# jianzhnie/RLZero

Measured on AMD Instinct MI355X. Metric: mcts_sims_per_sec, higher is better.
Workload: dtype f32 net (hi + lo f16 operand pairs on the f16 MFMA pipe, f32 accumulation) / f64 tree

## Files before the change

### include/rlzero_hip.h

```cpp
#ifndef RLZERO_HIP_H
#define RLZERO_HIP_H

#include <stdint.h>

#ifdef __cplusplus
extern "C" {
#endif

#define RZ_ABI_VERSION 31
#define RZ_MAX_BOARD_SIZE 16
#define RZ_BOARD_WORDS 4
#define RZ_MAX_IN_FLIGHT 16

enum {
    RZ_OK = 0,
    RZ_ERR_ARG = -1,
    RZ_ERR_HIP = -2,
    RZ_ERR_OOM = -3,
    RZ_ERR_OVERFLOW = -4,
    RZ_ERR_ILLEGAL = -5,
    RZ_ERR_INTERNAL = -6
};

enum {
    RZ_GAME_GOMOKU = 0,
    RZ_GAME_CONNECT4 = 1
};

enum {
    RZ_SCORE_UCT_REF = 0,
    RZ_SCORE_PUCT = 1
};

enum { RZ_EVAL_V0 = 0, RZ_EVAL_VLIN = 1 };

enum {
    RZ_FLAG_ARENA_FULL = 1,
    RZ_FLAG_BLOCKS_FULL = 2,
    RZ_FLAG_ILLEGAL_MOVE = 4,
    RZ_FLAG_LOGTAB = 8,
    RZ_FLAG_INTERNAL = 16,
    RZ_FLAG_REUSE_DROPPED = 32
};

typedef struct rz_engine rz_engine;

typedef struct rz_config {
    int32_t abi_version;
    int32_t game_kind;
    int32_t board_size;
    int32_t n_in_row;
    int32_t n_games;
    int32_t n_playout;
    int32_t score_mode;
    int32_t add_noise;
    double c_puct;
    double pool_factor;
    int32_t device;
    int32_t noise_seed;
    int32_t board_height;
    int32_t board_width;
    int32_t sims_in_flight;
    int32_t in_flight_impl;
} rz_config;

typedef struct rz_stats {
    int32_t error_flags;
    int32_t first_bad_game;
    int64_t arena_slots;
    int64_t prior_floats;
    int64_t max_slots_used;
    int64_t max_blocks_used;
    int64_t device_bytes;
    int64_t n_select_calls;
    int64_t reuse_dropped;
} rz_stats;

int rz_abi_version(void);
const char *rz_source_hash(void);
const char *rz_last_error(void);

int rz_create(const rz_config *cfg, rz_engine **out);
int rz_destroy(rz_engine *e);
int rz_geometry(rz_engine *e, int32_t *height, int32_t *width, int32_t *n_actions);

int rz_upload_log_table(rz_engine *e, const double *h_table, int64_t count);
int rz_log_table_size(rz_engine *e, int64_t *count);

int rz_set_roots(rz_engine *e, const uint64_t *d_stones, const int32_t *d_to_move,
                 const int32_t *d_last_move, const uint8_t *d_mask, int reset_trees,
                 void *stream);
int rz_get_roots(rz_engine *e, uint64_t *d_stones, int32_t *d_to_move, int32_t *d_last_move,
                 void *stream);
int rz_set_active(rz_engine *e, const uint8_t *d_active, void *stream);
int rz_set_noise_keys(rz_engine *e, const uint64_t *d_keys, const uint8_t *d_mask, void *stream);

int rz_select_step(rz_engine *e, float *d_obs, void *stream);
int rz_set_in_flight(rz_engine *e, int32_t k_backup, int32_t k_select);

int rz_leaf_buffers(rz_engine *e, const uint64_t **d_stones, const int32_t **d_to_move, const int32_t **d_last_cell);

int rz_encode_leaf_obs(rz_engine *e, float *d_obs, void *stream);
int rz_encode_root_obs(rz_engine *e, float *d_obs, void *stream);

int rz_get_leaves(rz_engine *e, uint64_t *d_stones, int32_t *d_to_move, int32_t *d_last_move,
                  int32_t *d_terminal, void *stream);

int rz_eval_synthetic(rz_engine *e, int kind, float *d_logp, float *d_value, void *stream);

int rz_eval_rollout(rz_engine *e, uint64_t seed, uint32_t sim_index, int32_t n_limit, float *d_value,
                    void *stream);

int rz_expand_backup(rz_engine *e, const float *d_logp, const float *d_value, void *stream);
int rz_expand_backup_f64(rz_engine *e, const float *d_logp, const double *d_value, void *stream);
int rz_expand_backup_probs(rz_engine *e, const float *d_probs, const double *d_value, void *stream);

int rz_tree_step(rz_engine *e, const float *d_logp, const float *d_value, float *d_obs, void *stream);

typedef struct rz_raw_heads {
    const float *raw;
    const float *hid;
    const float *w2;
    const float *b2;
    const float *act_scale;
    const float *act_bias;
    const float *val_scale;
    const float *val_bias;
    int64_t raw_part_stride;
    int64_t hid_part_stride;
    int32_t ld;
    int32_t n_parts;
} rz_raw_heads;

int rz_expand_backup_raw(rz_engine *e, const rz_raw_heads *heads, void *stream);
int rz_tree_step_raw(rz_engine *e, const rz_raw_heads *heads, float *d_obs, void *stream);

typedef struct rz_value_head {
    const float *valfeat;
    const float *w1t;
    const float *b1;
    const float *w2;
    const float *b2;
    int32_t ld;
    int32_t groups;
} rz_value_head;
typedef struct rz_deferred_logits {
    const float *raw;
    int32_t ld;
    int32_t rows_per_slot;
} rz_deferred_logits;
int rz_deferred_reserve(rz_engine *e, int32_t slots);
int rz_trace_attach(rz_engine *e, void *d_trace);
int rz_device_view(rz_engine *e, void *out, int64_t out_bytes);
int rz_set_playouts(rz_engine *e, const int32_t *d_counts, const int32_t *d_order, void *stream);
int rz_playouts_view(rz_engine *e, const int32_t **d_counts, const int32_t **d_order);
int rz_playouts_read(rz_engine *e, int32_t *h_counts, int32_t *h_order, int32_t *h_source);
int rz_deferred_slots(rz_engine *e, const int32_t **d_slot_of_game);
int rz_expand_backup_deferred(rz_engine *e, const rz_value_head *head, void *stream);
int rz_tree_step_deferred(rz_engine *e, const rz_value_head *head, void *stream);
int rz_deferred_flush(rz_engine *e, const rz_deferred_logits *logits, int32_t n_slots, void *stream);
typedef struct rz_kept_rows {
    const int32_t *rows;
    const int32_t *count;
    int64_t capacity;
    int32_t n_games;
    int32_t reserved;
} rz_kept_rows;
int rz_deferred_keep(rz_engine *e, rz_kept_rows *out, void *stream);
int rz_deferred_flush_kept(rz_engine *e, const rz_deferred_logits *logits, void *stream);
int rz_deferred_keep_stats(rz_engine *e, uint64_t *h_out2, int32_t reset);

int rz_root_visits(rz_engine *e, int32_t *d_visits, void *stream);
int rz_root_wsum(rz_engine *e, double *d_w, void *stream);
int rz_root_priors(rz_engine *e, float *d_p, void *stream);
int rz_root_stats(rz_engine *e, int32_t *d_n, double *d_w, void *stream);
int rz_root_values(rz_engine *e, double *d_out, void *stream);

int rz_advance_roots(rz_engine *e, const int32_t *d_moves, void *stream);

int rz_step_games(rz_engine *e, const int32_t *d_moves, int32_t *d_winner, uint8_t *d_ended,
                  void *stream);

#define RZ_PLAY_RECORD_WORDS 8
enum {
    RZ_PLAY_RUNNING = 1,
    RZ_PLAY_STALLED = 2,
    RZ_PLAY_RESOLVED = 4,
    RZ_PLAY_ENDED = 8,
    RZ_PLAY_SEARCHED = 16,
    RZ_PLAY_RESIGNED = 32,
    RZ_PLAY_NO_RESIGN = 64,
    RZ_PLAY_WOULD_RESIGN = 128,
    RZ_PLAY_FULL = 256
};
typedef struct rz_play_config {
    uint64_t seed;
    double temperature;
    double stall_margin;
    const int64_t *d_queue_ids;
    int32_t *d_queue_ctl;
    int32_t *d_log;
    int32_t ring_steps;
    int32_t reserved;
} rz_play_config;
int rz_play_attach(rz_engine *e, const rz_play_config *cfg);
int rz_play_draw(rz_engine *e, void *stream);
int rz_play_apply(rz_engine *e, void *stream);
int rz_play_set_resign(rz_engine *e, double threshold, double disabled_frac, void *stream);
int rz_play_set_cap(rz_engine *e, int32_t n_fast, double p_full, void *stream);
int rz_play_set_cap_order(rz_engine *e, int32_t longest_first);
int rz_play_set_match(rz_engine *e, const uint64_t *d_open_stones, const int32_t *d_open_to_move, const int32_t *d_open_last, int32_t n_openings,
                      void *stream);
int rz_play_side(rz_engine *e, int32_t side, void *stream);
int rz_active_read(rz_engine *e, uint8_t *h_active);
int rz_play_resolve(rz_engine *e, int32_t slot, int32_t move, void *stream);
int rz_play_stop(rz_engine *e, void *stream);
int rz_play_state(rz_engine *e, int64_t *h_game_id, int32_t *h_ply, int32_t *h_state, int64_t *h_steps);

int rz_get_stats(rz_engine *e, rz_stats *out);
int rz_clear_errors(rz_engine *e);
int rz_poll_errors(rz_engine *e, int32_t *h_flags, int32_t *h_reuse_dropped, void *stream);

int rz_copy_arena(rz_engine *e, int32_t game, int64_t max_slots, int32_t *h_n, double *h_w,
                  int32_t *h_first_child, int32_t *h_n_visited, int32_t *h_n_children,
                  int32_t *h_prior_block, float *h_root_prior, int32_t *h_top);
int rz_copy_priors(rz_engine *e, int32_t game, int64_t max_floats, float *h_priors, int32_t *h_count);

int rz_uct_scores(rz_engine *e, const double *d_w, const int32_t *d_n, const int32_t *d_np,
                  double c_puct, double *d_out, int64_t count, void *stream);

typedef struct rz_net rz_net;
enum {
    RZ_NET_DIRECT = 0,
    RZ_NET_WINOGRAD_F4 = 1,
    RZ_NET_SPLIT_F16 = 2
    ,
    RZ_NET_SPLIT_F16_TILES = 3
    ,
    RZ_NET_SPLIT_F16_FP8 = 4
};
int rz_net_range_info(rz_net *net, float *h_info8);
enum { RZ_NET_FLAG_F16_RANGE = 1 };
int rz_net_error_flags(rz_net *net, uint32_t *h_flags);
int rz_net_set_algo(rz_net *net, int32_t algo);
int rz_net_set_max_workgroups(rz_net *net, int32_t max_workgroups);
enum { RZ_NET_HEADS_AUTO = 0, RZ_NET_HEADS_F32 = 1, RZ_NET_HEADS_SPLIT_32 = 2, RZ_NET_HEADS_SPLIT_64 = 3, RZ_NET_HEADS_SPLIT_PARTS = 4,
       RZ_NET_HEADS_IN_TRUNK = 5    };
int rz_net_set_heads_algo(rz_net *net, int32_t heads_algo);
int rz_net_create(int32_t height, int32_t width, int32_t n_actions, int32_t device, rz_net **out);
int rz_net_destroy(rz_net *net);
int rz_net_load(rz_net *net, const float *const *h_params, int32_t n_params);
int rz_net_reserve(rz_net *net, int32_t max_boards);
int rz_net_trunk(rz_net *net, const float *d_obs, int32_t n_boards, float *d_feat, void *stream);
int rz_net_trunk_leaves(rz_net *net, const uint64_t *d_stones, const int32_t *d_to_move, const int32_t *d_last_cell,
                        int32_t n_boards, void *stream);
int rz_net_deferred_reserve(rz_net *net, int32_t max_boards, int32_t slots);
int rz_net_trunk_leaves_deferred(rz_net *net, const uint64_t *d_stones, const int32_t *d_to_move, const int32_t *d_last_cell,
                                 int32_t n_boards, const int32_t *d_slot_of_board, rz_value_head *out, void *stream);
int rz_net_deferred_gemm(rz_net *net, int32_t n_boards, int32_t n_slots, rz_deferred_logits *out, void *stream);
int rz_net_deferred_gemm_rows(rz_net *net, const rz_kept_rows *kept, rz_deferred_logits *out, void *stream);
int rz_net_trace_attach(rz_net *net, void *d_trace);
int rz_net_delta_reserve(rz_net *net, int32_t n_games);
int rz_net_delta_invalidate(rz_net *net, void *stream);
int rz_net_delta_resident(rz_net *net, int32_t on);
int rz_net_delta_bases(rz_net *net, const uint64_t *d_root_stones, const int32_t *d_root_to_move, int32_t n_games, void *stream);
int rz_net_delta_leaves(rz_net *net, const uint64_t *d_stones, const int32_t *d_to_move, const int32_t *d_last_cell, int32_t n_boards,
                        const int32_t *d_slot_of_board, const uint8_t *d_active, float *d_feat32, int32_t without_base, rz_value_head *out,
                        void *stream);
int rz_net_delta_bases_engine(rz_net *net, rz_engine *engine, void *stream);
int rz_net_delta_step(rz_net *net, rz_engine *engine, rz_value_head *out, void *stream);
int rz_net_delta_trunk_engine(rz_net *net, rz_engine *engine, void *stream);
int rz_net_delta_stats(rz_net *net, uint32_t *h_out8, int32_t reset);
int rz_net_search_resident(rz_net *net, rz_engine *engine, int32_t n_sims, int32_t select_first, void *stream);
int rz_net_heads(rz_net *net, int32_t n_boards, float *d_logp, float *d_value, void *stream);
int rz_net_heads_gemm(rz_net *net, int32_t n_boards, rz_raw_heads *out, void *stream);
int rz_net_forward(rz_net *net, const float *d_obs, int32_t n_boards, float *d_logp,
                   float *d_value, void *stream);

typedef struct rz_muzero rz_muzero;
typedef struct rz_mz_config {
    int32_t abi_version;
    int32_t n_games;
    int32_t n_actions;
    int32_t n_sims;
    double discount;
    double pb_c_base;
    double pb_c_init;
    int32_t device;
    int32_t reserved;
} rz_mz_config;

int rz_mz_create(const rz_mz_config *cfg, rz_muzero **out);
int rz_mz_destroy(rz_muzero *e);
int rz_mz_upload_log_table(rz_muzero *e, const double *h_table, int64_t count);
int rz_mz_init_roots(rz_muzero *e, const float *d_probs, const double *d_noise, double noise_frac,
                     const uint8_t *d_mask, void *stream);
int rz_mz_select(rz_muzero *e, int32_t *d_parent, int32_t *d_action, int32_t *d_leaf, const uint8_t *d_mask,
                 void *stream);
int rz_mz_expand_backup(rz_muzero *e, const float *d_reward, const float *d_probs, const float *d_value,
                        const uint8_t *d_mask, void *stream);
int rz_mz_load_model(rz_muzero *e, const float *const *h_params, int32_t n_params, int32_t hidden);
int rz_mz_search(rz_muzero *e, float *d_hidden, int32_t n_sims, int32_t *d_trace_parent, int32_t *d_trace_action,
                 int32_t *d_trace_leaf, float *d_trace_reward, float *d_trace_probs, float *d_trace_value, void *stream);
int rz_mz_set_search_shape(rz_muzero *e, int32_t games_per_workgroup);
typedef struct rz_mz_cartpole_play {
    double *d_state;
    int64_t *d_steps, *d_episode, *d_episode_start;
    uint64_t env_seed, noise_seed;
    double noise_frac, dirichlet_alpha, temperature;
    double *d_ring;
    int32_t ring_steps, reserved;
    int64_t first_step;
    double *d_arena;
    int64_t arena_rows;
    int64_t *d_counters, *d_entries;
    int64_t max_entries;
} rz_mz_cartpole_play;
int rz_mz_load_representation(rz_muzero *e, const float *const *h_params, int32_t n_params, int32_t obs_dim, int32_t hidden);
int rz_mz_play_cartpole(rz_muzero *e, float *d_hidden, int32_t n_sims, int32_t n_moves, const rz_mz_cartpole_play *play, void *stream);
int rz_cartpole_step(double *d_state, int64_t *d_steps, int64_t *d_episode, const int64_t *d_actions, int32_t n_envs, uint64_t seed,
                     float *d_obs, float *d_reward, uint8_t *d_terminated, uint8_t *d_truncated, void *stream);
int rz_mz_root_children(rz_muzero *e, int32_t what, void *d_out, void *stream);
int rz_mz_root_stats(rz_muzero *e, int32_t *d_n, double *d_value_sum, double *d_vmin, double *d_vmax, void *stream);
int rz_mz_geometry(rz_muzero *e, int32_t *slots_per_game, int64_t *device_bytes);
int rz_mz_error_flags(rz_muzero *e, int32_t *flags);

typedef struct rz_replay rz_replay;
int rz_replay_create(int32_t board_size, int64_t capacity, int32_t device, rz_replay **out);
int rz_replay_destroy(rz_replay *r);
int rz_replay_set_tables(rz_replay *r, const int16_t *h_src_state, const int16_t *h_src_pi, void *stream);
int rz_replay_state(rz_replay *r, int64_t *count, int64_t *cursor, int64_t *capacity);
int rz_replay_add(rz_replay *r, int32_t n_games, const int32_t *h_offsets, const int32_t *h_moves, const uint8_t *h_keep,
                  const int32_t *h_winner, const float *h_pi, void *stream);
int rz_replay_gather(rz_replay *r, const int64_t *h_indices, const int64_t *d_indices, int64_t n, float *d_states, float *d_pis,
                     float *d_zs, void *stream);
int rz_replay_sample(rz_replay *r, uint64_t seed, uint64_t step, int64_t n, float *d_states, float *d_pis, float *d_zs,
                     void *stream);
int rz_replay_read(rz_replay *r, int64_t first, int64_t n, uint64_t *h_stones, int32_t *h_meta, float *h_pi, void *stream);
int rz_replay_poll_errors(rz_replay *r, int32_t *flags, void *stream);

#ifdef __cplusplus
}
#endif
#endif
```

### profiles/microbench/delta_resident_phases.py

```python
import ctypes, os, sys
sys.path.insert(0, os.environ.get('GRAFT_REPO_ROOT', '.'))
import rlzero_amd._hip as H
H.library_path = lambda: os.environ.get('RZ_NETPROF_LIB') or os.path.join(os.path.dirname(os.path.abspath(__file__)), 'librlzero_netprof.so')
import rlzero_amd._build as B
B.needs_build = lambda: False
import numpy as np, torch
from rlzero_amd.engine import HipNetEvaluator, MCTSEngine
from rlzero_amd.games.gomoku.policy_value_net import PolicyValueNet
lib = H.load()
NAMES = [(0, 'leaf + changed cells'), (1, 'distances, requests, ranks'), (3, 'maps, base records'), (4, 'bar'), (5, 'conv1'), (6, 'bar'), (7, 'conv2'),
         (9, 'bar + conv3 + heads'), (10, 'bar'), (11, 'features'), (12, 'bar'), (16, 'value layer'), (17, 'expand + backup'),
         (2, 'sel: root record'), (8, 'sel: root scan / answer'), (13, 'sel: level-0 cell'), (14, 'sel: deeper levels'), (15, 'sel: terminal test + leaf stores'),
         (18, 'selection (rest: hand-over)'), (19, 'wave 1: pre-scan'), (20, 'wave 1: wait behind it')]
sizes = [int(a) for a in sys.argv[1:]] or [1, 256, 512]
for games in sizes:
    torch.manual_seed(0)
    net = PolicyValueNet(15).to('cuda:0')
    ev = HipNetEvaluator(net, 15, 'cuda:0', max_boards=games)
    sims = 800
    eng = MCTSEngine(15, 5, n_games=games, n_playout=sims, device='cuda:0', add_noise=True)
    eng.reset_games()
    assert ev.resident_ok(eng) and ev.resident_delta_ok(eng)
    rng = np.random.default_rng(0)
    for ply in range(6):
        eng.sim_chunk(ev, 40)
        visits = eng.root_visits()
        moves = np.array([int(rng.choice(np.flatnonzero(v > 0))) for v in visits], dtype=np.int32)
        eng.advance(moves)
        eng.step(moves)
    a, b = torch.cuda.Event(enable_timing=True), torch.cuda.Event(enable_timing=True)
    ev.hip.delta_stats(reset=True)
    a.record(); eng.sim_chunk(ev, sims); b.record(); torch.cuda.synchronize()
    st = ev.hip.delta_stats()
    out = (ctypes.c_longlong * 24)()
    assert lib.rz_net_debug_profile(out) == 0
    us = 1e3 * a.elapsed_time(b) / sims
    total = out[23] / sims
    print('%d games, %d simulations: %.2f us per simulation of a game (events, bases included), %d cycles (%.2f GHz); %.2f conv3 / %.2f conv2 tiles, %.2f changed cells per leaf, %d leaves without a base' % (
        games, sims, us, total, total / us / 1e3, st['tiles3'] / max(1, st['delta'] + st['no_base']), st['tiles2'] / max(1, st['delta'] + st['no_base']),
        st['cells'] / max(1, st['delta'] + st['no_base']), st['no_base']))
    print('   ' + '  '.join('%s=%d' % (nm, out[k] / sims) for k, nm in NAMES) + '  prescans=%d' % st['prescans'], flush=True)
    eng.close(); ev.hip.close()
```

### rlzero_amd/_hip.py

```python
import ctypes
import os
from ctypes import (POINTER, Structure, c_char_p, c_double, c_int, c_int32, c_int64, c_uint32, c_uint64,
                    c_void_p)

ABI_VERSION = 31
BOARD_WORDS = 4
MAX_BOARD_SIZE = 16
MAX_IN_FLIGHT = 16

OK = 0
SCORE_UCT_REF, SCORE_PUCT = 0, 1
GAME_GOMOKU, GAME_CONNECT4 = 0, 1
NET_DIRECT, NET_WINOGRAD_F4, NET_SPLIT_F16, NET_SPLIT_F16_TILES, NET_SPLIT_F16_FP8 = 0, 1, 2, 3, 4
NET_FLAG_F16_RANGE = 1
NET_HEADS_AUTO, NET_HEADS_F32, NET_HEADS_SPLIT_32, NET_HEADS_SPLIT_64, NET_HEADS_SPLIT_PARTS, NET_HEADS_IN_TRUNK = 0, 1, 2, 3, 4, 5
EVAL_V0, EVAL_VLIN = 0, 1
FLAG_NAMES = {1: 'arena full', 2: 'block queue full', 4: 'illegal move', 8: 'ln table too short',
              16: 'internal'}
FLAG_REUSE_DROPPED = 32


class RzConfig(Structure):
    _fields_ = [('abi_version', c_int32), ('game_kind', c_int32), ('board_size', c_int32),
                ('n_in_row', c_int32), ('n_games', c_int32), ('n_playout', c_int32),
                ('score_mode', c_int32), ('add_noise', c_int32), ('c_puct', c_double),
                ('pool_factor', c_double), ('device', c_int32), ('noise_seed', c_int32),
                ('board_height', c_int32), ('board_width', c_int32),
                ('sims_in_flight', c_int32), ('in_flight_impl', c_int32)]


class RzStats(Structure):
    _fields_ = [('error_flags', c_int32), ('first_bad_game', c_int32), ('arena_slots', c_int64),
                ('prior_floats', c_int64), ('max_slots_used', c_int64), ('max_blocks_used', c_int64),
                ('device_bytes', c_int64), ('n_select_calls', c_int64), ('reuse_dropped', c_int64)]


class RzMzConfig(Structure):
    _fields_ = [('abi_version', c_int32), ('n_games', c_int32), ('n_actions', c_int32), ('n_sims', c_int32),
                ('discount', c_double), ('pb_c_base', c_double), ('pb_c_init', c_double),
                ('device', c_int32), ('reserved', c_int32)]


class RzMzCartPolePlay(Structure):
    _fields_ = [('d_state', c_void_p), ('d_steps', c_void_p), ('d_episode', c_void_p), ('d_episode_start', c_void_p),
                ('env_seed', c_uint64), ('noise_seed', c_uint64), ('noise_frac', c_double), ('dirichlet_alpha', c_double),
                ('temperature', c_double), ('d_ring', c_void_p), ('ring_steps', c_int32), ('reserved', c_int32),
                ('first_step', c_int64), ('d_arena', c_void_p), ('arena_rows', c_int64), ('d_counters', c_void_p),
                ('d_entries', c_void_p), ('max_entries', c_int64)]


class RzRawHeads(Structure):
    _fields_ = [('raw', c_void_p), ('hid', c_void_p), ('w2', c_void_p), ('b2', c_void_p), ('act_scale', c_void_p),
                ('act_bias', c_void_p), ('val_scale', c_void_p), ('val_bias', c_void_p), ('raw_part_stride', c_int64),
                ('hid_part_stride', c_int64), ('ld', c_int32), ('n_parts', c_int32)]


class RzValueHead(Structure):
    _fields_ = [('valfeat', c_void_p), ('w1t', c_void_p), ('b1', c_void_p), ('w2', c_void_p), ('b2', c_void_p),
                ('ld', c_int32), ('groups', c_int32)]


class RzDeferredLogits(Structure):
    _fields_ = [('raw', c_void_p), ('ld', c_int32), ('rows_per_slot', c_int32)]


class RzKeptRows(Structure):
    _fields_ = [('rows', c_void_p), ('count', c_void_p), ('capacity', c_int64), ('n_games', c_int32), ('reserved', c_int32)]


class RzPlayConfig(Structure):
    _fields_ = [('seed', c_uint64), ('temperature', c_double), ('stall_margin', c_double), ('d_queue_ids', c_void_p),
                ('d_queue_ctl', c_void_p), ('d_log', c_void_p), ('ring_steps', c_int32), ('reserved', c_int32)]


PLAY_RECORD_WORDS = 8
PLAY_RUNNING, PLAY_STALLED, PLAY_RESOLVED, PLAY_ENDED, PLAY_SEARCHED = 1, 2, 4, 8, 16
PLAY_RESIGNED, PLAY_NO_RESIGN, PLAY_WOULD_RESIGN = 32, 64, 128
PLAY_FULL = 256
REPLAY_BAD_INDEX = 1


class HipError(RuntimeError):
    pass


P = c_void_p

_SIGNATURES = {
    'rz_abi_version': (c_int, []),
    'rz_last_error': (c_char_p, []),
    'rz_source_hash': (c_char_p, []),
    'rz_create': (c_int, [POINTER(RzConfig), POINTER(c_void_p)]),
    'rz_destroy': (c_int, [P]),
    'rz_geometry': (c_int, [P, POINTER(c_int32), POINTER(c_int32), POINTER(c_int32)]),
    'rz_upload_log_table': (c_int, [P, P, c_int64]),
    'rz_log_table_size': (c_int, [P, POINTER(c_int64)]),
    'rz_set_roots': (c_int, [P, P, P, P, P, c_int, P]),
    'rz_get_roots': (c_int, [P, P, P, P, P]),
    'rz_set_active': (c_int, [P, P, P]),
    'rz_set_noise_keys': (c_int, [P, P, P, P]),
    'rz_select_step': (c_int, [P, P, P]),
    'rz_set_in_flight': (c_int, [P, c_int32, c_int32]),
    'rz_leaf_buffers': (c_int, [P, POINTER(c_void_p), POINTER(c_void_p), POINTER(c_void_p)]),
    'rz_encode_leaf_obs': (c_int, [P, P, P]),
    'rz_encode_root_obs': (c_int, [P, P, P]),
    'rz_get_leaves': (c_int, [P, P, P, P, P, P]),
    'rz_eval_synthetic': (c_int, [P, c_int, P, P, P]),
    'rz_eval_rollout': (c_int, [P, c_uint64, c_uint32, c_int32, P, P]),
    'rz_expand_backup': (c_int, [P, P, P, P]),
    'rz_expand_backup_f64': (c_int, [P, P, P, P]),
    'rz_expand_backup_probs': (c_int, [P, P, P, P]),
    'rz_tree_step': (c_int, [P, P, P, P, P]),
    'rz_expand_backup_raw': (c_int, [P, POINTER(RzRawHeads), P]),
    'rz_tree_step_raw': (c_int, [P, POINTER(RzRawHeads), P, P]),
    'rz_trace_attach': (c_int, [P, P]),
    'rz_net_trace_attach': (c_int, [P, P]),
    'rz_device_view': (c_int, [P, P, c_int64]),
    'rz_deferred_reserve': (c_int, [P, c_int32]),
    'rz_deferred_slots': (c_int, [P, POINTER(c_void_p)]),
    'rz_expand_backup_deferred': (c_int, [P, POINTER(RzValueHead), P]),
    'rz_tree_step_deferred': (c_int, [P, POINTER(RzValueHead), P]),
    'rz_deferred_flush': (c_int, [P, POINTER(RzDeferredLogits), c_int32, P]),
    'rz_deferred_keep': (c_int, [P, POINTER(RzKeptRows), P]),
    'rz_deferred_flush_kept': (c_int, [P, POINTER(RzDeferredLogits), P]),
    'rz_deferred_keep_stats': (c_int, [P, POINTER(c_uint64), c_int32]),
    'rz_root_visits': (c_int, [P, P, P]),
    'rz_root_wsum': (c_int, [P, P, P]),
    'rz_root_priors': (c_int, [P, P, P]),
    'rz_root_stats': (c_int, [P, P, P, P]),
    'rz_root_values': (c_int, [P, P, P]),
    'rz_advance_roots': (c_int, [P, P, P]),
    'rz_step_games': (c_int, [P, P, P, P, P]),
    'rz_play_attach': (c_int, [P, POINTER(RzPlayConfig)]),
    'rz_play_draw': (c_int, [P, P]),
    'rz_play_apply': (c_int, [P, P]),
    'rz_play_set_resign': (c_int, [P, c_double, c_double, P]),
    'rz_play_set_cap': (c_int, [P, c_int32, c_double, P]),
    'rz_set_playouts': (c_int, [P, P, P, P]),
    'rz_playouts_view': (c_int, [P, POINTER(c_void_p), POINTER(c_void_p)]),
    'rz_play_set_cap_order': (c_int, [P, c_int32]),
    'rz_playouts_read': (c_int, [P, P, P, POINTER(c_int32)]),
    'rz_play_set_match': (c_int, [P, P, P, P, c_int32, P]),
    'rz_play_side': (c_int, [P, c_int32, P]),
    'rz_active_read': (c_int, [P, P]),
    'rz_play_resolve': (c_int, [P, c_int32, c_int32, P]),
    'rz_play_stop': (c_int, [P, P]),
    'rz_play_state': (c_int, [P, P, P, P, POINTER(c_int64)]),
    'rz_get_stats': (c_int, [P, POINTER(RzStats)]),
    'rz_clear_errors': (c_int, [P]),
    'rz_poll_errors': (c_int, [P, POINTER(c_int32), POINTER(c_int32), P]),
    'rz_copy_arena': (c_int, [P, c_int32, c_int64, P, P, P, P, P, P, P, P]),
    'rz_copy_priors': (c_int, [P, c_int32, c_int64, P, P]),
    'rz_uct_scores': (c_int, [P, P, P, P, c_double, P, c_int64, P]),
    'rz_net_create': (c_int, [c_int32, c_int32, c_int32, c_int32, POINTER(c_void_p)]),
    'rz_net_destroy': (c_int, [P]),
    'rz_net_set_algo': (c_int, [P, c_int32]),
    'rz_net_set_max_workgroups': (c_int, [P, c_int32]),
    'rz_net_set_heads_algo': (c_int, [P, c_int32]),
    'rz_net_error_flags': (c_int, [P, POINTER(ctypes.c_uint32)]),
    'rz_net_range_info': (c_int, [P, POINTER(ctypes.c_float)]),
    'rz_net_load': (c_int, [P, POINTER(c_void_p), c_int32]),
    'rz_net_reserve': (c_int, [P, c_int32]),
    'rz_net_trunk': (c_int, [P, P, c_int32, P, P]),
    'rz_net_trunk_leaves': (c_int, [P, P, P, P, c_int32, P]),
    'rz_net_deferred_reserve': (c_int, [P, c_int32, c_int32]),
    'rz_net_trunk_leaves_deferred': (c_int, [P, P, P, P, c_int32, P, POINTER(RzValueHead), P]),
    'rz_net_deferred_gemm': (c_int, [P, c_int32, c_int32, POINTER(RzDeferredLogits), P]),
    'rz_net_deferred_gemm_rows': (c_int, [P, POINTER(RzKeptRows), POINTER(RzDeferredLogits), P]),
    'rz_net_search_resident': (c_int, [P, P, c_int32, c_int32, P]),
    'rz_net_delta_reserve': (c_int, [P, c_int32]),
    'rz_net_delta_invalidate': (c_int, [P, P]),
    'rz_net_delta_resident': (c_int, [P, c_int32]),
    'rz_net_delta_bases': (c_int, [P, P, P, c_int32, P]),
    'rz_net_delta_leaves': (c_int, [P, P, P, P, c_int32, P, P, P, c_int32, POINTER(RzValueHead), P]),
    'rz_net_delta_stats': (c_int, [P, POINTER(ctypes.c_uint32), c_int32]),
    'rz_net_delta_bases_engine': (c_int, [P, P, P]),
    'rz_net_delta_step': (c_int, [P, P, POINTER(RzValueHead), P]),
    'rz_net_delta_trunk_engine': (c_int, [P, P, P]),
    'rz_net_heads': (c_int, [P, c_int32, P, P, P]),
    'rz_net_heads_gemm': (c_int, [P, c_int32, POINTER(RzRawHeads), P]),
    'rz_net_forward': (c_int, [P, P, c_int32, P, P, P]),
    'rz_mz_create': (c_int, [POINTER(RzMzConfig), POINTER(c_void_p)]),
    'rz_mz_destroy': (c_int, [P]),
    'rz_mz_upload_log_table': (c_int, [P, P, c_int64]),
    'rz_mz_init_roots': (c_int, [P, P, P, c_double, P, P]),
    'rz_mz_select': (c_int, [P, P, P, P, P, P]),
    'rz_mz_expand_backup': (c_int, [P, P, P, P, P, P]),
    'rz_mz_load_model': (c_int, [P, POINTER(c_void_p), c_int32, c_int32]),
    'rz_mz_search': (c_int, [P, P, c_int32, P, P, P, P, P, P, P]),
    'rz_mz_set_search_shape': (c_int, [P, c_int32]),
    'rz_mz_load_representation': (c_int, [P, POINTER(c_void_p), c_int32, c_int32, c_int32]),
    'rz_mz_play_cartpole': (c_int, [P, P, c_int32, c_int32, POINTER(RzMzCartPolePlay), P]),
    'rz_cartpole_step': (c_int, [P, P, P, P, c_int32, c_uint64, P, P, P, P, P]),
    'rz_mz_root_children': (c_int, [P, c_int32, P, P]),
    'rz_mz_root_stats': (c_int, [P, P, P, P, P, P]),
    'rz_mz_geometry': (c_int, [P, POINTER(c_int32), POINTER(c_int64)]),
    'rz_mz_error_flags': (c_int, [P, POINTER(c_int32)]),
    'rz_replay_create': (c_int, [c_int32, c_int64, c_int32, POINTER(c_void_p)]),
    'rz_replay_destroy': (c_int, [P]),
    'rz_replay_set_tables': (c_int, [P, P, P, P]),
    'rz_replay_state': (c_int, [P, POINTER(c_int64), POINTER(c_int64), POINTER(c_int64)]),
    'rz_replay_add': (c_int, [P, c_int32, P, P, P, P, P, P]),
    'rz_replay_gather': (c_int, [P, P, P, c_int64, P, P, P, P]),
    'rz_replay_sample': (c_int, [P, c_uint64, c_uint64, c_int64, P, P, P, P]),
    'rz_replay_read': (c_int, [P, c_int64, c_int64, P, P, P, P]),
    'rz_replay_poll_errors': (c_int, [P, POINTER(c_int32), P]),
}

_lib = None


def library_path():
    return os.environ.get('RZ_HIP_LIBRARY') or os.path.join(os.path.dirname(os.path.abspath(__file__)), 'librlzero_hip.so')


def load():
    global _lib
    if _lib is not None:
        return _lib
    path = library_path()
    if not os.path.exists(path):
        raise HipError('%s is missing: the HIP extension is required (no CPU fallback). '
                       'Build it with `python -m rlzero_amd._build`.' % path)
    lib = ctypes.CDLL(path)
    for name, (restype, argtypes) in _SIGNATURES.items():
        fn = getattr(lib, name)
        fn.restype = restype
        fn.argtypes = argtypes
    got = lib.rz_abi_version()
    if got != ABI_VERSION:
        raise HipError('librlzero_hip.so has ABI %d, binding expects %d: rebuild' % (got, ABI_VERSION))
    if not os.environ.get('RZ_HIP_LIBRARY'):
        from . import _build
        built, tree = (lib.rz_source_hash() or b'').decode(), _build.source_hash()
        if built != tree:
            raise HipError('librlzero_hip.so was built from other sources (hash %s, this tree %s): python -m rlzero_amd._build' % (built, tree))
    _lib = lib
    return lib


def exported_symbols():
    return sorted(_SIGNATURES)


def check(rc, what=''):
    if rc != OK:
        msg = load().rz_last_error()
        raise HipError('%s failed (%d): %s' % (what or 'rz call', rc, (msg or b'').decode()))
```

### rlzero_amd/csrc/rz_delta.h

```cpp
#ifndef RZ_DELTA_TREE_PRIO
#define RZ_DELTA_TREE_PRIO 1
#endif
#ifndef RZ_DELTA_PRO_PRIO
#define RZ_DELTA_PRO_PRIO 0
#endif
#ifndef RZ_DELTA_PRESCAN
#define RZ_DELTA_PRESCAN 1
#endif

namespace dl {

using sp::f16x4;
using sp::f16x8;
typedef const __attribute__((address_space(3))) f16x8 *lds_frag;
typedef const __attribute__((address_space(3))) uint32_t *lds_u32;
typedef __attribute__((address_space(3))) f16x4 *lds_h4;
typedef __attribute__((address_space(3))) f32x4 *lds_v4;

constexpr int kC1Slots = 128, kC2Slots = 164;
constexpr int kT1 = 4, kT2 = 8, kT3 = 8;
constexpr int kMaxD = 4;
constexpr int P1 = rt::Geo<32>::pos_bytes, P2 = rt::Geo<64>::pos_bytes;
constexpr int kGrid = kRowW * kRowW;
constexpr int kShareFloats = kT3 * 4 * 96;
// ... 73 lines not shown
#pragma unroll
    for (int t = 0; t < NT; ++t) acc[0][t] = f32x4{0.f, 0.f, 0.f, 0.f};
    constexpr int AHEAD = NT <= 2 ? 2 : 1;
    uint32_t rec[3][NT][3];
    f16x8 b[AHEAD + 1][NT][2];
#pragma unroll
    for (int dx = 0; dx < 3; ++dx) lookup<NT>(rec[dx], map, pos19, dx, g);
#pragma unroll
    for (int u = 0; u < AHEAD; ++u) read_unit<32, NT, NT>(b[u], rec[u / 3], 0, u % 3, 0);
#pragma unroll
    for (int u = 0; u < 9; ++u) {
        const int dx = u / 3, dy = u % 3;
        if (u + AHEAD < 9) read_unit<32, NT, NT>(b[(u + AHEAD) % (AHEAD + 1)], rec[(u + AHEAD) / 3], 0, (u + AHEAD) % 3, 0);
        mfma_unit<1, NT, NT>(acc, a2[dy * 3 + dx], b[u % (AHEAD + 1)], 0);
        __builtin_amdgcn_sched_barrier(0);
    }
}

#ifndef RZ_DELTA_RING6_UPTO
#define RZ_DELTA_RING6_UPTO 2
#endif
constexpr int ring3(int nt) { return nt <= RZ_DELTA_RING6_UPTO ? 6 : 3; }
__device__ __forceinline__ void load_a3(f16x8 (&a)[2][2], __amdgpu_buffer_rsrc_t w_rsrc, int lane, int dx, int j) {
    using G = rt::Geo<64>;
    const int c = j / 3, dy = j % 3;
#pragma unroll
    for (int m = 0; m < 2; ++m)
#pragma unroll
        for (int p = 0; p < 2; ++p)
            a[m][p] = sp::load_w(w_rsrc, lane * 16, dx * (G::chunks * 2048) + ((m * G::steps + dy * 3 * G::chunks + c) * 2 + p) * 1024);
}
template <int NT>
__device__ __forceinline__ void conv3_g(lds_u32 map, const uint16_t *list3, const void *wts, int lane, bool sync, f32x4 (&acc)[2][NT]) {
    static_assert(NT <= 6, "two units per step");
    constexpr int R = ring3(NT), H = units_of(NT);
    const int n = lane & 15, g = lane >> 4;
    const __amdgpu_buffer_rsrc_t w_rsrc = __builtin_amdgcn_make_buffer_rsrc(const_cast<void *>(wts), 0, 0x7fffffff, 0x00020000);
    f16x8 a3[R][2][2];
#pragma unroll
    for (int j = 0; j < R - 1; ++j) load_a3(a3[j], w_rsrc, lane, 0, j);
    if (sync) __syncthreads();
    int pos19[NT];
#pragma unroll
    for (int t = 0; t < NT; ++t) pos19[t] = (int)list3[16 * t + n] - 19;
#pragma unroll
    for (int m = 0; m < 2; ++m)
#pragma unroll
        for (int t = 0; t < NT; ++t) acc[m][t] = f32x4{0.f, 0.f, 0.f, 0.f};
    uint32_t rec[NT][3], recn[NT][3];
#ifndef RZ_DELTA_AHEAD3_SMALL
#define RZ_DELTA_AHEAD3_SMALL 1
#endif
    constexpr int UT = unit_tiles(NT), AH = UT <= 2 ? RZ_DELTA_AHEAD3_SMALL : 1, NB = AH + 1;
    static_assert((6 * H) % NB == 0 && AH <= H * 6, "a unit's registers are a constant of the unrolled body");
    f16x8 b[NB][UT][2];
    lookup<NT>(rec, map, pos19, 0, g);
#pragma unroll
    for (int u = 0; u < AH; ++u) read_unit<64, NT, UT>(b[u], rec, u % H, (u / H) % 3, u / H / 3);
#pragma unroll 1
    for (int dx = 0; dx < 3; ++dx) {
        lookup<NT>(recn, map, pos19, dx < 2 ? dx + 1 : 2, g);
#pragma unroll
        for (int u = 0; u < 6 * H; ++u) {
            const int j = u / H, h = u % H;
            if (h == 0) {
                const int jj = j + R - 1, dx2 = jj < 6 ? dx : (dx < 2 ? dx + 1 : 2);
                load_a3(a3[jj % R], w_rsrc, lane, dx2, jj % 6);
            }
            {
                const int v = u + AH;
                if (v < 6 * H) read_unit<64, NT, UT>(b[v % NB], rec, v % H, (v / H) % 3, v / H / 3);
                else read_unit<64, NT, UT>(b[v % NB], recn, (v - 6 * H) % H, ((v - 6 * H) / H) % 3, (v - 6 * H) / H / 3);
            }
            mfma_unit<2, NT, UT>(acc, a3[j % R], b[u % NB], h);
            __builtin_amdgcn_sched_barrier(0);
        }
#pragma unroll
        for (int t = 0; t < NT; ++t)
#pragma unroll
            for (int dy = 0; dy < 3; ++dy) rec[t][dy] = recn[t][dy];
    }
}

template <int T>
__device__ __forceinline__ void reduce_scatter(const float (&vals)[6 * T], float (&out)[6 * T / 4]) {
    float r1[3 * T];
#pragma unroll
    for (int i = 0; i < 3 * T; ++i) {
        const auto sw = __builtin_amdgcn_permlane16_swap(__float_as_uint(vals[i]), __float_as_uint(vals[3 * T + i]), false, false);
        r1[i] = __uint_as_float(sw[0]) + __uint_as_float(sw[1]);
    }
#pragma unroll
    for (int i = 0; i < 3 * T / 2; ++i) {
        const auto sw = __builtin_amdgcn_permlane32_swap(__float_as_uint(r1[i]), __float_as_uint(r1[3 * T / 2 + i]), false, false);
        out[i] = __uint_as_float(sw[0]) + __uint_as_float(sw[1]);
    }
}

template <int NT>
__device__ __forceinline__ void conv2_tiles(lds_u32 map1, lds_u32 map2, const uint16_t *list2, int n2, int lane, int wave, const f16x8 (&a2)[9][1][2],
                                            f32x4 bias2, float k2) {
    const int n = lane & 15, g = lane >> 4;
    int pos19[NT];
#pragma unroll
    for (int t = 0; t < NT; ++t) pos19[t] = (int)list2[16 * t + n] - 19;
    f32x4 acc[1][NT];
    conv2_g<NT>(map1, pos19, lane, a2, acc);
#pragma unroll
    for (int t = 0; t < NT; ++t) {
        if (16 * t + n < n2) {
            const uint32_t rec = map2[pos19[t] + kRowW + 1] + (uint32_t)((16 * wave + 4 * g) * 2);
            float z[4];
#pragma unroll
            for (int j = 0; j < 4; ++j) z[j] = fmaxf(fmaf(acc[0][t][j], k2, bias2[j]), 0.0f);
            f16x4 hi, lo;
            sp::split4(z, hi, lo);
            *(lds_h4)(uintptr_t)rec = hi;
            *(lds_h4)(uintptr_t)(rec + 128) = lo;
        }
    }
}

template <int NT>
__device__ __forceinline__ void conv3_tiles(lds_u32 map2, const uint16_t *list3, const void *wts, int lane, int wave, bool sync,
                                            const char *headw, float k3, float *shares) {
    constexpr int T = NT <= 4 ? 4 : 8;
    const int n = lane & 15, g = lane >> 4;
    float vals[6 * T];
    {
        f32x4 acc[2][NT];
        conv3_g<NT>(map2, list3, wts, lane, sync, acc);
        f32x4 hwr[2][6], b3r[2];
#pragma unroll
        for (int m = 0; m < 2; ++m) {
            const int c0 = 32 * wave + 16 * m + 4 * g;
#pragma unroll
            for (int i = 0; i < 6; ++i) hwr[m][i] = *reinterpret_cast<const f32x4 *>(headw + (c0 * 6 + 4 * i) * 4);
            b3r[m] = *reinterpret_cast<const f32x4 *>(headw + 128 * 6 * 4 + c0 * 4);
        }
#pragma unroll
        for (int t = 0; t < T; ++t) {
            f32x2 v2[3] = {f32x2{0.0f, 0.0f}, f32x2{0.0f, 0.0f}, f32x2{0.0f, 0.0f}};
            if (t < NT) {
#pragma unroll
                for (int m = 0; m < 2; ++m)
#pragma unroll
                    for (int j = 0; j < 4; ++j) {
                        const float hv = fmaxf(fmaf(acc[m][t < NT ? t : 0][j], k3, b3r[m][j]), 0.0f);
#pragma unroll
                        for (int o2 = 0; o2 < 3; ++o2) {
                            const int e = 6 * j + 2 * o2;
                            v2[o2] = __builtin_elementwise_fma(f32x2{hwr[m][e >> 2][e & 3], hwr[m][e >> 2][(e & 3) + 1]}, f32x2{hv, hv}, v2[o2]);
                        }
                    }
            }
#pragma unroll
            for (int o = 0; o < 6; ++o) vals[t * 6 + o] = v2[o >> 1][o & 1];
        }
    }
    float mine[6 * T / 4];
    reduce_scatter<T>(vals, mine);
    const int t0 = (T / 2) * (g & 1) + (T / 4) * (g >> 1);
#pragma unroll
    for (int i = 0; i < 6 * T / 4; ++i)
        if (t0 + i / 6 < NT) shares[((t0 + i / 6) * 4 + wave) * 96 + (i % 6) * 16 + n] = mine[i];
}

struct Leaf {
    f16x4 cell_planes;
    const char *base;
    int dys[kMaxD], dxs[kMaxD];
    _Float16 *dst16;
    float *vdst;
    float *dst32;
    const uint64_t *sets;
    bool deferred, store_head;
};
struct Layers {
    float k1, k2, k3, act1, act2, act3;
    const char *t2p, *t3p;
};
#ifdef RZ_NET_PROFILE
struct Prof { long long acc[24], t; };
#else
struct Prof {};
#endif

__device__ __forceinline__ void init_maps(char *lds, int tid) {
    uint32_t *map1 = reinterpret_cast<uint32_t *>(lds + kOffMap1);
    const uint32_t zaddr = lds_addr(lds + kOffZero);
    for (int i = tid; i < 2 * kGrid; i += 256) map1[i] = zaddr;
    if (tid < 3 * 128 / 2) reinterpret_cast<uint32_t *>(lds + kOffList)[tid] = 19u | (19u << 16);
}

__device__ __forceinline__ int cell_dist(int cy, int cx, int pass, const int (&dys)[kMaxD], const int (&dxs)[kMaxD], int BH, int BW) {
    int dist = 1000;
    if (pass < 0) {
#pragma unroll
        for (int i = 0; i < kMaxD; ++i) {
            const int ady = cy > dys[i] ? cy - dys[i] : dys[i] - cy, adx = cx > dxs[i] ? cx - dxs[i] : dxs[i] - cx;
            const int d = ady > adx ? ady : adx;
            dist = d < dist ? d : dist;
        }
    } else {
        const int y0 = 8 * (pass >> 1), x0 = 8 * (pass & 1);
        const int y1 = (y0 + 8 < BH ? y0 + 8 : BH) - 1, x1 = (x0 + 8 < BW ? x0 + 8 : BW) - 1;
        const int ddy = cy < y0 ? y0 - cy : (cy > y1 ? cy - y1 : 0), ddx = cx < x0 ? x0 - cx : (cx > x1 ? cx - x1 : 0);
        dist = ddy > ddx ? ddy : ddx;
    }
    return dist;
}

constexpr int kOutside = 1 << 30;
__device__ __forceinline__ f32x4 load_rec(__amdgpu_buffer_rsrc_t rsrc, int off) {
    return __builtin_bit_cast(f32x4, __builtin_amdgcn_raw_buffer_load_b128(rsrc, off, 0, 0));
}

__device__ __forceinline__ uint64_t uni64(uint64_t v) {
    return ((uint64_t)(unsigned)__builtin_amdgcn_readfirstlane((int)(v >> 32)) << 32) | (unsigned)__builtin_amdgcn_readfirstlane((int)v);
}

template <bool SETS>
__device__ __forceinline__ int delta_passes(const NetDev &nd, const DeltaArgs &da, char *lds, int tid0, int wave, const Leaf &leaf, const Layers &ly,
                                            f32x4 headv, bool &use_delta, Prof &prof) {
    char *in0 = lds, *c1 = lds + kOffC1, *c2 = lds + kOffC2, *zrec = lds + kOffZero, *headw = lds + kOffHead;
    uint32_t *map1 = reinterpret_cast<uint32_t *>(lds + kOffMap1), *map2 = reinterpret_cast<uint32_t *>(lds + kOffMap2);
    uint16_t *list1 = reinterpret_cast<uint16_t *>(lds + kOffList), *list2 = list1 + 128, *list3 = list2 + 128;
    float *shares = reinterpret_cast<float *>(c1);
    const int mode = da.mode, BH = nd.BH, BW = nd.BW, S = nd.S;
    const float k1 = ly.k1, k2 = ly.k2, k3 = ly.k3, act1 = ly.act1, act2 = ly.act2, act3 = ly.act3;
    const char *t2p = ly.t2p, *t3p = ly.t3p;
    const char *base = leaf.base;
    const f16x4 cell_planes = leaf.cell_planes;
    const int (&dys)[kMaxD] = leaf.dys, (&dxs)[kMaxD] = leaf.dxs;
    _Float16 *dst16 = leaf.dst16;
    float *vdst = leaf.vdst, *dst32 = leaf.dst32;
    const bool deferred = leaf.deferred, store_head = leaf.store_head;
    const uint32_t zaddr = lds_addr(zrec);
    int n_conv3_tiles = 0, n_conv2_tiles = 0;
#ifdef RZ_NET_PROFILE
    long long (&prof_acc)[24] = prof.acc, &prof_t = prof.t;
#endif
    for (int pass = use_delta ? -1 : 0; pass < 4; ++pass) {
        int tid = tid0;
        asm volatile("" : "+v"(tid));
        const int lane = tid & 63, g = lane >> 4;
        const int cy = (tid * da.bw_rcp) >> 16, cx = tid - cy * BW;
        const bool is_cell = tid < S;
        const int mypos = is_cell ? (cy + 1) * kRowW + cx + 1 : 0;
        if (RZ_DELTA_PRO_PRIO) __builtin_amdgcn_s_setprio(RZ_DELTA_PRO_PRIO);
        const int th[5] = {pass < 0 ? 1 : 2, pass < 0 ? 2 : 1, pass < 0 ? 3 : 0, pass < 0 ? 3 : 2, pass < 0 ? 4 : 1};
        bool f[5];
        uint64_t own[5];
        const bool handed = SETS && pass < 0;
        if (handed) {
#pragma unroll
            for (int k = 0; k < 5; ++k) {
                own[k] = uni64(leaf.sets[4 * (th[k] - 1) + wave]);
                f[k] = (own[k] >> lane) & 1ull;
            }
        } else {
            const int dist = cell_dist(cy, cx, pass, dys, dxs, BH, BW);
#pragma unroll
            for (int k = 0; k < 5; ++k) f[k] = is_cell && dist <= th[k];
        }
        const bool g1 = pass < 0 && f[3] && !f[0], g2 = pass < 0 && f[4] && !f[1];
        const __amdgpu_buffer_rsrc_t b_rsrc = __builtin_amdgcn_make_buffer_rsrc(const_cast<char *>(base), 0, kBaseBytes, 0x00020000);
        f32x4 r1[8], r2[16];
        {
            const int o1 = g1 ? tid * 128 : kOutside, o2 = g2 ? (int)kBaseC2 + tid * 256 : kOutside;
#pragma unroll
            for (int i = 0; i < 8; ++i) r1[i] = load_rec(b_rsrc, o1 + 16 * i);
#pragma unroll
            for (int i = 0; i < 16; ++i) r2[i] = load_rec(b_rsrc, o2 + 16 * i);
        }
        float bv[6];
        {
            const int ov = pass < 0 && is_cell && !f[2] ? (int)kBaseV + tid * 4 : kOutside;
#pragma unroll
            for (int o = 0; o < 6; ++o) bv[o] = __builtin_bit_cast(float, __builtin_amdgcn_raw_buffer_load_b32(b_rsrc, ov + o * kCells * 4, 0, 0));
        }
        sp::f16x8 a1[3][2];
        f32x4 bias1[4];
        if (32 * wave < 32 * kT1) {
#pragma unroll
            for (int ky = 0; ky < 3; ++ky)
#pragma unroll
                for (int p_ = 0; p_ < 2; ++p_) a1[ky][p_] = __builtin_bit_cast(sp::f16x8, nd.s1[(ky * 2 + p_) * 64 + lane]);
#pragma unroll
            for (int gg = 0; gg < 4; ++gg) bias1[gg] = *reinterpret_cast<const f32x4 *>(nd.b1 + 8 * gg + 4 * (lane >> 5));
        }
        f32x4 bias2 = *reinterpret_cast<const f32x4 *>(nd.b2 + 16 * wave + 4 * g);
        int rank[5], tot[5];
        if (handed) {
            const int *cnt = reinterpret_cast<const int *>(leaf.sets + kWinSets);
#pragma unroll
            for (int k = 0; k < 5; ++k) {
                int before = 0, all = 0;
#pragma unroll
                for (int w = 0; w < 4; ++w) {
                    const int c = __builtin_amdgcn_readfirstlane(cnt[4 * (th[k] - 1) + w]);
                    all += c;
                    before += w < wave ? c : 0;
                }
                rank[k] = before + (int)__builtin_amdgcn_mbcnt_hi((unsigned)(own[k] >> 32), __builtin_amdgcn_mbcnt_lo((unsigned)own[k], 0u));
                tot[k] = all;
            }
        } else {
            int before[5] = {0, 0, 0, 0, 0}, all[5] = {0, 0, 0, 0, 0};
            unsigned long long own[5] = {0ull, 0ull, 0ull, 0ull, 0ull};
#pragma unroll
            for (int b = 0; b < 4; ++b) {
                const int cell = 64 * b + lane, by = (cell * da.bw_rcp) >> 16, bx = cell - by * BW;
                const int d = cell_dist(by, bx, pass, dys, dxs, BH, BW);
#pragma unroll
                for (int k = 0; k < 5; ++k) {
                    const unsigned long long m = __ballot(cell < S && d <= th[k]);
                    const int c = __popcll(m);
                    all[k] += c;
                    before[k] += b < wave ? c : 0;
                    own[k] = b == wave ? m : own[k];
                }
            }
#pragma unroll
            for (int k = 0; k < 5; ++k) {
                rank[k] = before[k] + (int)__builtin_amdgcn_mbcnt_hi((unsigned)(own[k] >> 32), __builtin_amdgcn_mbcnt_lo((unsigned)own[k], 0u));
                tot[k] = all[k];
            }
        }
        NET_TICK(1);
        if (pass < 0 && (tot[0] > 32 * kT1 || tot[1] > 16 * kT2 || tot[2] > 16 * kT3 || tot[3] > kC1Slots || tot[4] > kC2Slots)) {
            use_delta = false;
            continue;
        }
        uint32_t rec1 = 0, rec2 = 0;
        if (f[3]) {
            rec1 = lds_addr(c1 + rank[3] * P1);
            map1[mypos] = rec1;
        }
        if (f[4]) {
            rec2 = lds_addr(c2 + rank[4] * P2);
            map2[mypos] = rec2;
        }
        if (f[0]) list1[rank[0]] = (uint16_t)mypos;
        if (f[1]) list2[rank[1]] = (uint16_t)mypos;
        if (f[2]) list3[rank[2]] = (uint16_t)mypos;
        if (pass <= 0 && is_cell) *reinterpret_cast<f16x4 *>(in0 + ((cy + 1) * sp::kInCols + (cx + 1)) * 8) = cell_planes;
        if (pass <= 0 && store_head && tid < 226) reinterpret_cast<f32x4 *>(headw)[tid] = headv;
        if (g1) {
#pragma unroll
            for (int i = 0; i < 8; ++i) *(lds_v4)(uintptr_t)(rec1 + 16 * i) = r1[i];
        }
        if (g2) {
#pragma unroll
            for (int i = 0; i < 16; ++i) *(lds_v4)(uintptr_t)(rec2 + 16 * i) = r2[i];
        }
        __builtin_amdgcn_sched_barrier(0);
        f16x8 a2[9][1][2];
        {
            const __amdgpu_buffer_rsrc_t w_rsrc = __builtin_amdgcn_make_buffer_rsrc(const_cast<char *>(t2p), 0, 0x7fffffff, 0x00020000);
#pragma unroll
            for (int tap = 0; tap < 9; ++tap)
#pragma unroll
                for (int p = 0; p < 2; ++p) a2[tap][0][p] = sp::load_w(w_rsrc, lane * 16, (tap * 2 + p) * 1024);
        }
        NET_TICK(3);
        __syncthreads();
        NET_TICK(4);

        if (32 * wave < tot[0]) {
            const int n32 = lane & 31, h = lane >> 5, idx = 32 * wave + n32;
            const int pos = list1[idx];
            const int py = (pos * 3641) >> 16, px = pos - py * kRowW;
            typedef const __attribute__((address_space(3))) f16x4 *lds_half;
            const lds_half q = (lds_half)(in0 + ((py - 1) * sp::kInCols + (px - 1) + 2 * h) * 8);
            sp::f16x8 b1[3];
#pragma unroll
            for (int ky = 0; ky < 3; ++ky) {
                const int o = ky * sp::kInCols;
                const f16x4 lo4 = q[o], hi4 = q[o + 1];
                b1[ky] = __builtin_shufflevector(lo4, hi4, 0, 1, 2, 3, 4, 5, 6, 7);
            }
            sp::f32x16 acc1;
#pragma unroll
            for (int r = 0; r < 16; ++r) acc1[r] = 0.0f;
#pragma unroll
            for (int ky = 0; ky < 3; ++ky)
#pragma unroll
                for (int combo = 0; combo < 3; combo += 2)
                    acc1 = __builtin_amdgcn_mfma_f32_32x32x16_f16(a1[ky][combo == 2], b1[ky], acc1, 0, 0, 0);
            if (idx < tot[0]) {
                const uint32_t rec = map1[pos] + (uint32_t)(4 * h * 2);
#pragma unroll
                for (int gg = 0; gg < 4; ++gg) {
                    float z[4];
#pragma unroll
                    for (int j = 0; j < 4; ++j) z[j] = fmaxf(fmaf(acc1[4 * gg + j], k1, bias1[gg][j] * act1), 0.0f);
                    f16x4 hi, lo;
                    sp::split4(z, hi, lo);
                    *(lds_h4)(uintptr_t)(rec + 8 * gg * 2) = hi;
                    *(lds_h4)(uintptr_t)(rec + 8 * gg * 2 + 64) = lo;
                }
            }
        }
        NET_TICK(5);
        __syncthreads();
        NET_TICK(6);
        if (mode == 1 && f[0]) {
            f32x4 *dstp = reinterpret_cast<f32x4 *>(const_cast<char *>(base) + (size_t)tid * 128);
#pragma unroll
            for (int i = 0; i < 8; ++i) dstp[i] = *(lds_v4)(uintptr_t)(rec1 + 16 * i);
        }

        if (RZ_DELTA_PRO_PRIO) __builtin_amdgcn_s_setprio(0);
        const int nt3 = (tot[2] + 15) >> 4;
        {
            const lds_u32 m1 = (lds_u32)map1, m2 = (lds_u32)map2;
            const int nt2 = (tot[1] + 15) >> 4;
            n_conv2_tiles += nt2;
            for (int t0 = 0; t0 < nt2; t0 += 4) {
                const uint16_t *l2 = list2 + 16 * t0;
                const int left = tot[1] - 16 * t0;
                switch (nt2 - t0) {
                    case 1: conv2_tiles<1>(m1, m2, l2, left, lane, wave, a2, bias2 * act2, k2); break;
                    case 2: conv2_tiles<2>(m1, m2, l2, left, lane, wave, a2, bias2 * act2, k2); break;
                    case 3: conv2_tiles<3>(m1, m2, l2, left, lane, wave, a2, bias2 * act2, k2); break;
                    default: conv2_tiles<4>(m1, m2, l2, left, lane, wave, a2, bias2 * act2, k2); break;
                }
            }
        }
        NET_TICK(7);

        {
            const lds_u32 m2 = (lds_u32)map2;
            n_conv3_tiles += nt3;
            const int first = nt3 <= 6 ? nt3 : 4;
            switch (first) {
                case 0: __syncthreads(); break;
                case 1: conv3_tiles<1>(m2, list3, t3p, lane, wave, true, headw, k3, shares); break;
                case 2: conv3_tiles<2>(m2, list3, t3p, lane, wave, true, headw, k3, shares); break;
                case 3: conv3_tiles<3>(m2, list3, t3p, lane, wave, true, headw, k3, shares); break;
                case 4: conv3_tiles<4>(m2, list3, t3p, lane, wave, true, headw, k3, shares); break;
                case 5: conv3_tiles<5>(m2, list3, t3p, lane, wave, true, headw, k3, shares); break;
                default: conv3_tiles<6>(m2, list3, t3p, lane, wave, true, headw, k3, shares); break;
            }
            if (nt3 == 7) conv3_tiles<3>(m2, list3 + 64, t3p, lane, wave, false, headw, k3, shares + 4 * 4 * 96);
            else if (nt3 >= 8) conv3_tiles<4>(m2, list3 + 64, t3p, lane, wave, false, headw, k3, shares + 4 * 4 * 96);
        }
        NET_TICK(9);
        __syncthreads();
        NET_TICK(10);
        if (mode == 1 && f[1]) {
            f32x4 *dstp = reinterpret_cast<f32x4 *>(const_cast<char *>(base) + kBaseC2 + (size_t)tid * 256);
#pragma unroll
            for (int i = 0; i < 16; ++i) dstp[i] = *(lds_v4)(uintptr_t)(rec2 + 16 * i);
        }

        if (is_cell && (pass < 0 || f[2])) {
            const float *share = shares + (rank[2] >> 4) * 4 * 96 + (rank[2] & 15);
            float *basev = mode == 1 ? reinterpret_cast<float *>(const_cast<char *>(base) + kBaseV) : nullptr;
#pragma unroll
            for (int o = 0; o < 6; ++o) {
                float v;
                if (f[2]) {
                    float s = share[o * 16];
#pragma unroll
                    for (int w = 1; w < 4; ++w) s += share[w * 96 + o * 16];
                    v = fmaxf(s + reinterpret_cast<const float *>(headw + 128 * 7 * 4)[o], 0.0f);
                } else {
                    v = bv[o];
                }
                if (mode == 1) {
                    basev[o * kCells + tid] = v;
                    continue;
                }
                if (dst32) dst32[o * S + tid] = v;
                if (deferred && o >= 4) {
                    vdst[(o - 4) * S + tid] = v;
                } else if (dst16) {
                    const int k = (o < 4 ? o : o - 4) * S + tid;
                    const int step = (o < 4 ? 0 : nd.groups_act) + (k >> 4);
                    const float z = v * act3;
                    const _Float16 zh = (_Float16)z;
                    _Float16 *q = dst16 + (size_t)step * 1024 + (k & 15);
                    q[0] = zh;
                    q[512] = (_Float16)(z - (float)zh);
                }
            }
        }
        if (f[3]) map1[mypos] = zaddr;
        if (f[4]) map2[mypos] = zaddr;
        NET_TICK(11);
        if (pass < 0) break;
        __syncthreads();
    }
    return n_conv3_tiles | (n_conv2_tiles << 16);
}

__device__ __forceinline__ f16x4 planes_of(const uint64_t (&ls)[8], int tid, int tm_eff, bool has_last, int lc, int par_count) {
    f16x4 cell_planes;
    const int word = (tid >> 6) & 3, bit = tid & 63;
    uint64_t w0 = 0ull, w1 = 0ull;
#pragma unroll
    for (int w = 0; w < 4; ++w) {
        const uint64_t mk = word == w ? ~0ull : 0ull;
        w0 |= ls[w] & mk;
        w1 |= ls[4 + w] & mk;
    }
    const bool s0 = (w0 >> bit) & 1ull, s1 = (w1 >> bit) & 1ull;
    const bool mine = tm_eff == 0 ? s0 : s1, theirs = tm_eff == 0 ? s1 : s0;
    const _Float16 one = (_Float16)sp::kObsScale, zero = (_Float16)0.0f;
    cell_planes[0] = mine ? one : zero;
    cell_planes[1] = theirs ? one : zero;
    cell_planes[2] = (has_last && tid == lc) ? one : zero;
    cell_planes[3] = (par_count & 1) ? zero : one;
    return cell_planes;
}

__device__ __forceinline__ bool changed_cells(const uint64_t (&ls)[8], const uint64_t (&rs)[8], int nst, int tm, int lc, bool has_last, bool base_ok, int h_tm,
                                              int bw_rcp, int BW, int (&dys)[kMaxD], int (&dxs)[kMaxD], int &parity, int &nD) {
    bool use_delta = false;
    {
        bool sup = true;
        int nroot = 0;
        uint64_t D[4] = {0ull, 0ull, 0ull, 0ull};
#pragma unroll
        for (int q = 0; q < 8; ++q) {
            sup = sup && (rs[q] & ~ls[q]) == 0ull;
            nroot += __popcll(rs[q]);
            D[q & 3] |= rs[q] ^ ls[q];
        }
#pragma unroll
        for (int w = 0; w < 4; ++w) D[w] |= (has_last && lc >= 0 && (lc >> 6) == w) ? 1ull << (lc & 63) : 0ull;
        parity = (nst - nroot) & 1;
        nD = __popcll(D[0]) + __popcll(D[1]) + __popcll(D[2]) + __popcll(D[3]);
        use_delta = base_ok && sup && tm == (h_tm ^ parity) && nD <= kMaxD;
#pragma unroll
        for (int i = 0; i < kMaxD; ++i) {
            const bool z0 = D[0] == 0ull, z1 = D[1] == 0ull, z2 = D[2] == 0ull;
            const int w = !z0 ? 0 : !z1 ? 1 : !z2 ? 2 : 3;
            const uint64_t word = !z0 ? D[0] : !z1 ? D[1] : !z2 ? D[2] : D[3];
            const bool any = word != 0ull;
            const int cell = 64 * w + __builtin_ctzll(word | (1ull << 63));
            const uint64_t rest = word & (word - 1ull);
#pragma unroll
// ... 121 lines not shown
    }
    {
        const auto a = __builtin_amdgcn_permlane32_swap(lo, lo, false, false), b = __builtin_amdgcn_permlane32_swap(hi, hi, false, false);
        lo = a[0] | a[1];
        hi = b[0] | b[1];
    }
    const uint64_t v = ((uint64_t)hi << 32) | lo;
    int *cnt = reinterpret_cast<int *>(ws + kWinSets);
    if (lane < kWinSets) {
        ws[lane] = v;
        cnt[lane] = __popcll(v);
    }
    if (lane == 0) cnt[kWinSets] = (use_delta ? 1 : 0) | (parity << 1) | (nD << 8);
}
__device__ __forceinline__ void leaf_windows(const uint64_t *leaf_lds, const uint64_t (&rs)[8], bool base_ok, int h_tm, const DeltaArgs &da, int BW,
                                             int lane, uint64_t *ws) {
    uint64_t ls[8];
    int nst = 0;
#pragma unroll
    for (int q = 0; q < 8; ++q) {
        ls[q] = uni64(leaf_lds[q]);
        nst += __popcll(ls[q]);
    }
    const int tm = __builtin_amdgcn_readfirstlane(reinterpret_cast<const int *>(leaf_lds + 2 * RZ_BOARD_WORDS)[0]);
    const int lc = __builtin_amdgcn_readfirstlane(reinterpret_cast<const int *>(leaf_lds + 2 * RZ_BOARD_WORDS)[1]);
    int dys[kMaxD], dxs[kMaxD], parity = 0, nD = 0;
    const bool use_delta = changed_cells(ls, rs, nst, tm, lc, nst > 0, base_ok, h_tm, da.bw_rcp, BW, dys, dxs, parity, nD);
    const int i = lane >> 4;
    int dy = dys[0], dx = dxs[0];
#pragma unroll
    for (int j = 1; j < kMaxD; ++j) {
        dy = i == j ? dys[j] : dy;
        dx = i == j ? dxs[j] : dx;
    }
    const bool any = dy >= 0;
    const uint64_t row = da.win[(any ? dy * BW + dx : 0) * kWinSets + (lane & (kWinSets - 1))];
    windows_store(any ? row : 0ull, use_delta, parity, nD, lane, ws);
}

#if defined(RZ_NET_PROFILE) && !defined(RZ_SEL_TICKS)
#define RZ_SEL_TICKS 0
#endif
struct ResHook {
    static constexpr bool kOn = true;
    rzt::RootPre *pre;
    const uint64_t *win;
    int depth;
    bool any0;
    uint64_t row;
    __device__ __forceinline__ void root_cell(int last, int stones, int lane) {
        any0 = stones > 0 && last >= 0 && last < kCells;
        row = win[(any0 ? last : 0) * kWinSets + (lane & (kWinSets - 1))];
    }
    __device__ __forceinline__ void cell(int level, int c, int lane) {
        const uint64_t v = win[c * kWinSets + (lane & (kWinSets - 1))];
        row = (lane >> 4) == level ? v : row;
    }
#ifdef RZ_NET_PROFILE
    Prof *prof;
    __device__ __forceinline__ void tick(int i, int arrived) {
        if ((RZ_SEL_TICKS >> i) & 1) {
            asm volatile("" ::"v"(arrived));
            const int slot = i == 0 ? 2 : i == 1 ? 8 : 12 + i;
            __builtin_amdgcn_sched_barrier(0);
            const long long now = __builtin_readcyclecounter();
            prof->acc[slot] += now - prof->t;
            prof->t = now;
            __builtin_amdgcn_sched_barrier(0);
        }
    }
#else
    __device__ __forceinline__ void tick(int, int) {}
#endif
};

__device__ __forceinline__ void path_windows(const ResHook &hook, bool base_ok, int lane, uint64_t *ws) {
    const int depth = hook.depth;
    const bool mine = depth == 0 ? (lane < 16 && hook.any0) : (lane >> 4) < depth;
    const int nD = depth == 0 ? (hook.any0 ? 1 : 0) : depth;
    windows_store(mine ? hook.row : 0ull, base_ok && nD <= kMaxD, depth & 1, nD, lane, ws);
}

constexpr int kResVrow = 512;
__global__ __launch_bounds__(256, 2) void k_delta_res(NetDev nd, _Float16 *__restrict__ store16, DeferredOut later, DeltaArgs da, ResArgs<true> res) {
    __shared__ __attribute__((aligned(16))) char lds[kLdsBytes];
    __shared__ float res_vrow[kResVrow];
    __shared__ float res_part[rzt::kDefWaves][rzt::kWave];
    __shared__ __attribute__((aligned(16))) uint64_t res_leaf[2 * RZ_BOARD_WORDS + 2];
    __shared__ __attribute__((aligned(16))) uint64_t res_win[kWinLds / 8];
    __shared__ __attribute__((aligned(16))) rzt::RootPre res_pre;
    const int game = res.order != nullptr ? res.order[blockIdx.x] : (int)blockIdx.x;
    if ((unsigned)game >= (unsigned)res.E.n_games || res.E.active[game] == 0) return;
    const int n_sims = res_sims(res, game);
    const unsigned long long clk0 = __builtin_readcyclecounter(), rt0 = __builtin_amdgcn_s_memrealtime();
    const int tid0 = threadIdx.x, wave = __builtin_amdgcn_readfirstlane(tid0 >> 6);
    const int BW = nd.BW;
    Prof prof;
#ifdef RZ_NET_PROFILE
    for (int i = 0; i < 24; ++i) prof.acc[i] = 0;
    prof.t = __builtin_readcyclecounter();
    const long long prof_k0 = prof.t;
    long long (&prof_acc)[24] = prof.acc, &prof_t = prof.t;
#endif
    Layers ly;
    ly.t2p = reinterpret_cast<const char *>(nd.t2) + (size_t)wave * rt::Geo<32>::steps * 2 * 1024;
    ly.t3p = reinterpret_cast<const char *>(nd.t3) + (size_t)(2 * wave) * rt::Geo<64>::steps * 2 * 1024;
    f32x4 headv = tid0 < 192 ? reinterpret_cast<const f32x4 *>(nd.whp)[tid0] : reinterpret_cast<const f32x4 *>(nd.b3)[(tid0 - 192) & 31];
    {
        const float *bh = nd.bh + (tid0 == 225 ? 4 : 0);
        const f32x4 hbv = {bh[0], bh[1], tid0 == 225 ? 0.0f : bh[2], tid0 == 225 ? 0.0f : bh[3]};
        headv = (tid0 == 224 || tid0 == 225) ? hbv : headv;
    }
    ly.k1 = nd.s_inv[2], ly.k2 = nd.s_inv[0], ly.k3 = nd.s_inv[1];
    ly.act1 = nd.s_inv[5], ly.act2 = nd.s_inv[6], ly.act3 = nd.s_inv[7];
    const int slot0 = res.E.pend[game];
    uint64_t rs[8];
    bool base_ok = da.hdr[game].valid != 0;
#pragma unroll
    for (int q = 0; q < 8; ++q) {
        rs[q] = res.E.root_stones[(size_t)game * 8 + q];
        base_ok = base_ok && da.hdr[game].stones[q] == rs[q];
    }
    const int h_tm = res.E.root_to_move[game];
    base_ok = base_ok && da.hdr[game].to_move == h_tm;
    {
        const f32x4 zero = {0.f, 0.f, 0.f, 0.f};
        f32x4 *z = reinterpret_cast<f32x4 *>(lds);
        for (int i = tid0; i < sp::kInPieceBytes / 16; i += 256) z[i] = zero;
        if (tid0 < P2 / 16) reinterpret_cast<f32x4 *>(lds + kOffZero)[tid0] = zero;
        init_maps(lds, tid0);
        for (int i = tid0; i < kResVrow; i += 256) res_vrow[i] = 0.0f;
    }
    if (tid0 == 0) res_pre.scan = res_pre.valid = res_pre.answered = 0;
    ResHook hook;
    hook.pre = &res_pre;
    hook.win = da.win;
    hook.depth = 0;
    hook.any0 = false;
    hook.row = 0ull;
#ifdef RZ_NET_PROFILE
    hook.prof = &prof;
    long long pre_cycles = 0, pre_wait = 0;
#endif
    if (res.select_first == 0 && tid0 == 0) {
#pragma unroll
        for (int q = 0; q < 8; ++q) res_leaf[q] = res.E.leaf_stones[(size_t)game * 8 + q];
        reinterpret_cast<int *>(res_leaf + 2 * RZ_BOARD_WORDS)[0] = res.E.leaf_to_move[game];
        reinterpret_cast<int *>(res_leaf + 2 * RZ_BOARD_WORDS)[1] = res.E.leaf_last[game];
    }
    __syncthreads();
    if (wave == 0) {
        const int lane0 = tid0 & 63;
        if (res.select_first != 0) {
            rzt::select_body<false, rzt::kWords, ResHook>(res.E, nullptr, game, lane0, 0, res_leaf, &hook);
            path_windows(hook, base_ok, lane0, res_win);
        } else {
            leaf_windows(res_leaf, rs, base_ok, h_tm, da, BW, lane0, res_win);
        }
    }
    __syncthreads();
    int tiles_total = 0, tiles2_total = 0, deltas = 0, cells_total = 0;
    for (int sim = 0; sim < n_sims; ++sim) {
        int tid_s = tid0;
        asm volatile("" : "+v"(tid_s));
        uint64_t ls[8];
        int nst = 0;
#pragma unroll
        for (int q = 0; q < 8; ++q) {
            const uint64_t v = res_leaf[q];
            ls[q] = ((uint64_t)(unsigned)__builtin_amdgcn_readfirstlane((int)(v >> 32)) << 32) | (unsigned)__builtin_amdgcn_readfirstlane((int)v);
            nst += __popcll(ls[q]);
        }
        const int tm = __builtin_amdgcn_readfirstlane(reinterpret_cast<const int *>(res_leaf + 2 * RZ_BOARD_WORDS)[0]);
        const int lc = __builtin_amdgcn_readfirstlane(reinterpret_cast<const int *>(res_leaf + 2 * RZ_BOARD_WORDS)[1]);
        const bool has_last = nst > 0;
        const int verdict = __builtin_amdgcn_readfirstlane(reinterpret_cast<const int *>(res_win + kWinSets)[kWinSets]);
        bool use_delta = (verdict & 1) != 0;
        const int parity = (verdict >> 1) & 1, nD = verdict >> 8;
        Leaf leaf;
        leaf.sets = res_win;
#pragma unroll
        for (int i = 0; i < kMaxD; ++i) leaf.dys[i] = leaf.dxs[i] = -100;
        leaf.base = da.recs + ((size_t)game * 2 + parity) * kBaseBytes;
        leaf.cell_planes = planes_of(ls, tid_s, tm, has_last, lc, nst);
        leaf.dst16 = slot0 + sim < later.n_slots ? store16 + (size_t)(slot0 + sim) * later.slot_halfs + (size_t)(game >> 5) * nd.groups_act * 1024 + (game & 31) * 16 : nullptr;
        leaf.vdst = res_vrow;
        leaf.dst32 = nullptr;
        leaf.deferred = true;
        leaf.store_head = sim == 0;
        NET_TICK(0);
        const int n_tiles = delta_passes<true>(nd, da, lds, tid_s, wave, leaf, ly, headv, use_delta, prof);
        tiles_total += n_tiles & 0xffff;
        tiles2_total += n_tiles >> 16;
        deltas += use_delta ? 1 : 0;
        cells_total += nD;
        __syncthreads();
        NET_TICK(12);
        const int lane = tid_s & 63;
        if (RZ_DELTA_TREE_PRIO) __builtin_amdgcn_s_setprio(RZ_DELTA_TREE_PRIO);
        if (res.vh.groups == 128) rzt::value_quarter_lds<16>(res.vh, res_vrow, lane, wave, res_part);
        else rzt::value_quarter_lds<8>(res.vh, res_vrow, lane, wave, res_part);
        NET_TICK(16);
        const bool more = sim + 1 < n_sims;
        if (wave == 0) {
            rzt::expand_backup_body<float, false, false, false, true>(res.E, nullptr, nullptr, game, lane, rz_raw_heads(), 0, res.vh, res_part);
        } else {
            __syncthreads();
            if (RZ_DELTA_PRESCAN && wave == 1 && more) {
#ifdef RZ_NET_PROFILE
                const long long t0 = __builtin_readcyclecounter();
#endif
                rzt::root_prescan<rzt::kWords>(res.E, game, lane, &res_pre);
#ifdef RZ_NET_PROFILE
                __builtin_amdgcn_s_waitcnt(0);
                const long long t1 = __builtin_readcyclecounter();
                pre_cycles += t1 - t0;
                pre_wait -= t1;
#endif
            }
        }
        __syncthreads();
#ifdef RZ_NET_PROFILE
        if (RZ_DELTA_PRESCAN && wave == 1 && more) pre_wait += __builtin_readcyclecounter();
#endif
        NET_TICK(17);
        if (wave == 0 && more) {
            hook.depth = 0, hook.any0 = false, hook.row = 0ull;
            int lane_t = lane;
            asm volatile("" : "+v"(lane_t));
            rzt::select_body<false, rzt::kWords, ResHook>(res.E, nullptr, game, lane_t, 0, res_leaf, &hook);
            path_windows(hook, base_ok, lane_t, res_win);
        }
        if (RZ_DELTA_TREE_PRIO) __builtin_amdgcn_s_setprio(0);
        __syncthreads();
        NET_TICK(18);
    }
    if (da.stats != nullptr && tid0 == 0) {
        atomicAdd(da.stats + 0, (unsigned)deltas);
        atomicAdd(da.stats + 1, (unsigned)(n_sims - deltas));
        atomicAdd(da.stats + 2, (unsigned)tiles_total);
        atomicAdd(da.stats + 3, (unsigned)cells_total);
        atomicAdd(da.stats + 4, (unsigned)tiles2_total);
        atomicAdd(da.stats + 5, (unsigned)res_pre.answered);
        if (game == 0) {
            da.stats[6] = (unsigned)((__builtin_readcyclecounter() - clk0) >> 8);
            da.stats[7] = (unsigned)(__builtin_amdgcn_s_memrealtime() - rt0);
        }
    }
#ifdef RZ_NET_PROFILE
    if (blockIdx.x == 0 && tid0 == 0) {
        for (int i = 0; i < 24; ++i)
            if (i != 19 && i != 20) net_prof[i] = prof_acc[i];
        net_prof[23] = __builtin_readcyclecounter() - prof_k0;
        net_prof[22] = tiles_total;
    }
    if (blockIdx.x == 0 && tid0 == 64) {
        net_prof[19] = pre_cycles;
        net_prof[20] = pre_wait;
    }
#endif
}

}
```

### rlzero_amd/csrc/rz_engine.hip

```cpp

#include <hip/hip_runtime.h>

#include <algorithm>
#include <cmath>
#include <cstdarg>
#include <cstdio>
#include <cstring>
#include <new>
#include <vector>

#include "rlzero_hip.h"
#include "rz_trace.h"

#pragma clang fp contract(off)

#include "rz_tree.h"

using namespace rzt;

namespace {

__global__ __launch_bounds__(kWave) void k_select(Dev E, float *obs) {
    __builtin_amdgcn_s_setprio(3);
    select_body<false>(E, obs, blockIdx.x, threadIdx.x);
// ... 41 lines not shown
    value_quarter_def<PER>(vh, blockIdx.x, lane, wave, part);
    if (wave != 0) {
        __syncthreads();
        return;
    }
    expand_backup_body<float, false, false, false, true, words_of_per<PER>()>(E, nullptr, nullptr, blockIdx.x, lane, RawHeads(), 0, vh, part);
    __syncthreads();
    select_body<false, words_of_per<PER>()>(E, obs, blockIdx.x, lane);
    if (TRACE && lane == 0) rz_trace_write(E.trace, RZ_TRACE_TREE, E.pend[blockIdx.x] - 1, blockIdx.x, trace_t0);
}

__device__ __forceinline__ void deferred_priors_body(const Dev &E, int g, long long rec, const float *__restrict__ r, int lane) {
    const int pb = E.pend_pb[rec];
    if (pb < 0) return;
    const int ctr = E.pend_ctr[rec];
    uint64_t st[2][kWords];
    load_board(E.pend_stones, (int)rec, st);
    float x[kWords];
    float mx = -INFINITY;
#pragma unroll
    for (int i = 0; i < kWords; ++i) {
        const int j = lane + 64 * i;
        x[i] = j < E.A ? r[j] : -INFINITY;
        mx = fmaxf(mx, x[i]);
    }
    mx = wave_max(mx, lane);
    float sum = 0.0f;
#pragma unroll
    for (int i = 0; i < kWords; ++i) sum += (lane + 64 * i < E.A) ? expf(x[i] - mx) : 0.0f;
    sum = wave_sum(sum, lane);
    const float lse = mx + logf(sum);
    float *P = arena_priors(E, g, E.cur_arena[g]);
    uint64_t occ[kWords];
#pragma unroll
    for (int j = 0; j < kWords; ++j) occ[j] = st[0][j] | st[1][j];
    const Legal L = legal_of(E, occ, lane);
    int ranks[kWords];
    int before = 0;
#pragma unroll
    for (int j = 0; j < kWords; ++j) ranks[j] = lane_action_rank(E, occ, L, j, lane, before);
    float noise[kWords] = {0.f, 0.f, 0.f, 0.f};
    float noise_sum = 1.0f;
    if (E.add_noise) {
        const uint64_t key = mix64(mix64(E.noise_key[g]) ^ (uint64_t)ctr);
        float local = 0.0f;
#pragma unroll
        for (int j = 0; j < kWords; ++j)
            if (ranks[j] >= 0) {
                noise[j] = gamma03(hash32((uint32_t)key ^ (uint32_t)(key >> 32)) + 0x9E3779B9u * (uint32_t)(64 * j + lane + 1));
                local += noise[j];
            }
        local = wave_sum(local, lane);
        noise_sum = local > 0.0f ? local : 1.0f;
    }
#pragma unroll
    for (int j = 0; j < kWords; ++j) {
        const int rk = ranks[j];
        if (rk < 0) continue;
        float prior = expf(x[j] - lse);
        if (E.add_noise) prior = 0.75f * prior + 0.25f * (noise[j] / noise_sum);
        P[pb + rk] = prior;
    }
}

__global__ __launch_bounds__(kWave) void k_deferred_priors(Dev E, const float *__restrict__ raw, int ld, long long rows_per_slot) {
    const int g = blockIdx.x, slot = blockIdx.y, lane = threadIdx.x;
    if (slot >= E.pend[g]) return;
    deferred_priors_body(E, g, (long long)slot * E.n_games + g, raw + ((size_t)slot * rows_per_slot + g) * ld, lane);
}

struct Keep {
    unsigned long long *mask;
    int32_t *cnt, *pcnt;
    int32_t *rows;
    int32_t *count;
    unsigned long long *stats;
    int words;
};

__global__ __launch_bounds__(256) void k_keep_mark(Dev E, const int32_t *__restrict__ keep_of, Keep Kp) {
    __shared__ int sh[4][2];
    const int g = blockIdx.x, tid = threadIdx.x, lane = tid & 63, wave = tid >> 6;
    const int n = E.pend[g] < E.pend_cap ? E.pend[g] : E.pend_cap;
    const int keep = keep_of[g];
    uint64_t root[2][kWords], occ[kWords];
    load_board(E.root_stones, g, root);
#pragma unroll
    for (int j = 0; j < kWords; ++j) occ[j] = root[0][j] | root[1][j];
    const Legal L = legal_of(E, occ, lane);
    int rank = 0, cell = 0;
    const bool all = keep < 0 || !locate_action(E, occ, L, keep, rank, cell);
    const bool second = E.root_to_move[g] != 0;
    int kept = 0, with_block = 0;
    for (int s0 = 64 * wave; s0 < n; s0 += 256) {
        const int s = s0 + lane;
        const long long rec = (long long)s * E.n_games + g;
        const bool has = s < n && E.pend_pb[rec] >= 0;
        bool need = has && all;
        if (has && !all) {
            uint64_t st[2][kWords];
            load_board(E.pend_stones, (int)rec, st);
            bool same = true;
            uint64_t mine[kWords];
#pragma unroll
            for (int j = 0; j < kWords; ++j) {
                same = same && st[0][j] == root[0][j] && st[1][j] == root[1][j];
                mine[j] = second ? st[1][j] : st[0][j];
            }
            need = same || test_bit(mine, cell);
        }
        const unsigned long long m = __ballot(need);
        if (lane == 0) Kp.mask[(long long)g * Kp.words + (s0 >> 6)] = m;
        kept += __popcll(m);
        with_block += __popcll(__ballot(has));
    }
    if (lane == 0) sh[wave][0] = kept, sh[wave][1] = with_block;
    __syncthreads();
    if (tid == 0) {
        Kp.cnt[g] = (sh[0][0] + sh[1][0]) + (sh[2][0] + sh[3][0]);
        Kp.pcnt[g] = (sh[0][1] + sh[1][1]) + (sh[2][1] + sh[3][1]);
    }
}

__global__ __launch_bounds__(kWave) void k_keep_rows(Dev E, Keep Kp) {
    const int g = blockIdx.x, lane = threadIdx.x;
    const bool last = g == E.n_games - 1;
    int base = 0, pending = 0;
    for (int h = lane; h < g; h += kWave) base += Kp.cnt[h];
    if (last)
        for (int h = lane; h < E.n_games; h += kWave) pending += Kp.pcnt[h];
    for (int off = 32; off >= 1; off >>= 1) {
        base += __shfl_xor(base, off);
        pending += __shfl_xor(pending, off);
    }
    const int n = E.pend[g] < E.pend_cap ? E.pend[g] : E.pend_cap;
    int at = base;
    for (int s0 = 0; s0 < n; s0 += kWave) {
        const unsigned long long m = Kp.mask[(long long)g * Kp.words + (s0 >> 6)];
        const int pre = __builtin_amdgcn_mbcnt_hi((unsigned)(m >> 32), __builtin_amdgcn_mbcnt_lo((unsigned)m, 0));
        if ((m >> lane) & 1ull) Kp.rows[at + pre] = (s0 + lane) * E.n_games + g;
        at += __popcll(m);
    }
    if (last && lane == 0) {
        Kp.count[0] = at;
        Kp.stats[0] += (unsigned long long)at;
        Kp.stats[1] += (unsigned long long)pending;
    }
}

__global__ __launch_bounds__(kWave) void k_deferred_priors_rows(Dev E, const float *__restrict__ raw, int ld, const int32_t *__restrict__ rows,
                                                                const int32_t *__restrict__ count) {
    const int lane = threadIdx.x, n = count[0];
    for (int i = blockIdx.x; i < n; i += gridDim.x) {
        const int rec = rows[i];
        deferred_priors_body(E, rec % E.n_games, rec, raw + (size_t)i * ld, lane);
    }
}

__global__ void k_deferred_reset(Dev E) {
    const int g = blockIdx.x * blockDim.x + threadIdx.x;
    if (g < E.n_games) E.pend[g] = 0;
}

template <typename VT>
__global__ __launch_bounds__(kWave) void k_tree_step(Dev E, const float *logp, const VT *value, float *obs) {
    __builtin_amdgcn_s_setprio(3);
    expand_backup_body<VT>(E, logp, value, blockIdx.x, threadIdx.x);
    __syncthreads();
    select_body<false>(E, obs, blockIdx.x, threadIdx.x);
}

template <bool RAW>
__global__ __launch_bounds__(kWave) void k_tree_step_vl(Dev E, const float *logp, const float *value, RawHeads rh,
                                                        float *obs, int kb, int ks) {
    __builtin_amdgcn_s_setprio(3);
#pragma unroll 1
    for (int j = 0; j < kb; ++j) {
        expand_backup_body<float, false, RAW, true>(E, logp, value, blockIdx.x, threadIdx.x, rh, j);
        __syncthreads();
    }
#pragma unroll 1
    for (int j = 0; j < ks; ++j) {
        select_body<true>(E, obs, blockIdx.x, threadIdx.x, j);
        __syncthreads();
    }
}

struct MlSlot {
    uint64_t st[2][kWords];
    int4 lo, hi;
    int4 xlo;
    int node, rank, owner, depth, fresh, active, to_move, last, nst, moved, pad0, pad1;
};

__host__ __device__ inline int ml_prior_bytes(int K, int A, bool puct) { return puct ? ((K * A * 4 + 15) / 16) * 16 : 0; }
__host__ __device__ inline int ml_lds_bytes(int K, int A, bool puct) {
    return K * (int)sizeof(MlSlot) + K * A * 32 + ml_prior_bytes(K, A, puct) + 64 + K * 16;
}

template <bool RAW>
__global__ void k_tree_step_ml(Dev E, const float *logp, const float *value, RawHeads rh, float *obs, int kb, int ks) {
    extern __shared__ __attribute__((aligned(16))) char ml_lds[];
    const int g = blockIdx.x, K = E.K, A = E.A, S = E.S;
    const int tid = threadIdx.x, lane = tid & 63, w = __builtin_amdgcn_readfirstlane(tid >> 6);
    const bool puct_mode = E.score_mode == RZ_SCORE_PUCT;
    MlSlot *SL = reinterpret_cast<MlSlot *>(ml_lds);
    int4 *stage = reinterpret_cast<int4 *>(ml_lds + K * sizeof(MlSlot));
    float *stage_p = reinterpret_cast<float *>(stage + (size_t)K * A * 2);
    int *misc = reinterpret_cast<int *>(reinterpret_cast<char *>(stage_p) + ml_prior_bytes(K, A, puct_mode));
    double *bval = reinterpret_cast<double *>(misc + 16);
    int *bdepth = reinterpret_cast<int *>(bval + K);
    int *bexp = bdepth + K;
    if (!E.active[g]) return;
    const int arena = E.cur_arena[g];
    int4 *R = arena_records(E, g, arena);
    float *P = arena_priors(E, g, arena);

    if (kb > 0) {
        const int j = w, gk = g * K + j;
        const bool mine = j < kb;
        const int ptop0 = E.ptop[g], nblk0 = E.nblk[g], ctr0 = E.noise_ctr[g], top0 = E.top[g];
        int depth = 0, fresh = 0, term = 0, leaf = 0, k = 0;
        double v = 0.0;
        float lse = 0.0f;
        float x[kWords] = {0.f, 0.f, 0.f, 0.f};
        uint64_t st[2][kWords] = {{0, 0, 0, 0}, {0, 0, 0, 0}}, occ[kWords] = {0, 0, 0, 0};
        Legal L;
        L.k = 0; L.cols = 0ull; L.height = 0;
        bool expand = false;
// ... 1596 lines not shown
        return launched("k_tree_step_vl");
    }
    k_expand_backup<float><<<per_game(e), dim3(kWave), 0, as_stream(stream)>>>(e->dev, d_logp, d_value);
    return launched("k_expand_backup");
}

int rz_expand_backup_f64(rz_engine *e, const float *d_logp, const double *d_value, void *stream) {
    RZ_ENTER(e);
    RZ_NO_PLAYOUTS(e);
    RZ_NEED(d_value);
    if (e->dev.K > 1) return fail(RZ_ERR_ARG, "host evaluators are not available with sims_in_flight > 1");
    k_expand_backup<double><<<per_game(e), dim3(kWave), 0, as_stream(stream)>>>(e->dev, d_logp, d_value);
    return launched("k_expand_backup");
}

int rz_expand_backup_probs(rz_engine *e, const float *d_probs, const double *d_value, void *stream) {
    RZ_ENTER(e);
    RZ_NO_PLAYOUTS(e);
    RZ_NEED(d_value);
    if (e->dev.K > 1) return fail(RZ_ERR_ARG, "host evaluators are not available with sims_in_flight > 1");
    k_expand_backup<double, true><<<per_game(e), dim3(kWave), 0, as_stream(stream)>>>(e->dev, d_probs, d_value);
    return launched("k_expand_backup");
}

int rz_tree_step(rz_engine *e, const float *d_logp, const float *d_value, float *d_obs, void *stream) {
    RZ_ENTER(e);
    RZ_NO_PLAYOUTS(e);
    RZ_NEED(d_value);
    e->n_select += 1;
    if (e->dev.K > 1) {
        if (e->ml) k_tree_step_ml<false><<<per_game(e), dim3(kWave * e->dev.K), e->ml_lds, as_stream(stream)>>>(e->dev, d_logp, d_value, RawHeads(), d_obs, e->kb, e->ks);
        else k_tree_step_vl<false><<<per_game(e), dim3(kWave), 0, as_stream(stream)>>>(e->dev, d_logp, d_value, RawHeads(), d_obs, e->kb, e->ks);
        return launched("k_tree_step_vl");
    }
    k_tree_step<float><<<per_game(e), dim3(kWave), 0, as_stream(stream)>>>(e->dev, d_logp, d_value, d_obs);
    return launched("k_tree_step");
}

static int raw_heads_ok(rz_engine *e, const rz_raw_heads *h) {
    if (!h || !h->raw || !h->hid || !h->w2 || !h->b2) return fail(RZ_ERR_ARG, "NULL device pointer");
    if (h->ld < e->dev.A) return fail(RZ_ERR_ARG, "ld %d < n_actions %d", h->ld, e->dev.A);
    if (h->n_parts != 1 && h->n_parts != 4) return fail(RZ_ERR_ARG, "n_parts %d is neither 1 nor 4", h->n_parts);
    if (h->n_parts == 4 && (!h->act_scale || !h->act_bias || !h->val_scale || !h->val_bias))
        return fail(RZ_ERR_ARG, "partial sums need their scales and biases");
    return RZ_OK;
}

int rz_expand_backup_raw(rz_engine *e, const rz_raw_heads *heads, void *stream) {
    RZ_ENTER(e);
    RZ_NO_PLAYOUTS(e);
    int rc = raw_heads_ok(e, heads);
    if (rc != RZ_OK) return rc;
    const RawHeads rh = *heads;
    if (e->dev.K > 1) {
        if (e->ml) k_tree_step_ml<true><<<per_game(e), dim3(kWave * e->dev.K), e->ml_lds, as_stream(stream)>>>(e->dev, nullptr, nullptr, rh, nullptr, e->kb, 0);
        else k_tree_step_vl<true><<<per_game(e), dim3(kWave), 0, as_stream(stream)>>>(e->dev, nullptr, nullptr, rh, nullptr, e->kb, 0);
        return launched("k_tree_step_vl");
    }
    k_expand_backup_raw<<<per_game(e), dim3(kWave), 0, as_stream(stream)>>>(e->dev, rh);
    return launched("k_expand_backup_raw");
}

static int deferred_ok(rz_engine *e, const rz_value_head *h) {
    if (h == nullptr || !h->valfeat || !h->w1t || !h->b1 || !h->w2 || !h->b2) return fail(RZ_ERR_ARG, "rz_value_head: NULL pointer");
    if ((h->groups != 16 && h->groups != 32 && h->groups != 64 && h->groups != 128) || h->ld != 4 * h->groups)
        return fail(RZ_ERR_ARG, "rz_value_head: groups = %d must be 16, 32, 64 or 128 and ld = 4 * groups", h->groups);
    if (2 * e->dev.S > 4 * h->groups)
        return fail(RZ_ERR_ARG, "rz_value_head: %d groups of 4 inputs do not hold the 2 x %d inputs of this board", h->groups, e->dev.S);
    if (e->dev.pend_cap <= 0) return fail(RZ_ERR_ARG, "call rz_deferred_reserve first");
    return RZ_OK;
}

int rz_deferred_reserve(rz_engine *e, int32_t slots) {
    int rc = check_engine(e);
    if (rc != RZ_OK) return rc;
    if (slots < 1) return fail(RZ_ERR_ARG, "rz_deferred_reserve: slots must be positive");
    if (e->cfg.score_mode != RZ_SCORE_UCT_REF || e->dev.K != 1)
        return fail(RZ_ERR_ARG, "deferred priors need RZ_SCORE_UCT_REF (the rule that never reads a prior) and sims_in_flight == 1");
    if (slots <= e->dev.pend_cap) return RZ_OK;
    RZ_HIP(hipDeviceSynchronize());
    const long long G = e->cfg.n_games;
    if ((rc = dev_alloc(e, &e->dev.pend_pb, (long long)slots * G)) != RZ_OK) return rc;
    if ((rc = dev_alloc(e, &e->dev.pend_ctr, (long long)slots * G)) != RZ_OK) return rc;
    if ((rc = dev_alloc(e, &e->dev.pend_stones, (long long)slots * G * 2 * kWords)) != RZ_OK) return rc;
    if (e->dev.pend == nullptr) {
        if ((rc = dev_alloc(e, &e->dev.pend, G)) != RZ_OK) return rc;
    }
    RZ_HIP(hipMemset(e->dev.pend, 0, (size_t)G * sizeof(int32_t)));
    Keep &kp = e->keep;
    kp.words = (slots + 63) / 64;
    if ((rc = dev_alloc(e, &kp.mask, (long long)kp.words * G)) != RZ_OK) return rc;
    if ((rc = dev_alloc(e, &kp.rows, (long long)slots * G)) != RZ_OK) return rc;
    if (kp.cnt == nullptr) {
        if ((rc = dev_alloc(e, &kp.cnt, G)) != RZ_OK || (rc = dev_alloc(e, &kp.pcnt, G)) != RZ_OK) return rc;
        if ((rc = dev_alloc(e, &kp.count, 1)) != RZ_OK || (rc = dev_alloc(e, &kp.stats, 2)) != RZ_OK) return rc;
        RZ_HIP(hipMemset(kp.stats, 0, 2 * sizeof(unsigned long long)));
    }
    RZ_HIP(hipMemset(kp.count, 0, sizeof(int32_t)));
    e->dev.pend_cap = slots;
    return RZ_OK;
}

int rz_trace_attach(rz_engine *e, void *d_trace) {
    int rc = check_engine(e);
    if (rc != RZ_OK) return rc;
    e->dev.trace = (unsigned long long *)d_trace;
    return RZ_OK;
}

int rz_device_view(rz_engine *e, void *out, int64_t out_bytes) {
    int rc = check_engine(e);
    if (rc != RZ_OK) return rc;
    if (out == nullptr || out_bytes != (int64_t)sizeof(Dev)) return fail(RZ_ERR_ARG, "rz_device_view: the caller's view is %lld bytes, the engine's %zu", (long long)out_bytes, sizeof(Dev));
    memcpy(out, &e->dev, sizeof(Dev));
    return RZ_OK;
}

int rz_deferred_slots(rz_engine *e, const int32_t **d_slot_of_game) {
    int rc = check_engine(e);
    if (rc != RZ_OK) return rc;
    if (!d_slot_of_game) return fail(RZ_ERR_ARG, "NULL output pointer");
    if (e->dev.pend_cap <= 0) return fail(RZ_ERR_ARG, "call rz_deferred_reserve first");
    *d_slot_of_game = e->dev.pend;
    return RZ_OK;
}

int rz_expand_backup_deferred(rz_engine *e, const rz_value_head *head, void *stream) {
    int rc = check_engine(e);
    if (rc != RZ_OK) return rc;
    if ((rc = deferred_ok(e, head)) != RZ_OK) return rc;
    RZ_NO_PLAYOUTS(e);
    const dim3 block(kWave * kDefWaves);
    switch (head->groups) {
        case 16: k_expand_backup_def<2><<<per_game(e), block, 0, as_stream(stream)>>>(e->dev, *head); break;
        case 32: k_expand_backup_def<4><<<per_game(e), block, 0, as_stream(stream)>>>(e->dev, *head); break;
        case 64: k_expand_backup_def<8><<<per_game(e), block, 0, as_stream(stream)>>>(e->dev, *head); break;
        default: k_expand_backup_def<16><<<per_game(e), block, 0, as_stream(stream)>>>(e->dev, *head); break;
    }
    return launched("k_expand_backup_def");
}

int rz_tree_step_deferred(rz_engine *e, const rz_value_head *head, void *stream) {
    int rc = check_engine(e);
    if (rc != RZ_OK) return rc;
    if ((rc = deferred_ok(e, head)) != RZ_OK) return rc;
    RZ_NO_PLAYOUTS(e);
    e->n_select += 1;
    const dim3 block(kWave * kDefWaves);
    if (e->dev.trace && head->groups == 128) {
        k_tree_step_def<16, true><<<per_game(e), block, 0, as_stream(stream)>>>(e->dev, *head, nullptr);
        return launched("k_tree_step_def");
    }
    switch (head->groups) {
        case 16: k_tree_step_def<2, false><<<per_game(e), block, 0, as_stream(stream)>>>(e->dev, *head, nullptr); break;
        case 32: k_tree_step_def<4, false><<<per_game(e), block, 0, as_stream(stream)>>>(e->dev, *head, nullptr); break;
        case 64: k_tree_step_def<8, false><<<per_game(e), block, 0, as_stream(stream)>>>(e->dev, *head, nullptr); break;
        default: k_tree_step_def<16, false><<<per_game(e), block, 0, as_stream(stream)>>>(e->dev, *head, nullptr); break;
    }
    return launched("k_tree_step_def");
}

int rz_deferred_flush(rz_engine *e, const rz_deferred_logits *logits, int32_t n_slots, void *stream) {
    int rc = check_engine(e);
    if (rc != RZ_OK) return rc;
    if (e->dev.pend_cap <= 0 || n_slots <= 0) return RZ_OK;
    if (!logits || !logits->raw) return fail(RZ_ERR_ARG, "rz_deferred_logits: NULL pointer");
    if (n_slots > e->dev.pend_cap) return fail(RZ_ERR_ARG, "more slots than rz_deferred_reserve()d");
    if (logits->ld < e->dev.A || logits->rows_per_slot < e->cfg.n_games) return fail(RZ_ERR_ARG, "rz_deferred_logits: rows shorter than the batch");
    k_deferred_priors<<<dim3((unsigned)e->cfg.n_games, (unsigned)n_slots), dim3(kWave), 0, as_stream(stream)>>>(
        e->dev, logits->raw, logits->ld, (long long)logits->rows_per_slot);
    if (!(e->play_on && e->play_drawn)) k_deferred_reset<<<flat_grid(e), dim3(256), 0, as_stream(stream)>>>(e->dev);
    return launched("k_deferred_priors");
}

static int keep_ok(rz_engine *e) {
    if (e->dev.pend_cap <= 0) return fail(RZ_ERR_ARG, "call rz_deferred_reserve first");
    if (!(e->play_on && e->play_drawn)) return fail(RZ_ERR_ARG, "the kept flush runs between rz_play_draw and rz_play_apply (the move decides what is kept)");
    return RZ_OK;
}

int rz_deferred_keep(rz_engine *e, rz_kept_rows *out, void *stream) {
    int rc = check_engine(e);
    if (rc != RZ_OK) return rc;
    if (!out) return fail(RZ_ERR_ARG, "NULL output pointer");
    if ((rc = keep_ok(e)) != RZ_OK) return rc;
    k_keep_mark<<<per_game(e), dim3(256), 0, as_stream(stream)>>>(e->dev, e->play.keep, e->keep);
    k_keep_rows<<<per_game(e), dim3(kWave), 0, as_stream(stream)>>>(e->dev, e->keep);
    out->rows = e->keep.rows;
    out->count = e->keep.count;
    out->capacity = (int64_t)e->dev.pend_cap * e->cfg.n_games;
    out->n_games = e->cfg.n_games;
    out->reserved = 0;
    return launched("k_keep_rows");
}

int rz_deferred_flush_kept(rz_engine *e, const rz_deferred_logits *logits, void *stream) {
    int rc = check_engine(e);
    if (rc != RZ_OK) return rc;
    if ((rc = keep_ok(e)) != RZ_OK) return rc;
    if (!logits || !logits->raw) return fail(RZ_ERR_ARG, "rz_deferred_logits: NULL pointer");
    if (logits->ld < e->dev.A) return fail(RZ_ERR_ARG, "rz_deferred_logits: rows shorter than the policy");
    k_deferred_priors_rows<<<dim3(2048), dim3(kWave), 0, as_stream(stream)>>>(e->dev, logits->raw, logits->ld, e->keep.rows, e->keep.count);
    return launched("k_deferred_priors_rows");
}

int rz_deferred_keep_stats(rz_engine *e, uint64_t *h_out2, int32_t reset) {
    int rc = check_engine(e);
    if (rc != RZ_OK) return rc;
    if (!h_out2) return fail(RZ_ERR_ARG, "NULL output pointer");
    h_out2[0] = h_out2[1] = 0;
    if (!e->keep.stats) return RZ_OK;
    RZ_HIP(hipDeviceSynchronize());
    RZ_HIP(hipMemcpy(h_out2, e->keep.stats, 2 * sizeof(uint64_t), hipMemcpyDeviceToHost));
    if (reset) RZ_HIP(hipMemset(e->keep.stats, 0, 2 * sizeof(uint64_t)));
    return RZ_OK;
}

int rz_tree_step_raw(rz_engine *e, const rz_raw_heads *heads, float *d_obs, void *stream) {
    RZ_ENTER(e);
    RZ_NO_PLAYOUTS(e);
    int rc = raw_heads_ok(e, heads);
    if (rc != RZ_OK) return rc;
    e->n_select += 1;
    const RawHeads rh = *heads;
    if (e->dev.K > 1) {
        if (e->ml) k_tree_step_ml<true><<<per_game(e), dim3(kWave * e->dev.K), e->ml_lds, as_stream(stream)>>>(e->dev, nullptr, nullptr, rh, d_obs, e->kb, e->ks);
        else k_tree_step_vl<true><<<per_game(e), dim3(kWave), 0, as_stream(stream)>>>(e->dev, nullptr, nullptr, rh, d_obs, e->kb, e->ks);
        return launched("k_tree_step_vl");
    }
    k_tree_step_raw<<<per_game(e), dim3(kWave), 0, as_stream(stream)>>>(e->dev, rh, d_obs);
    return launched("k_tree_step_raw");
}

int rz_root_visits(rz_engine *e, int32_t *d_visits, void *stream) {
    RZ_ENTER(e);
    RZ_NEED(d_visits);
    k_root_children<<<per_game(e), dim3(kWave), 0, as_stream(stream)>>>(e->dev, 0, d_visits);
    return launched("k_root_children");
}

int rz_root_wsum(rz_engine *e, double *d_w, void *stream) {
    RZ_ENTER(e);
    RZ_NEED(d_w);
    k_root_children<<<per_game(e), dim3(kWave), 0, as_stream(stream)>>>(e->dev, 1, d_w);
    return launched("k_root_children");
}

int rz_root_priors(rz_engine *e, float *d_p, void *stream) {
    RZ_ENTER(e);
    RZ_NEED(d_p);
    k_root_children<<<per_game(e), dim3(kWave), 0, as_stream(stream)>>>(e->dev, 2, d_p);
    return launched("k_root_children");
}

int rz_root_stats(rz_engine *e, int32_t *d_n, double *d_w, void *stream) {
    RZ_ENTER(e);
    RZ_NEED(d_n); RZ_NEED(d_w);
    k_root_stats<<<flat_grid(e), dim3(256), 0, as_stream(stream)>>>(e->dev, d_n, d_w);
    return launched("k_root_stats");
}

int rz_root_values(rz_engine *e, double *d_out, void *stream) {
    RZ_ENTER(e);
    RZ_NEED(d_out);
    k_root_values<<<per_game(e), dim3(kWave), 0, as_stream(stream)>>>(e->dev, d_out);
    return launched("k_root_values");
}

int rz_advance_roots(rz_engine *e, const int32_t *d_moves, void *stream) {
    RZ_ENTER(e);
    RZ_NEED(d_moves);
    k_advance<<<per_game(e), dim3(kWave), 0, as_stream(stream)>>>(e->dev, d_moves);
    return launched("k_advance");
}

int rz_step_games(rz_engine *e, const int32_t *d_moves, int32_t *d_winner, uint8_t *d_ended, void *stream) {
// ... 376 lines not shown
```

### rlzero_amd/csrc/rz_net.hip

```cpp

#include <hip/hip_runtime.h>

#include <cmath>
#include <cstdio>
#include <cstring>
#include <new>
#include <type_traits>
#include <utility>
#include <vector>

#include "rlzero_hip.h"
#include "rz_trace.h"
#include "rz_tree.h"
#include "rz_window.h"

void rz_set_error(const char *msg);

namespace {

typedef float f32x4 __attribute__((ext_vector_type(4)));
typedef float f32x2 __attribute__((ext_vector_type(2)));

constexpr int kRowW = 18;
constexpr int kPlaneDirect = 336, kPlaneWino = 337;
// ... 2988 lines not shown
    if (n_boards == 0) return RZ_OK;
    if (!d_obs) return net_fail(RZ_ERR_ARG, "NULL device pointer");
    if (net->fp8_cross)
        return net_fail(RZ_ERR_ARG, "RZ_NET_SPLIT_F16_FP8 evaluates positions (rz_net_trunk_leaves*, rz_net_search_resident): float planes are refused, "
                                    "not computed in another arithmetic");
    if (!d_feat) {
        if (n_boards > net->feat_boards) return net_fail(RZ_ERR_ARG, "batch larger than rz_net_reserve()d");
        d_feat = net->d_feat;
    }
    launch_trunk(net, d_obs, d_feat, n_boards, stream);
    if (hipGetLastError() != hipSuccess) return net_fail(RZ_ERR_HIP, "launch of k_trunk failed");
    return RZ_OK;
}

int rz_net_trunk_leaves(rz_net *net, const uint64_t *d_stones, const int32_t *d_to_move, const int32_t *d_last_cell,
                        int32_t n_boards, void *stream) {
    int rc = net_ready(net, n_boards);
    if (rc != RZ_OK) return rc;
    if (n_boards == 0) return RZ_OK;
    if (!d_stones || !d_to_move || !d_last_cell) return net_fail(RZ_ERR_ARG, "NULL device pointer");
    if (n_boards > net->feat_boards) return net_fail(RZ_ERR_ARG, "batch larger than rz_net_reserve()d");
    if (!split_trunk_ok(net))
        return net_fail(RZ_ERR_ARG, "rz_net_trunk_leaves needs the RZ_NET_SPLIT_F16 trunk (the others read float planes: rz_net_trunk)");
    launch_trunk(net, nullptr, net->d_feat, n_boards, stream, LeafBits{d_stones, d_to_move, d_last_cell});
    if (hipGetLastError() != hipSuccess) return net_fail(RZ_ERR_HIP, "launch of k_trunk_split failed");
    return RZ_OK;
}

int rz_net_deferred_reserve(rz_net *net, int32_t max_boards, int32_t slots) {
    int rc = net_ready(net, max_boards);
    if (rc != RZ_OK) return rc;
    if (slots < 1 || max_boards < 1) return net_fail(RZ_ERR_ARG, "rz_net_deferred_reserve: slots and max_boards must be positive");
    if (max_boards <= net->store_boards && slots <= net->store_slots) return RZ_OK;
    if (max_boards < net->store_boards) max_boards = net->store_boards;
    if (slots < net->store_slots) slots = net->store_slots;
    (void)hipDeviceSynchronize();
    if (net->d_store16) (void)hipFree(net->d_store16);
    if (net->d_store_raw) (void)hipFree(net->d_store_raw);
    if (net->d_valfeat) (void)hipFree(net->d_valfeat);
    net->d_store16 = nullptr;
    net->d_store_raw = net->d_valfeat = nullptr;
    net->store_boards = 0;
    net->store_slots = 0;
    const int tiles = ((max_boards + 63) / 64) * 2;
    const size_t store_bytes = (size_t)slots * tiles * net->dev.groups_act * 2048;
    const size_t raw_bytes = (size_t)slots * tiles * 32 * net->dev.Npad * sizeof(float);
    const size_t val_bytes = (size_t)tiles * 32 * net->vf_groups * 4 * sizeof(float);
    if (hipMalloc((void **)&net->d_store16, store_bytes) != hipSuccess || hipMalloc((void **)&net->d_store_raw, raw_bytes) != hipSuccess ||
        hipMalloc((void **)&net->d_valfeat, val_bytes) != hipSuccess)
        return net_fail(RZ_ERR_OOM, "hipMalloc failed (deferred-priors store)");
    if (hipMemset(net->d_store16, 0, store_bytes) != hipSuccess || hipMemset(net->d_valfeat, 0, val_bytes) != hipSuccess)
        return net_fail(RZ_ERR_HIP, "hipMemset failed (deferred-priors store)");
    net->store_tiles = tiles;
    net->store_slots = slots;
    net->store_boards = max_boards;
    return RZ_OK;
}

int rz_net_trunk_leaves_deferred(rz_net *net, const uint64_t *d_stones, const int32_t *d_to_move, const int32_t *d_last_cell,
                                 int32_t n_boards, const int32_t *d_slot_of_board, rz_value_head *out, void *stream) {
    int rc = net_ready(net, n_boards);
    if (rc != RZ_OK) return rc;
    if (!out) return net_fail(RZ_ERR_ARG, "NULL output pointer");
    if (!split_trunk_ok(net))
        return net_fail(RZ_ERR_ARG, "the deferred-priors route needs the RZ_NET_SPLIT_F16 trunk (a net with finite activation bounds)");
    if (n_boards > net->store_boards) return net_fail(RZ_ERR_ARG, "batch larger than rz_net_deferred_reserve()d");
    if (n_boards > 0) {
        if (!d_stones || !d_to_move || !d_last_cell || !d_slot_of_board) return net_fail(RZ_ERR_ARG, "NULL device pointer");
        const DeferredOut later{d_slot_of_board, (long long)net->store_tiles * net->dev.groups_act * 1024, net->d_valfeat, net->vf_groups * 4, net->d_trace, net->store_slots};
        launch_trunk(net, nullptr, net->d_feat, n_boards, stream, LeafBits{d_stones, d_to_move, d_last_cell}, later);
        if (hipGetLastError() != hipSuccess) return net_fail(RZ_ERR_HIP, "launch of the split-f16 trunk failed");
    }
    memset(out, 0, sizeof(*out));
    out->valfeat = net->d_valfeat;
    out->w1t = net->d_w1t;
    out->b1 = net->dev.fc_val1_b;
    out->w2 = net->dev.fc_val2_w;
    out->b2 = net->dev.fc_val2_b;
    out->ld = net->vf_groups * 4;
    out->groups = net->vf_groups;
    return RZ_OK;
}

int rz_net_search_resident(rz_net *net, rz_engine *engine, int32_t n_sims, int32_t select_first, void *stream) {
    rzt::Dev dev;
    int rc = rz_device_view(engine, &dev, (int64_t)sizeof(dev));
    if (rc != RZ_OK) return rc;
    if ((rc = net_ready(net, dev.n_games)) != RZ_OK) return rc;
    if (n_sims < 1) return net_fail(RZ_ERR_ARG, "rz_net_search_resident: n_sims must be positive");
    if (n_sims > net->store_slots || n_sims > dev.pend_cap) {
        char detail[160];
        snprintf(detail, sizeof(detail), ": %d simulations, %d / %d slots (rz_net_deferred_reserve / rz_deferred_reserve)", n_sims, net->store_slots, dev.pend_cap);
        return net_fail(RZ_ERR_ARG, "rz_net_search_resident: more simulations than the store has slots", detail);
    }
    const bool rows = net->algo == RZ_NET_SPLIT_F16 && rows_kernel_covers(net->dev.BH, net->dev.BW);
    const TrunkClass tc = trunk_class(net);
    if (!split_trunk_ok(net) || (!rows && (tc.ms == 0 || net->dev.BH > 10 || net->dev.BW > 10)))
        return net_fail(RZ_ERR_ARG, "the resident search needs the RZ_NET_SPLIT_F16 trunk on a board of 11 .. 16 rows and columns (the row-tile "
                                    "kernel) or of up to 10 x 10 (k_trunk_split with one N-tile per wave)");
    if (dev.K != 1 || dev.score_mode != RZ_SCORE_UCT_REF || dev.pend_cap <= 0)
        return net_fail(RZ_ERR_ARG, "the resident search is the deferred-priors route: RZ_SCORE_UCT_REF, one simulation in flight, rz_deferred_reserve first");
    if (dev.BH != net->dev.BH || dev.BW != net->dev.BW || dev.A != net->dev.A) return net_fail(RZ_ERR_ARG, "engine and network disagree on the board");
    const bool delta_res = net->delta_resident && delta_covers(net) && net->base_games >= dev.n_games;
    const bool compact_res = !rows && tc.compact;
    if (dev.n_games > net->store_boards || (!delta_res && !compact_res && dev.n_games > net->n_cus))
        return net_fail(RZ_ERR_ARG, "the resident search runs one workgroup per game, at most one per CU (any number with rz_net_delta_reserve, or on a board of "
                                    "the compact grid) and rz_net_deferred_reserve()d");
    if (rows ? (net->vf_groups != 64 && net->vf_groups != 128) : net->vf_groups > 64) return net_fail(RZ_ERR_INTERNAL, "value head groups");
    ResArgs<true> res;
    res.E = dev;
    memset(&res.vh, 0, sizeof(res.vh));
    res.vh.w1t = net->d_w1t;
    res.vh.b1 = net->dev.fc_val1_b;
    res.vh.w2 = net->dev.fc_val2_w;
    res.vh.b2 = net->dev.fc_val2_b;
    res.vh.ld = net->vf_groups * 4;
    res.vh.groups = net->vf_groups;
    res.n_sims = n_sims;
    res.select_first = select_first ? 1 : 0;
    if ((rc = rz_playouts_view(engine, &res.sims_of, &res.order)) != RZ_OK) return rc;
    const DeferredOut later{dev.pend, (long long)net->store_tiles * net->dev.groups_act * 1024, nullptr, 0, nullptr, net->store_slots};
    const LeafBits leaves{dev.leaf_stones, dev.leaf_to_move, dev.leaf_last};
    const dim3 grid((unsigned)dev.n_games);
    const hipStream_t st = (hipStream_t)stream;
    net->feat16_valid = net->feat32_valid = false;
    if (delta_res) {
        if (select_first) {
            if ((rc = rz_net_delta_bases(net, dev.root_stones, dev.root_to_move, dev.n_games, stream)) != RZ_OK) return rc;
        }
        dl::DeltaArgs da{net->d_base_hdr, net->d_base_recs, net->d_base_ones, nullptr, net->d_delta_stats, 0, (65536 + net->dev.BW - 1) / net->dev.BW, net->d_win};
        dl::k_delta_res<<<grid, dim3(256), 0, st>>>(net->dev, net->d_store16, later, da, res);
        if (hipGetLastError() != hipSuccess) return net_fail(RZ_ERR_HIP, "launch of the resident search (k_delta_res) failed");
        return RZ_OK;
    }
    if (rows)
        with_board_rows(net->dev.BH, [&](auto nt) {
            launch_search_rows<decltype(nt)::value>(grid, st, net->dev, leaves, net->d_store16, dev.n_games, net->d_flags, later, res, net->fp8_cross);
        });
    else
        launch_trunk_split<true>(tc.ms, compact_res, grid, st, net->dev, nullptr, leaves, nullptr, net->d_store16, dev.n_games, net->d_flags,
                                 nullptr, nullptr, later, res);
    if (hipGetLastError() != hipSuccess) return net_fail(RZ_ERR_HIP, "launch of the resident search failed");
    return RZ_OK;
}

int rz_net_delta_reserve(rz_net *net, int32_t n_games) {
    int rc = net_ready(net, n_games);
    if (rc != RZ_OK) return rc;
    if (!delta_covers(net))
        return net_fail(RZ_ERR_ARG, "receptive-field evaluation exists for the RZ_NET_SPLIT_F16 trunk on boards of 11 .. 16 rows and columns");
    if (n_games < 1) return net_fail(RZ_ERR_ARG, "rz_net_delta_reserve: n_games must be positive");
    if (n_games <= net->base_games) return RZ_OK;
    (void)hipDeviceSynchronize();
    if (!net->d_win) {
        std::vector<uint64_t> win(rzw::kEntries);
        rzw::window_table(win.data(), net->dev.BH, net->dev.BW);
        if (hipMalloc((void **)&net->d_win, win.size() * sizeof(uint64_t)) != hipSuccess) return net_fail(RZ_ERR_OOM, "hipMalloc failed (window table)");
        if (hipMemcpy(net->d_win, win.data(), win.size() * sizeof(uint64_t), hipMemcpyHostToDevice) != hipSuccess)
            return net_fail(RZ_ERR_HIP, "hipMemcpy failed (window table)");
    }
    if (net->d_base_hdr) (void)hipFree(net->d_base_hdr);
    if (net->d_base_recs) (void)hipFree(net->d_base_recs);
    if (net->d_base_ones) (void)hipFree(net->d_base_ones);
    net->d_base_ones = nullptr;
    net->d_base_hdr = nullptr;
    net->d_base_recs = nullptr;
    net->base_games = 0;
    const size_t hdr_bytes = (size_t)n_games * sizeof(dl::BaseHdr), rec_bytes = (size_t)n_games * 2 * dl::kBaseBytes;
    if (hipMalloc((void **)&net->d_base_hdr, hdr_bytes) != hipSuccess || hipMalloc((void **)&net->d_base_recs, rec_bytes) != hipSuccess ||
        hipMalloc((void **)&net->d_base_ones, (size_t)n_games) != hipSuccess)
        return net_fail(RZ_ERR_OOM, "hipMalloc failed (base cache)");
    if (hipMemset(net->d_base_ones, 1, (size_t)n_games) != hipSuccess) return net_fail(RZ_ERR_HIP, "hipMemset failed (base cache)");
    if (!net->d_delta_stats && hipMalloc((void **)&net->d_delta_stats, 8 * sizeof(unsigned)) != hipSuccess)
        return net_fail(RZ_ERR_OOM, "hipMalloc failed (delta counters)");
    if (hipMemset(net->d_base_hdr, 0, hdr_bytes) != hipSuccess || hipMemset(net->d_delta_stats, 0, 8 * sizeof(unsigned)) != hipSuccess)
        return net_fail(RZ_ERR_HIP, "hipMemset failed (base cache)");
    net->base_games = n_games;
    return RZ_OK;
}

int rz_net_delta_resident(rz_net *net, int32_t on) {
    if (!net) return net_fail(RZ_ERR_ARG, "net handle is NULL");
    net->delta_resident = on != 0;
    return RZ_OK;
}

int rz_net_delta_invalidate(rz_net *net, void *stream) {
    if (!net) return net_fail(RZ_ERR_ARG, "net handle is NULL");
    if (net->base_games > 0 &&
        hipMemsetAsync(net->d_base_hdr, 0, (size_t)net->base_games * sizeof(dl::BaseHdr), (hipStream_t)stream) != hipSuccess)
        return net_fail(RZ_ERR_HIP, "hipMemsetAsync failed (base cache)");
    return RZ_OK;
}

int rz_net_delta_bases(rz_net *net, const uint64_t *d_root_stones, const int32_t *d_root_to_move, int32_t n_games, void *stream) {
    int rc = net_ready(net, n_games);
    if (rc != RZ_OK) return rc;
    if (n_games == 0) return RZ_OK;
    if (!delta_covers(net)) return net_fail(RZ_ERR_ARG, "receptive-field evaluation: RZ_NET_SPLIT_F16 on boards of 11 .. 16 rows and columns");
    if (n_games > net->base_games) return net_fail(RZ_ERR_ARG, "more games than rz_net_delta_reserve()d");
    if (!d_root_stones || !d_root_to_move) return net_fail(RZ_ERR_ARG, "NULL device pointer");
    dl::DeltaArgs da{net->d_base_hdr, net->d_base_recs, net->d_base_ones, nullptr, nullptr, 1, (65536 + net->dev.BW - 1) / net->dev.BW};
    const DeferredOut none{nullptr, 0, nullptr, 0, nullptr, 0};
    dl::k_trunk_delta<false><<<dim3((unsigned)(2 * n_games)), dim3(256), 0, (hipStream_t)stream>>>(
        net->dev, LeafBits{d_root_stones, d_root_to_move, nullptr}, nullptr, 2 * n_games, none, da);
    if (hipGetLastError() != hipSuccess) return net_fail(RZ_ERR_HIP, "launch of k_trunk_delta (bases) failed");
    return RZ_OK;
}

int rz_net_delta_leaves(rz_net *net, const uint64_t *d_stones, const int32_t *d_to_move, const int32_t *d_last_cell, int32_t n_boards,
                        const int32_t *d_slot_of_board, const uint8_t *d_active, float *d_feat32, int32_t without_base, rz_value_head *out,
                        void *stream) {
    int rc = net_ready(net, n_boards);
    if (rc != RZ_OK) return rc;
    if (!delta_covers(net)) return net_fail(RZ_ERR_ARG, "receptive-field evaluation: RZ_NET_SPLIT_F16 on boards of 11 .. 16 rows and columns");
    if (without_base && n_boards > net->base_games && (rc = rz_net_delta_reserve(net, n_boards)) != RZ_OK) return rc;
    if (n_boards > net->base_games) return net_fail(RZ_ERR_ARG, "more boards than rz_net_delta_reserve()d games");
    if (d_slot_of_board && n_boards > net->store_boards) return net_fail(RZ_ERR_ARG, "batch larger than rz_net_deferred_reserve()d");
    if (n_boards > 0) {
        if (!d_stones || !d_to_move || !d_last_cell) return net_fail(RZ_ERR_ARG, "NULL device pointer");
        if (!d_slot_of_board && !d_feat32) return net_fail(RZ_ERR_ARG, "rz_net_delta_leaves: neither a store slot nor an f32 buffer to write to");
        const DeferredOut later{d_slot_of_board, (long long)net->store_tiles * net->dev.groups_act * 1024, net->d_valfeat, net->vf_groups * 4,
                                net->d_trace, net->store_slots};
        dl::DeltaArgs da{net->d_base_hdr, net->d_base_recs, d_active ? d_active : net->d_base_ones, d_feat32, net->d_delta_stats, without_base ? 2 : 0, (65536 + net->dev.BW - 1) / net->dev.BW};
        const dim3 grid((unsigned)n_boards);
// ... 217 lines not shown
```

### rlzero_amd/csrc/rz_tree.h

```cpp
#pragma once
#include <hip/hip_runtime.h>

#include <cmath>
#include <stdint.h>

#include "rlzero_hip.h"
#include "rz_trace.h"

#pragma clang fp contract(off)

namespace rzt {
namespace {

constexpr int kWave = 64;
constexpr int kWords = RZ_BOARD_WORDS;

struct Dev {
    int kind, BH, BW, S, A, n_row, n_games, score_mode, n_playout;
    int K;
    int path_stride, qcap;
    long long cap, pcap, logtab_n;
    double c_puct;
    int4 *R;
    float *P;
    int32_t *cur_arena, *top, *ptop, *nblk;
    uint64_t *root_stones;
    int32_t *root_to_move, *root_last;
    uint8_t *active;
    int32_t *path, *leaf_node, *leaf_depth, *leaf_fresh, *leaf_term;
    double *leaf_tval;
    uint64_t *leaf_stones;
    int32_t *leaf_to_move, *leaf_last;
    int32_t *queue;
    int32_t *err, *err_any, *reuse_drops;
    const double *logtab;
    int32_t *noise_ctr;
    uint64_t *noise_key;
    uint64_t noise_seed;
    int add_noise;
    int pend_cap;
    int32_t *pend, *pend_pb, *pend_ctr;
    uint64_t *pend_stones;
    unsigned long long *trace;
    uint64_t valid[kWords];
    int bw_rcp, n_rcp;
    uint64_t col0;
    const uint64_t *line_tab;
    int line_masks;
};

constexpr int kFirstCap = 4;
__device__ __forceinline__ int rec_k(const int4 &lo) { return lo.w & 0xffff; }
__device__ __forceinline__ int rec_cap(const int4 &lo) { return (int)((unsigned)lo.w >> 16); }
__device__ __forceinline__ int pack_kc(int k, int cap) { return k | (cap << 16); }
__device__ __forceinline__ double rec_w(const int4 &hi) { return __hiloint2double(hi.y, hi.x); }
__device__ __forceinline__ int4 make_hi(double w, int pb, float prior) {
    return make_int4(__double2loint(w), __double2hiint(w), pb, __float_as_int(prior));
}
__device__ __forceinline__ int4 *arena_records(const Dev &E, int g, int arena) {
    return E.R + 2 * (((long long)g * 2 + arena) * E.cap);
}
__device__ __forceinline__ float *arena_priors(const Dev &E, int g, int arena) {
    return E.P + ((long long)g * 2 + arena) * E.pcap;
}
__device__ __forceinline__ int32_t *rec_n(int4 *R, int slot) { return reinterpret_cast<int32_t *>(R + 2 * slot); }
__device__ __forceinline__ double *rec_wsum(int4 *R, int slot) { return reinterpret_cast<double *>(R + 2 * slot + 1); }
__device__ __forceinline__ int32_t *rec_pb(int4 *R, int slot) { return reinterpret_cast<int32_t *>(R + 2 * slot + 1) + 2; }

template <int W = kWords>
__device__ __forceinline__ uint64_t word_of(const uint64_t *a, int j) {
    if constexpr (W == 1) return a[0];
    if constexpr (W == 2) {
        const uint64_t m0 = j == 0 ? ~0ull : 0ull;
        return (a[0] & m0) | (a[1] & ~m0);
    }
    const uint64_t m0 = j == 0 ? ~0ull : 0ull, m1 = j == 1 ? ~0ull : 0ull, m2 = j == 2 ? ~0ull : 0ull,
                   m3 = j == 3 ? ~0ull : 0ull;
    return (a[0] & m0) | (a[1] & m1) | (a[2] & m2) | (a[3] & m3);
}
template <int W = kWords>
__device__ __forceinline__ bool test_bit(const uint64_t *a, int c) {
    return (word_of<W>(a, c >> 6) >> (c & 63)) & 1ull;
}
template <int W = kWords>
__device__ __forceinline__ void set_bit(uint64_t *a, int c) {
    const uint64_t m = 1ull << (c & 63);
    if constexpr (W == 1) {
        a[0] |= m;
    } else {
        const int j = c >> 6;
        a[0] |= (j == 0) ? m : 0ull;
        a[1] |= (j == 1) ? m : 0ull;
        if constexpr (W > 2) {
            a[2] |= (j == 2) ? m : 0ull;
            a[3] |= (j == 3) ? m : 0ull;
        }
    }
}
template <int W = kWords>
__device__ __forceinline__ int count_bits(const uint64_t *a) {
    int n = 0;
#pragma unroll
    for (int j = 0; j < W; ++j) n += __popcll(a[j]);
    return n;
}
template <int W = kWords>
__device__ __forceinline__ void load_board(const uint64_t *src, int g, uint64_t (&st)[2][kWords]) {
#pragma unroll
    for (int j = 0; j < kWords; ++j) {
        st[0][j] = j < W ? src[((long long)g * 2 + 0) * kWords + j] : 0ull;
        st[1][j] = j < W ? src[((long long)g * 2 + 1) * kWords + j] : 0ull;
    }
}
template <int W = kWords>
__device__ __forceinline__ void store_board(uint64_t *dst, int g, const uint64_t (&st)[2][kWords], int lane) {
    typedef unsigned long long u64x2 __attribute__((ext_vector_type(2)));
    if (lane < 2) {
        const bool c1 = lane == 1;
        u64x2 lo, hi;
        lo[0] = c1 ? st[1][0] : st[0][0];
        lo[1] = W >= 2 ? (c1 ? st[1][1] : st[0][1]) : 0ull;
        hi[0] = W > 2 ? (c1 ? st[1][2] : st[0][2]) : 0ull;
        hi[1] = W > 2 ? (c1 ? st[1][3] : st[0][3]) : 0ull;
        u64x2 *p = reinterpret_cast<u64x2 *>(dst + ((long long)g * 2 + lane) * kWords);
        p[0] = lo;
        p[1] = hi;
    }
}

struct Legal {
    int k;
    unsigned long long cols;
// ... 554 lines not shown
        if (fresh) break;
        lo = clo;
        hi = chi;
    }
    if constexpr (Hook::kOn) {
        hook->tick(3, node);
        hook->depth = depth;
        if (lane == 0) {
            RootPre *pre = hook->pre;
            pre->lo = st_lo;
            pre->r = st_r;
            pre->scan = st_scan;
            pre->arena = arena;
        }
    }
    if (lane == 0 && top != top0) E.top[g] = top;
    if (VL && fresh != 1 && lane == 0) {
        *rec_n(R, node) = lo.x + 1;
        *rec_wsum(R, node) = rec_w(hi) - 1.0;
    }

    int term = 0;
    double tval = 0.0;
    {
        int winner = -1;
        if (depth == 0) {
            if (line_anywhere<W>(st[0], S, E.BH, E.BW, E.n_row, lane, E.bw_rcp)) winner = 0;
            else if (line_anywhere<W>(st[1], S, E.BH, E.BW, E.n_row, lane, E.bw_rcp)) winner = 1;
        } else {
            const int mover = to_move ^ 1;
            if (line_through<W>(mover == 0 ? st[0] : st[1], last, E.BH, E.BW, E.n_row, lane, E.bw_rcp, E.n_rcp, window, window_hi, E.line_masks != 0)) winner = mover;
        }
        if (winner >= 0) {
            term = 2;
            tval = (winner == to_move) ? 1.0 : -1.0;
        } else if (nst == S) {
            term = 1;
            tval = 0.0;
        }
    }
    if (lane == 0) {
        E.leaf_node[gk] = node;
        E.leaf_depth[gk] = depth;
        E.leaf_fresh[gk] = fresh;
        E.leaf_term[gk] = term;
        E.leaf_tval[gk] = tval;
        E.leaf_to_move[gk] = to_move;
        E.leaf_last[gk] = last;
    }
    store_board<W>(E.leaf_stones, gk, st, lane);
    if (lds_leaf != nullptr) {
        store_board<W>(lds_leaf, 0, st, lane);
        if (lane == 0) {
            reinterpret_cast<int *>(lds_leaf + 2 * kWords)[0] = to_move;
            reinterpret_cast<int *>(lds_leaf + 2 * kWords)[1] = last;
        }
    }
    if constexpr (Hook::kOn) hook->tick(4, term);
    if (obs != nullptr)
        write_obs(obs + (long long)gk * 4 * S, to_move == 0 ? st[0] : st[1],
                  to_move == 0 ? st[1] : st[0], last, nst, S, lane);
}

typedef rz_raw_heads RawHeads;
typedef rz_value_head ValueHead;
constexpr int kDefWaves = 4;

template <typename VT, bool PROBS = false, bool RAW = false, bool VL = false, bool DEF = false, int W = kWords>
__device__ __forceinline__ void expand_backup_body(const Dev &E, const float *logp, const VT *value, int g,
                                                   int lane, RawHeads rh = RawHeads(), int j = 0, ValueHead vh = ValueHead(),
                                                   float (*part)[kWave] = nullptr) {
    const int gk = VL ? g * E.K + j : g;
    const int slot = DEF ? E.pend[g] : 0;
    const bool act = E.active[g] != 0;
    const int arena = E.cur_arena[g];
    const int depth = E.leaf_depth[gk];
    const int fresh = E.leaf_fresh[gk];
    const int term = E.leaf_term[gk];
    const double leaf_tval = E.leaf_tval[gk];
    const int ptop = E.ptop[g];
    const int nblk = E.nblk[g];
    const int top_now = E.top[g];
    const int noise_ctr = E.noise_ctr[g];
    const int32_t *path = E.path + (long long)gk * E.path_stride;
    const int path_lane = path[lane < E.path_stride ? lane : 0];
    uint64_t st[2][kWords];
    load_board<W>(E.leaf_stones, gk, st);
    float lse = 0.0f, raw_value = 0.0f;
    float x[kWords] = {0.f, 0.f, 0.f, 0.f};
    if (RAW) {
        const float *r = rh.raw + (size_t)gk * rh.ld;
        const float *hp = rh.hid + (size_t)gk * 64 + lane;
        const float w2 = rh.w2[lane], b2 = rh.b2[0];
        float hid = hp[0];
        float mx = -INFINITY;
        if (rh.n_parts == 4) {
            const long long rs = rh.raw_part_stride, hs = rh.hid_part_stride;
            const float act_scale = rh.act_scale[0], val_scale = rh.val_scale[0];
            float part[kWords][4], bias[kWords];
#pragma unroll
            for (int i = 0; i < kWords; ++i) {
                const int j = lane + 64 * i;
                const bool in = j < E.A;
#pragma unroll
                for (int q = 0; q < 4; ++q) part[i][q] = in ? r[j + q * rs] : 0.0f;
                bias[i] = in ? rh.act_bias[j] : 0.0f;
            }
            const float h1 = hp[hs], h2 = hp[2 * hs], h3 = hp[3 * hs], hb = rh.val_bias[lane];
#pragma unroll
            for (int i = 0; i < kWords; ++i) {
                const float sum4 = ((part[i][0] + part[i][1]) + part[i][2]) + part[i][3];
                x[i] = lane + 64 * i < E.A ? fmaf(sum4, act_scale, bias[i]) : -INFINITY;
                mx = fmaxf(mx, x[i]);
            }
            hid = fmaxf(fmaf(((hid + h1) + h2) + h3, val_scale, hb), 0.0f);
        } else {
#pragma unroll
            for (int i = 0; i < kWords; ++i) {
                const int j = lane + 64 * i;
                x[i] = j < E.A ? r[j] : -INFINITY;
                mx = fmaxf(mx, x[i]);
            }
        }
        mx = wave_max(mx, lane);
        float sum = 0.0f;
#pragma unroll
        for (int i = 0; i < kWords; ++i) sum += (lane + 64 * i < E.A) ? expf(x[i] - mx) : 0.0f;
        sum = wave_sum(sum, lane);
        lse = mx + logf(sum);
        float h = hid * w2;
        h = wave_sum(h, lane);
        raw_value = tanhf(h + b2);
    }
    float def_value = 0.0f;
    if (DEF) {
        const float b1 = vh.b1[lane], w2 = vh.w2[lane], b2 = vh.b2[0];
        __syncthreads();
        float hid = part[0][lane];
#pragma unroll
        for (int q = 1; q < kDefWaves; ++q) hid += part[q][lane];
        hid = fmaxf(hid + b1, 0.0f);
        def_value = tanhf(wave_sum(hid * w2, lane) + b2);
    }
    if (!act) return;
    int4 *R = arena_records(E, g, arena);
    float *P = arena_priors(E, g, arena);

    const double v = term ? leaf_tval : (DEF ? (double)def_value : RAW ? (double)raw_value : (double)value[gk]);
    if (DEF && slot >= E.pend_cap) {
        flag(E, g, RZ_FLAG_INTERNAL, lane);
        return;
    }
    const long long rec = DEF ? (long long)slot * E.n_games + g : 0;

    int new_fc = -1, new_nv = 0, new_k = 0, new_cap = 0, new_pb = -1;
    bool expand_now = !term && fresh != 2;
    if (VL && expand_now) {
        const int leaf = __shfl(path_lane, depth < kWave ? depth : 0);
        expand_now = rec_k(R[2 * (depth < kWave ? leaf : path[depth])]) == 0;
    }
    if (expand_now) {
        uint64_t occ[kWords];
#pragma unroll
        for (int j = 0; j < kWords; ++j) occ[j] = st[0][j] | st[1][j];
        const Legal L = legal_of<W>(E, occ, lane);
        const int k = L.k;
        const bool dense = !DEF && E.score_mode == RZ_SCORE_PUCT;
        const int top = dense ? top_now : 0;
        if ((long long)ptop + k > E.pcap || nblk >= E.qcap) {
            flag(E, g, RZ_FLAG_BLOCKS_FULL, lane);
        } else if (dense && (long long)top + k > E.cap) {
            flag(E, g, RZ_FLAG_ARENA_FULL, lane);
        } else {
            new_pb = ptop;
            new_k = k;
            if (dense) {
                new_fc = top;
                new_nv = k;
                new_cap = k;
            }
            if (lane == 0) {
                E.ptop[g] = ptop + k;
                E.nblk[g] = nblk + 1;
                if (dense) E.top[g] = top + k;
            }
            if (DEF) {
                if (lane == 0) {
                    E.pend_pb[rec] = ptop;
                    E.pend_ctr[rec] = noise_ctr;
                    if (E.add_noise) E.noise_ctr[g] = noise_ctr + 1;
                }
                store_board<W>(E.pend_stones, (int)rec, st, lane);
            }
            const float uniform = 1.0f / (float)k;
            if (!DEF) {
            int ranks[kWords];
            int before = 0;
#pragma unroll
            for (int j = 0; j < kWords; ++j) ranks[j] = lane_action_rank(E, occ, L, j, lane, before);
            float noise[kWords] = {0.f, 0.f, 0.f, 0.f};
            float noise_sum = 1.0f;
            if (E.add_noise) {
                const int ctr = noise_ctr;
                const uint64_t key = mix64(mix64(E.noise_key[g]) ^ (uint64_t)ctr);
                float local = 0.0f;
#pragma unroll
                for (int j = 0; j < kWords; ++j)
                    if (ranks[j] >= 0) {
                        noise[j] = gamma03(hash32((uint32_t)key ^ (uint32_t)(key >> 32)) + 0x9E3779B9u * (uint32_t)(64 * j + lane + 1));
                        local += noise[j];
                    }
                local = wave_sum(local, lane);
                noise_sum = local > 0.0f ? local : 1.0f;
                if (lane == 0) E.noise_ctr[g] = ctr + 1;
            }
#pragma unroll
            for (int j = 0; j < kWords; ++j) {
                const int r = ranks[j];
                if (r < 0) continue;
                const int a = 64 * j + lane;
                float prior = uniform;
                if (RAW) prior = expf(x[j] - lse);
                else if (logp) prior = PROBS ? logp[(long long)gk * E.A + a] : expf(logp[(long long)gk * E.A + a]);
                if (E.add_noise) prior = 0.75f * prior + 0.25f * (noise[j] / noise_sum);
                P[ptop + r] = prior;
                if (dense) {
                    R[2 * (top + r)] = make_int4(0, -1, 0, 0);
                    R[2 * (top + r) + 1] = make_hi(0.0, -1, prior);
                }
            }
            }
        }
    }
    if (DEF && lane == 0) {
        if (new_pb < 0) E.pend_pb[rec] = -1;
        E.pend[g] = slot + 1;
    }

    for (int d = lane; d <= depth; d += kWave) {
        const int node = d == lane ? path_lane : path[d];
        const double x = ((depth - d) & 1) ? v : -v;
        if (VL) {
            if (d == depth && new_k > 0) {
                const int4 m = R[2 * node];
                R[2 * node] = make_int4(m.x, new_fc, new_nv, pack_kc(new_k, new_cap));
                *rec_pb(R, node) = new_pb;
            }
            *rec_wsum(R, node) += x + 1.0;
        } else if (d == depth) {
            if (fresh == 1) {
                R[2 * node] = make_int4(1, new_fc, new_nv, pack_kc(new_k, new_cap));
                R[2 * node + 1] = make_hi(0.0 + x, new_pb, 0.0f);
            } else {
                const int4 m = R[2 * node];
                R[2 * node] = (new_k > 0) ? make_int4(m.x + 1, new_fc, new_nv, pack_kc(new_k, new_cap))
                                          : make_int4(m.x + 1, m.y, m.z, m.w);
                *rec_wsum(R, node) += x;
                if (new_k > 0) *rec_pb(R, node) = new_pb;
            }
        } else {
            *rec_n(R, node) += 1;
            *rec_wsum(R, node) += x;
        }
    }
}

template <int PER>
__device__ __forceinline__ void value_quarter_def(const ValueHead &vh, int gk, int lane, int q, float (*part)[kWave]) {
    typedef float vec4 __attribute__((ext_vector_type(4)));
    typedef const __attribute__((address_space(4))) vec4 *uniform_row;
    const vec4 *w = reinterpret_cast<const vec4 *>(vh.w1t) + (size_t)q * 2 * PER * kWave + lane;
    const uniform_row f = (uniform_row)(reinterpret_cast<const vec4 *>(vh.valfeat + (size_t)gk * vh.ld) + q * 2 * PER);
// ... 50 lines not shown
```

### rlzero_amd/engine.py

```python
import ctypes
import functools
import os

import numpy as np

from . import _hip
from . import route as _route
from ._hip import HipError, check
from .route import compact_grid_board

WORDS = _hip.BOARD_WORDS


def _ptr(t):
    return None if t is None else ctypes.c_void_p(t.data_ptr())


_DEVICE_INDEX = {}


def _current_stream(torch, device):
    raw = getattr(torch._C, '_cuda_getCurrentRawStream', None)
    if raw is None:
        return ctypes.c_void_p(torch.cuda.current_stream(device).cuda_stream)
# ... 101 lines not shown
        return self

    def route(self, **how):
        return _route.decide(self.rows, self.cols, self.algo, self._split_ok, self.heads_algo, **how)

    def reads_positions(self):
        return not self.route(environ={}).needs_planes

    def trunk_leaves(self, eng):
        n = eng.n_leaves
        if n > self.max_boards:
            self.reserve(n)
        stones, to_move, last = eng.leaf_buffers()
        check(self.lib.rz_net_trunk_leaves(self.handle, stones, to_move, last, n, self._stream()), 'rz_net_trunk_leaves')

    def supports_deferred(self):
        return self.route(environ={}).deferred

    def deferred_bytes_per_slot(self, n_boards):
        tiles = (n_boards + 63) // 64 * 2
        k_steps = (4 * self.n_cells + 15) // 16
        n_pad = (self.n_actions + 31) // 32 * 32
        return tiles * k_steps * 2048 + tiles * 32 * n_pad * 4

    def deferred_reserve(self, n_boards, slots):
        have = self._store
        check(self.lib.rz_net_deferred_reserve(self.handle, int(n_boards), int(slots)), 'rz_net_deferred_reserve')
        moved = int(n_boards) > have[0] or int(slots) > have[1]
        if moved:
            self._store = (max(have[0], int(n_boards)), max(have[1], int(slots)))
        return moved and have != (0, 0)

    def trunk_leaves_deferred(self, eng):
        stones, to_move, last = eng.leaf_buffers()
        out = _hip.RzValueHead()
        check(self.lib.rz_net_trunk_leaves_deferred(self.handle, stones, to_move, last, eng.n_leaves, eng.deferred_slot_ptr(),
                                                    ctypes.byref(out), self._stream()), 'rz_net_trunk_leaves_deferred')
        return out

    def supports_delta(self):
        return self.route(environ={}).delta

    def delta_reserve(self, n_games):
        check(self.lib.rz_net_delta_reserve(self.handle, int(n_games)), 'rz_net_delta_reserve')
        self._delta_games = max(self._delta_games, int(n_games))

    def delta_invalidate(self):
        check(self.lib.rz_net_delta_invalidate(self.handle, self._stream()), 'rz_net_delta_invalidate')

    def delta_bases(self, stones, to_move, n_games):
        check(self.lib.rz_net_delta_bases(self.handle, stones, to_move, int(n_games), self._stream()), 'rz_net_delta_bases')

    def delta_leaves(self, stones, to_move, last, n, slot_of=None, active=None, feat32=None, without_base=False, want_head=True):
        out = _hip.RzValueHead() if want_head else None
        check(self.lib.rz_net_delta_leaves(self.handle, stones, to_move, last, int(n), slot_of, active, feat32, 1 if without_base else 0,
                                           ctypes.byref(out) if out is not None else None, self._stream()), 'rz_net_delta_leaves')
        return out

    def delta_bases_engine(self, eng):
        check(self.lib.rz_net_delta_bases_engine(self.handle, eng.handle, self._stream()), 'rz_net_delta_bases_engine')

    def delta_step(self, eng):
        out = _hip.RzValueHead()
        check(self.lib.rz_net_delta_step(self.handle, eng.handle, ctypes.byref(out), self._stream()), 'rz_net_delta_step')
        return out

    def delta_trunk_engine(self, eng):
        check(self.lib.rz_net_delta_trunk_engine(self.handle, eng.handle, self._stream()), 'rz_net_delta_trunk_engine')

    def delta_stats(self, reset=False):
        out = (ctypes.c_uint32 * 8)()
        check(self.lib.rz_net_delta_stats(self.handle, out, 1 if reset else 0), 'rz_net_delta_stats')
        ghz = (256.0 * out[6]) / (10.0 * out[7]) if out[7] else None
        return {'delta': int(out[0]), 'no_base': int(out[1]), 'tiles3': int(out[2]), 'cells': int(out[3]), 'tiles2': int(out[4]),
                'prescans': int(out[5]), 'resident_sclk_ghz': ghz}

    def compact_resident(self):
        return self.route().compact_resident

    def supports_resident(self):
        return self.route(environ={}).resident

    def search_resident(self, eng, n_sims, select_first=False):
        check(self.lib.rz_net_search_resident(self.handle, eng.handle, int(n_sims), 1 if select_first else 0, self._stream()), 'rz_net_search_resident')

    def deferred_gemm(self, n_boards, n_slots):
        out = _hip.RzDeferredLogits()
        check(self.lib.rz_net_deferred_gemm(self.handle, int(n_boards), int(n_slots), ctypes.byref(out), self._stream()),
              'rz_net_deferred_gemm')
        return out

    def deferred_gemm_rows(self, kept):
        out = _hip.RzDeferredLogits()
        check(self.lib.rz_net_deferred_gemm_rows(self.handle, ctypes.byref(kept), ctypes.byref(out), self._stream()), 'rz_net_deferred_gemm_rows')
        return out

    def range_info(self):
        out = (ctypes.c_float * 8)()
        check(self.lib.rz_net_range_info(self.handle, out), 'rz_net_range_info')
        return {'bounds': (out[0], out[1], out[2]), 'scales': (out[3], out[4], out[5]), 'split_ok': bool(out[6])}

    def check_flags(self):
        flags = ctypes.c_uint32(0)
        check(self.lib.rz_net_error_flags(self.handle, ctypes.byref(flags)), 'rz_net_error_flags')
        if flags.value & _hip.NET_FLAG_F16_RANGE:
            raise HipError("an input outside [0, 1] drove an activation out of the range of the split-f16 trunk: "
                           "use set_algo('direct') for such inputs")
        return self

    def set_heads_algo(self, algo):
        code = {'auto': _hip.NET_HEADS_AUTO, 'f32': _hip.NET_HEADS_F32, 'split32': _hip.NET_HEADS_SPLIT_32,
                'split64': _hip.NET_HEADS_SPLIT_64, 'parts': _hip.NET_HEADS_SPLIT_PARTS, 'in_trunk': _hip.NET_HEADS_IN_TRUNK}[algo]
        check(self.lib.rz_net_set_heads_algo(self.handle, code), 'rz_net_set_heads_algo')
        self.heads_algo = algo
        return self

    def set_max_workgroups(self, n):
        check(self.lib.rz_net_set_max_workgroups(self.handle, int(n)), 'rz_net_set_max_workgroups')
        return self

    def load_state_dict(self, state_dict):
        check_state_dict(state_dict, self.rows, self.cols, self.n_actions)
        arrays = []
        for name in PARAM_ORDER:
            t = state_dict[name]
            a = t.detach().to('cpu', self.torch.float32).contiguous().numpy() if hasattr(t, 'detach') \
                else np.ascontiguousarray(t, dtype=np.float32)
            arrays.append(a)
        ptrs = (ctypes.c_void_p * 16)(*[a.ctypes.data for a in arrays])
        check(self.lib.rz_net_load(self.handle, ptrs, 16), 'rz_net_load')
        self.generation += 1
        self.reserve(max(self._want, self.max_boards))
        self._split_ok = self.range_info()['split_ok']
        return self

    def route_state(self):
        r = self.route(environ={})
        return not r.needs_planes, r.deferred, r.delta, r.resident

    def reserve(self, max_boards):
        check(self.lib.rz_net_reserve(self.handle, int(max_boards)), 'rz_net_reserve')
        self.max_boards = max(self.max_boards, int(max_boards))

    def forward(self, obs, logp=None, value=None):
        t = self.torch
        n = obs.shape[0]
        if n > self.max_boards:
            self.reserve(n)
        if logp is None:
            logp = t.empty((n, self.n_actions), dtype=t.float32, device=self.device)
        if value is None:
            value = t.empty(n, dtype=t.float32, device=self.device)
        st = ctypes.c_void_p(t.cuda.current_stream(self.device).cuda_stream)
        check(self.lib.rz_net_forward(self.handle, _ptr(obs), n, _ptr(logp), _ptr(value), st), 'rz_net_forward')
        return logp, value

    def _stream(self):
        return _current_stream(self.torch, self.device)

    def trunk_internal(self, obs):
        n = obs.shape[0]
        if n > self.max_boards:
            self.reserve(n)
        check(self.lib.rz_net_trunk(self.handle, _ptr(obs), n, None, self._stream()), 'rz_net_trunk')

    def heads_gemm(self, n):
        out = _hip.RzRawHeads()
        check(self.lib.rz_net_heads_gemm(self.handle, int(n), ctypes.byref(out), self._stream()), 'rz_net_heads_gemm')
        return out

    def heads(self, n, logp, value):
        check(self.lib.rz_net_heads(self.handle, int(n), _ptr(logp), _ptr(value), self._stream()), 'rz_net_heads')
        return logp, value
# ... 173 lines not shown
        eng.value64.copy_(torch.from_numpy(values))
        eng.logp.copy_(torch.from_numpy(probs))
        return eng.logp, eng.value64


def bits_to_int(words):
    out = 0
    for j, w in enumerate(words):
        out |= int(w) << (64 * j)
    return out


def int_to_bits(x):
    return [(x >> (64 * j)) & 0xFFFFFFFFFFFFFFFF for j in range(WORDS)]


class MCTSEngine(object):

    def __init__(self, board_size, n_in_row, n_games=1, n_playout=1000, c_puct=5.0,
                 device='cuda:0', pool_factor=2.0, score_mode='uct_ref', add_noise=False, noise_seed=0,
                 game='gomoku', sims_in_flight=1, in_flight_impl='level_sync'):
        import torch
        self.lib = _hip.load()
        self.torch = torch
        dev = torch.device(device)
        if dev.type != 'cuda' or not torch.cuda.is_available():
            raise HipError('the MCTS engine needs an MI355X (device=%r, cuda available=%s); '
                           'there is no CPU fallback' % (device, torch.cuda.is_available()))
        self.device = torch.device('cuda', dev.index if dev.index is not None else torch.cuda.current_device())
        self.game = game
        if game == 'connect4':
            rows, cols = (6, 7) if board_size is None else (int(board_size[0]), int(board_size[1]))
            self.board_size = (rows, cols)
        else:
            rows = cols = int(board_size)
            self.board_size = rows
        self.rows, self.cols, self.n_in_row = rows, cols, int(n_in_row)
        self.n_cells = rows * cols
        self.n_actions = cols if game == 'connect4' else self.n_cells
        self.n_games, self.n_playout, self.c_puct = int(n_games), int(n_playout), float(c_puct)
        self.score_mode = {'uct_ref': _hip.SCORE_UCT_REF, 'puct': _hip.SCORE_PUCT}[score_mode] \
            if isinstance(score_mode, str) else int(score_mode)
        self.add_noise = bool(add_noise)
        self.sims_in_flight = max(1, int(sims_in_flight))
        self.n_leaves = self.n_games * self.sims_in_flight
        cfg = _hip.RzConfig(abi_version=_hip.ABI_VERSION,
                            game_kind=_hip.GAME_CONNECT4 if game == 'connect4' else _hip.GAME_GOMOKU,
                            board_size=rows if game != 'connect4' else 0,
                            n_in_row=self.n_in_row, n_games=self.n_games, n_playout=self.n_playout,
                            score_mode=self.score_mode, add_noise=1 if add_noise else 0, c_puct=self.c_puct,
                            pool_factor=float(pool_factor), device=self.device.index,
                            noise_seed=int(noise_seed) & 0x7FFFFFFF, board_height=rows, board_width=cols,
                            sims_in_flight=self.sims_in_flight,
                            in_flight_impl={'level_sync': 0, 'sequential': 1}[in_flight_impl])
        handle = ctypes.c_void_p()
        check(self.lib.rz_create(ctypes.byref(cfg), ctypes.byref(handle)), 'rz_create')
        self.handle = handle
        G, S, GL = self.n_games, self.n_actions, self.n_leaves
        kw = dict(device=self.device)
        self.obs = torch.zeros((GL, 4, rows, cols), dtype=torch.float32, **kw)
        self.logp = torch.zeros((GL, S), dtype=torch.float32, **kw)
        self.value = torch.zeros(GL, dtype=torch.float32, **kw)
        self.value64 = torch.zeros(GL, dtype=torch.float64, **kw)
        self.visits = torch.zeros((G, S), dtype=torch.int32, **kw)
        self.wsum = torch.zeros((G, S), dtype=torch.float64, **kw)
        self.priors = torch.zeros((G, S), dtype=torch.float32, **kw)
        self.root_n = torch.zeros(G, dtype=torch.int32, **kw)
        self.root_w = torch.zeros(G, dtype=torch.float64, **kw)
        self.moves = torch.zeros(G, dtype=torch.int32, **kw)
        self.winner = torch.zeros(G, dtype=torch.int32, **kw)
        self.ended = torch.zeros(G, dtype=torch.uint8, **kw)
        self.stones = torch.zeros((G, 2, WORDS), dtype=torch.int64, **kw)
        self.to_move = torch.zeros(G, dtype=torch.int32, **kw)
        self.last_move = torch.zeros(G, dtype=torch.int32, **kw)
        self.terminal = torch.zeros(G, dtype=torch.int32, **kw)
        self.mask = torch.zeros(G, dtype=torch.uint8, **kw)
        self.active_dev = torch.ones(G, dtype=torch.uint8, **kw)
        self.noise_keys = torch.zeros(G, dtype=torch.int64, **kw)
        self.noise_mask = torch.zeros(G, dtype=torch.uint8, **kw)
        self.active_host = np.ones(G, dtype=np.uint8)
        self._graphs = {}
        self.roots_epoch = 0
        self._def_ev, self._def_pending, self._def_slots, self._def_slot_ptr, self._capturing = None, 0, 0, None, False
        self.deferred_max_bytes = 32 << 30
        self._playouts = None
        self.flush_kept = os.environ.get('RZ_FLUSH_KEPT', '1') != '0'

    def stream(self):
        return _current_stream(self.torch, self.device)

    def close(self):
        if getattr(self, 'handle', None):
            self._graphs = {}
            self.lib.rz_destroy(self.handle)
            self.handle = None

    def __del__(self):
        try:
            self.close()
        except Exception:
            pass

    def stats(self):
        out = _hip.RzStats()
        check(self.lib.rz_get_stats(self.handle, ctypes.byref(out)), 'rz_get_stats')
        return out

    def check(self):
        st = self.stats()
        if st.error_flags & ~_hip.FLAG_REUSE_DROPPED:
            names = [n for bit, n in _hip.FLAG_NAMES.items() if st.error_flags & bit]
            raise HipError('engine error flags 0x%x (%s), first bad game %d, arena %d/%d slots' %
                           (st.error_flags, ', '.join(names), st.first_bad_game,
                            st.max_slots_used, st.arena_slots))
        return st

    def poll_errors(self):
        flags, drops = ctypes.c_int32(0), ctypes.c_int32(0)
        check(self.lib.rz_poll_errors(self.handle, ctypes.byref(flags), ctypes.byref(drops), self.stream()), 'rz_poll_errors')
        if flags.value & ~_hip.FLAG_REUSE_DROPPED:
            self.check()
        return drops.value

    def set_roots(self, stones, to_move, last_move, mask=None, reset_trees=False):
        t = self.torch
        self.flush_deferred()
        G, nb = self.n_games, 2 * WORDS * 8
        if getattr(self, '_roots_io', None) is None:
            host = t.empty(G * (nb + 8), dtype=t.uint8, pin_memory=True)
            dev = t.empty(G * (nb + 8), dtype=t.uint8, device=self.device)
            hn = host.numpy()
            self._roots_io = (host, dev, hn[:G * nb].view(np.uint64).reshape(G, 2, WORDS), hn[G * nb:G * nb + 4 * G].view(np.int32),
                              hn[G * nb + 4 * G:].view(np.int32), t.cuda.Event())
        host, dev, h_stones, h_to_move, h_last, done = self._roots_io
        done.synchronize()
        h_stones[...] = np.asarray(stones, dtype=np.uint64).reshape(G, 2, WORDS)
        h_to_move[:] = to_move
        h_last[:] = last_move
        dev.copy_(host, non_blocking=True)
        done.record(t.cuda.current_stream(self.device))
        mptr = None
        if mask is not None:
            self.mask.copy_(t.from_numpy(np.ascontiguousarray(mask, dtype=np.uint8)))
            mptr = _ptr(self.mask)
        base = dev.data_ptr()
        check(self.lib.rz_set_roots(self.handle, ctypes.c_void_p(base), ctypes.c_void_p(base + G * nb), ctypes.c_void_p(base + G * nb + 4 * G),
                                    mptr, 1 if reset_trees else 0, self.stream()), 'rz_set_roots')
        self.roots_epoch += 1

    def reset_games(self, mask=None):
        G = self.n_games
        self.set_roots(np.zeros((G, 2, WORDS), np.uint64), np.zeros(G, np.int32),
                       np.full(G, -1, np.int32), mask=mask, reset_trees=True)

    def get_roots(self):
        check(self.lib.rz_get_roots(self.handle, _ptr(self.stones), _ptr(self.to_move),
                                    _ptr(self.last_move), self.stream()), 'rz_get_roots')
        return (self.stones.cpu().numpy().view(np.uint64), self.to_move.cpu().numpy(),
                self.last_move.cpu().numpy())

    def set_active(self, active):
        self._play_active = None
        self.active_host = np.ascontiguousarray(active, dtype=np.uint8).copy()
        self.active_dev.copy_(self.torch.from_numpy(self.active_host))
        check(self.lib.rz_set_active(self.handle, _ptr(self.active_dev), self.stream()), 'rz_set_active')

    def set_noise_keys(self, keys=None, mask=None):
        t = self.torch
        kptr = mptr = None
# ... 46 lines not shown
            check(self.lib.rz_expand_backup_probs(self.handle, _ptr(logp), _ptr(value), self.stream()),
                  'rz_expand_backup_probs')
        elif value.dtype == self.torch.float64:
            check(self.lib.rz_expand_backup_f64(self.handle, _ptr(logp), _ptr(value), self.stream()),
                  'rz_expand_backup_f64')
        else:
            check(self.lib.rz_expand_backup(self.handle, _ptr(logp), _ptr(value), self.stream()),
                  'rz_expand_backup')

    def _in_flight(self, k_backup, k_select):
        check(self.lib.rz_set_in_flight(self.handle, int(k_backup), int(k_select)), 'rz_set_in_flight')

    def sim_chunk(self, evaluator, n, r=None):
        if n <= 0:
            return
        K = self.sims_in_flight
        r = self._ask(evaluator)[0] if r is None else r
        if not r.resident and (self._playouts is not None or getattr(self, 'play_cap_on', False)):
            raise ValueError('per-game simulation counts (set_playouts, play_set_cap) need the resident search: this evaluator\'s '
                             'route for this engine has none')
        if not r.deferred:
            self.flush_deferred()
        if isinstance(evaluator, HostEvaluator):
            if K > 1:
                raise HipError('host evaluators are not available with sims_in_flight > 1')
            if getattr(self, 'play_log', None) is not None and getattr(self, '_play_on', False):
                self._play_active = (self.play_state()[2] == 1).astype(np.uint8)
            for _ in range(n):
                self.sim_step(evaluator)
            return
        lib, h = self.lib, self.handle
        begin = getattr(evaluator, 'begin_chunk', None)
        if begin is not None:
            begin()
        if r.deferred:
            return self._sim_chunk_deferred(evaluator, n, r.resident)
        obs = _ptr(self.obs) if r.needs_planes else None
        steps = -(-n // K)
        counts = [min(K, n - i * K) for i in range(steps)] + [0]
        if K > 1:
            self._in_flight(0, counts[0])
        check(lib.rz_select_step(h, obs, self.stream()), 'rz_select_step')
        fused = getattr(evaluator, 'fused_heads', False)
        for i in range(steps):
            if K > 1 and (i == 0 or counts[i + 1] != K or counts[i] != K):
                self._in_flight(counts[i], counts[i + 1])
            if fused:
                heads = evaluator.raw_heads(self)
                if i + 1 < steps:
                    check(lib.rz_tree_step_raw(h, ctypes.byref(heads), obs, self.stream()), 'rz_tree_step_raw')
                else:
                    check(lib.rz_expand_backup_raw(h, ctypes.byref(heads), self.stream()), 'rz_expand_backup_raw')
                continue
            logp, value = evaluator(self)
            if value.dtype != self.torch.float32:
                raise HipError('device evaluators must return float32 values')
            if i + 1 < steps:
                check(lib.rz_tree_step(h, _ptr(logp), _ptr(value), obs, self.stream()), 'rz_tree_step')
            else:
                check(lib.rz_expand_backup(h, _ptr(logp), _ptr(value), self.stream()), 'rz_expand_backup')
        if K > 1:
            self._in_flight(K, K)

    def deferred_slot_ptr(self):
        if self._def_slot_ptr is None:
            p = ctypes.c_void_p()
            check(self.lib.rz_deferred_slots(self.handle, ctypes.byref(p)), 'rz_deferred_slots')
            self._def_slot_ptr = p
        return self._def_slot_ptr

    def _deferred_begin(self, evaluator, n):
        owner = getattr(evaluator, '_def_owner', None)
        owner = owner() if owner is not None else None
        if owner is not None and owner is not self:
            self.torch.cuda.synchronize(self.device)
            owner.flush_deferred()
            self.torch.cuda.synchronize(self.device)
        if owner is not self:
            import weakref
            evaluator._def_owner = weakref.ref(self)
        if self._def_ev is not evaluator:
            self.flush_deferred()
            hip = evaluator.hip
            per_slot = hip.deferred_bytes_per_slot(self.n_leaves) + 80 * self.n_games
            slots = int(max(16, min(max(self.n_playout, 16), self.deferred_max_bytes // per_slot)))
            if self._capturing:
                raise HipError('the deferred-priors store must be reserved before a hipGraph capture (warm_graph does that)')
            if slots > self._def_slots:
                check(self.lib.rz_deferred_reserve(self.handle, slots), 'rz_deferred_reserve')
                self._def_slots = slots
                self._def_slot_ptr = None
                self._drop_graphs('rz_deferred_reserve moved the pending records')
            if hip.deferred_reserve(self.n_leaves, self._def_slots):
                for other in list(getattr(evaluator, '_deferring', ())) + [self]:
                    other._drop_graphs('rz_net_deferred_reserve moved the feature store')
            self._def_ev = evaluator
            refs = getattr(evaluator, '_deferring', None)
            if refs is None:
                import weakref
                refs = evaluator._deferring = weakref.WeakSet()
            refs.add(self)
        if self._capturing:
            return n
        if self._def_pending + min(n, self._def_slots) > self._def_slots:
            self.flush_deferred()
        return min(n, self._def_slots - self._def_pending)

    def _drop_graphs(self, why):
        if self._graphs or getattr(self, '_move_graph', None) is not None:
            self._graphs = {}
            self._move_graph = None
            self._graphs_dropped = why

    def _sim_chunk_deferred(self, evaluator, n, resident):
        lib, h = self.lib, self.handle
        while n > 0:
            m = self._deferred_begin(evaluator, n)
            if m < n and (self._playouts is not None or getattr(self, 'play_cap_on', False)):
                raise ValueError('per-game simulation counts need the whole search in one launch: %d simulations, %d store slots' % (n, m))
            if resident:
                evaluator.search_resident(self, m, True)
            else:
                check(lib.rz_select_step(h, None, self.stream()), 'rz_select_step')
                for i in range(m):
                    head = evaluator.deferred_trunk(self)
                    if i + 1 < m:
                        check(lib.rz_tree_step_deferred(h, ctypes.byref(head), self.stream()), 'rz_tree_step_deferred')
                    else:
                        check(lib.rz_expand_backup_deferred(h, ctypes.byref(head), self.stream()), 'rz_expand_backup_deferred')
            if not self._capturing:
                self._def_pending += m
                self._def_stream = self.torch.cuda.current_stream(self.device)
            n -= m

    def flush_deferred(self, move=False):
        if self._def_pending <= 0 or self._def_ev is None:
            return
        cur, then = self.torch.cuda.current_stream(self.device), getattr(self, '_def_stream', None)
        if then is not None and then != cur:
            cur.wait_stream(then)
        if move:
            self._enqueue_move_flush(self._def_ev.hip, self._def_pending)
        else:
            logits = self._def_ev.hip.deferred_gemm(self.n_leaves, self._def_pending)
            check(self.lib.rz_deferred_flush(self.handle, ctypes.byref(logits), self._def_pending, self.stream()), 'rz_deferred_flush')
        if then is not None and then != cur:
            then.wait_stream(cur)
        self._def_pending = 0

    def _enqueue_move_flush(self, hip, n_slots):
        lib, h, st = self.lib, self.handle, self.stream()
        if self.flush_kept:
            kept = _hip.RzKeptRows()
            check(lib.rz_deferred_keep(h, ctypes.byref(kept), st), 'rz_deferred_keep')
            logits = hip.deferred_gemm_rows(kept)
            check(lib.rz_deferred_flush_kept(h, ctypes.byref(logits), st), 'rz_deferred_flush_kept')
        else:
            logits = hip.deferred_gemm(self.n_leaves, n_slots)
            check(lib.rz_deferred_flush(h, ctypes.byref(logits), n_slots, st), 'rz_deferred_flush')

    def flush_kept_stats(self, reset=False):
        out = (ctypes.c_uint64 * 2)()
        check(self.lib.rz_deferred_keep_stats(self.handle, out, 1 if reset else 0), 'rz_deferred_keep_stats')
        return int(out[0]), int(out[1])

    def _whole_steps(self, n_sims):
        K = self.sims_in_flight
        return max(K, int(n_sims) - int(n_sims) % K)

    def graph_chunk(self, sims_per_graph):
        per = max(1, int(sims_per_graph))
        K = self.sims_in_flight
        if K == 1:
            return per
        full = max(1, self.n_playout // K)
        steps = max(s for s in range(1, min(per, full) + 1) if full % s == 0)
        return K * steps

    def simulate(self, evaluator, n_sims=None, use_graph=False, sims_per_graph=8):
        n = self.n_playout if n_sims is None else int(n_sims)
        r, _, prepare = self._ask(evaluator)
        prepare()
        per = self._whole_steps(sims_per_graph)
        if not use_graph or isinstance(evaluator, HostEvaluator) or r.resident or per > n:
            self.sim_chunk(evaluator, n, r)
            return
        key = (id(evaluator), per)
        if key not in self._graphs:
            why = getattr(self, '_graphs_dropped', None)
            raise HipError('call warm_graph(evaluator, %d) before simulate(use_graph=True)%s' % (per, ' (the graphs were dropped: %s)' % why if why else ''))
        graph = self._graphs[key][0]
        full, rest = divmod(n, per)
        for _ in range(full):
            if r.deferred:
                if self._deferred_begin(evaluator, per) < per:
                    raise HipError('the deferred-priors store (%d slots) is smaller than a graph of %d steps' % (self._def_slots, per))
                self._def_pending += per
                self._def_stream = self.torch.cuda.current_stream(self.device)
            graph.replay()
        self.sim_chunk(evaluator, rest, r)

    def set_playouts(self, counts, longest_first=True, order=None):
        t = self.torch
        if counts is None:
            check(self.lib.rz_set_playouts(self.handle, None, None, self.stream()), 'rz_set_playouts')
            self._playouts = None
            return
        if self.sims_in_flight != 1 or self.score_mode != _hip.SCORE_UCT_REF:
            raise ValueError('per-game simulation counts need the resident search (score_mode uct_ref, sims_in_flight 1)')
        c = np.asarray(counts)
        if c.shape != (self.n_games, ) or not np.issubdtype(c.dtype, np.integer) or (c < 1).any() or (c > 0x7FFFFFFF).any():
            raise ValueError('counts: %d integers >= 1, one per game' % self.n_games)
        c = c.astype(np.int32)
        if order is not None:
            o = np.asarray(order, dtype=np.int64)
            if o.shape != c.shape or (np.sort(o) != np.arange(self.n_games)).any():
                raise ValueError('order: a permutation of the %d games' % self.n_games)
        else:
            o = np.argsort(-c.astype(np.int64), kind='stable') if longest_first else None
        dc = t.from_numpy(c).to(self.device)
        do = None if o is None else t.from_numpy(o.astype(np.int32)).to(self.device)
        check(self.lib.rz_set_playouts(self.handle, _ptr(dc), None if do is None else _ptr(do), self.stream()), 'rz_set_playouts')
        self._playouts = (dc, do)

    def playouts(self):
        counts, order = np.zeros(self.n_games, np.int32), np.zeros(self.n_games, np.int32)
        source = ctypes.c_int32(0)
        check(self.lib.rz_playouts_read(self.handle, ctypes.c_void_p(counts.ctypes.data), ctypes.c_void_p(order.ctypes.data),
                                        ctypes.byref(source)), 'rz_playouts_read')
        src = source.value
        if src == 0:
            return None, None, None
        return counts, (order if src & 4 else None), 'host' if src & 3 == 1 else 'device'

    def warm_graph(self, evaluator, per):
# ... 91 lines not shown
        h_in[0].numpy()[:] = keep_moves
        h_in[1].numpy()[:] = step_moves
        d_in.copy_(h_in, non_blocking=True)
        check(self.lib.rz_advance_roots(self.handle, _ptr(d_in[0]), self.stream()), 'rz_advance_roots')
        check(self.lib.rz_step_games(self.handle, _ptr(d_in[1]), _ptr(self.winner), _ptr(self.ended), self.stream()), 'rz_step_games')
        self.roots_epoch += 1
        h_win.copy_(self.winner, non_blocking=True)
        h_end.copy_(self.ended, non_blocking=True)
        done.record(t.cuda.current_stream(self.device))
        done.synchronize()
        return h_win.numpy().copy(), h_end.numpy().copy()

    def step(self, moves):
        self.moves.copy_(self.torch.from_numpy(np.ascontiguousarray(moves, dtype=np.int32)))
        check(self.lib.rz_step_games(self.handle, _ptr(self.moves), _ptr(self.winner),
                                     _ptr(self.ended), self.stream()), 'rz_step_games')
        self.roots_epoch += 1
        return self.winner.cpu().numpy(), self.ended.cpu().numpy()

    def play_attach(self, seed, temperature, queue_ids, queue_ctl, ring_steps=64, stall_margin=0.0):
        t = self.torch
        self.flush_deferred()
        t.cuda.synchronize(self.device)
        shape = (int(ring_steps), self.n_games, _hip.PLAY_RECORD_WORDS + self.n_actions)
        self.play_log_on_host = os.environ.get('RZ_PLAY_DEVICE_LOG') != '1'
        if self.play_log_on_host:
            self.play_log = t.zeros(shape, dtype=t.int32).pin_memory()
        else:
            self.play_log = t.zeros(shape, dtype=t.int32, device=self.device)
        self._play_queue = (queue_ids, queue_ctl)
        def attach():
            cfg = _hip.RzPlayConfig(seed=int(seed) & 0xFFFFFFFFFFFFFFFF, temperature=float(temperature), stall_margin=float(stall_margin),
                                    d_queue_ids=queue_ids.data_ptr(), d_queue_ctl=queue_ctl.data_ptr(), d_log=self.play_log.data_ptr(),
                                    ring_steps=int(ring_steps), reserved=0)
            check(self.lib.rz_play_attach(self.handle, ctypes.byref(cfg)), 'rz_play_attach')
        try:
            attach()
        except HipError as exc:
            if not self.play_log_on_host or 'cannot address' not in str(exc):
                raise
            self.play_log_on_host = False
            self.play_log = t.zeros(shape, dtype=t.int32, device=self.device)
            attach()
        self.play_steps = 0
        self.play_resign_on = False
        self.play_cap_on = False
        self.play_match_on = False
        self._play_on, self._play_active = True, None
        self.active_host[:] = 0
        return self.play_log

    def play_move(self):
        st = self.stream()
        check(self.lib.rz_play_draw(self.handle, st), 'rz_play_draw')
        self.flush_deferred(move=True)
        check(self.lib.rz_play_apply(self.handle, st), 'rz_play_apply')
        self.roots_epoch += 1
        row = self.play_steps % self.play_log.shape[0]
        self.play_steps += 1
        return row

    def warm_move_graph(self, evaluator):
        t = self.torch
        r, owner, _ = self._ask(evaluator)
        if not r.resident or getattr(self, 'play_log', None) is None:
            return None
        if getattr(self, 'play_match_on', False):
            raise HipError('warm_move_graph: a match (play_set_match) searches with two evaluators per move; its moves are enqueued eagerly')
        n = self.n_playout
        if self._playouts is not None:
            raise HipError('warm_move_graph: clear set_playouts first (the graph would hold the host\'s counts, not play_set_cap\'s)')
        self.flush_deferred()
        if self._deferred_begin(evaluator, n) < n or self._def_slots < n:
            return None
        if r.resident_delta:
            owner.reserve_bases(self)
        hip, lib, h = evaluator.hip, self.lib, self.handle
        t.cuda.synchronize(self.device)
        graph = t.cuda.CUDAGraph()
        self._capturing = True
        try:
            with t.cuda.graph(graph):
                st = self.stream()
                evaluator.search_resident(self, n, True)
                check(lib.rz_play_draw(h, st), 'rz_play_draw')
                self._enqueue_move_flush(hip, n)
                check(lib.rz_play_apply(h, st), 'rz_play_apply')
        finally:
            self._capturing = False
        self._move_graph_ev = evaluator
        self._move_graph = graph
        self._note_capture(owner or evaluator)
        return graph

    def play_move_replay(self, graph):
        if graph is not getattr(self, '_move_graph', None):
            raise HipError('this whole-move graph was dropped (%s): call warm_move_graph again' % getattr(self, '_graphs_dropped', 'a buffer it addresses moved'))
        if self._def_pending > 0:
            self.flush_deferred()
        graph.replay()
        self.roots_epoch += 1
        row = self.play_steps % self.play_log.shape[0]
        self.play_steps += 1
        return row

    def play_refill(self):
        self.flush_deferred()
        check(self.lib.rz_play_apply(self.handle, self.stream()), 'rz_play_apply')
        self.roots_epoch += 1
        self.play_steps += 1

    def play_set_resign(self, threshold, disabled_frac):
        check(self.lib.rz_play_set_resign(self.handle, float(threshold), float(disabled_frac), self.stream()), 'rz_play_set_resign')
        self.play_resign_on = True

    def play_set_cap(self, n_fast, p_full):
        p_full = float(p_full)
        if self.sims_in_flight != 1 or self.score_mode != _hip.SCORE_UCT_REF:
            raise ValueError('the playout cap needs the resident search (score_mode uct_ref, sims_in_flight 1)')
        if not np.isnan(p_full) and not (0.0 < p_full <= 1.0 and 1 <= int(n_fast) <= self.n_playout):
            raise ValueError('playout cap: n_fast %r in 1 .. n_playout = %d, p_full %r in (0, 1]' % (n_fast, self.n_playout, p_full))
        check(self.lib.rz_play_set_cap(self.handle, int(n_fast), p_full, self.stream()), 'rz_play_set_cap')
        self.play_cap_on = True

    def play_set_cap_order(self, longest_first):
        check(self.lib.rz_play_set_cap_order(self.handle, 1 if longest_first else 0), 'rz_play_set_cap_order')

    def play_set_match(self, openings):
        t = self.torch
        if openings is None:
            check(self.lib.rz_play_set_match(self.handle, None, None, None, 0, self.stream()), 'rz_play_set_match')
            self.play_match_on, self._play_openings = False, None
            return
        stones, to_move, last = openings
        stones = np.ascontiguousarray(stones, dtype=np.uint64)
        n = stones.shape[0]
        if n < 1 or stones.shape != (n, 2, WORDS):
            raise ValueError('openings: stones uint64 [n >= 1, 2, %d]' % WORDS)
        dev = [t.from_numpy(stones.view(np.int64)).to(self.device)] + \
              [t.from_numpy(np.ascontiguousarray(x, dtype=np.int32).reshape(n)).to(self.device) for x in (to_move, last)]
        check(self.lib.rz_play_set_match(self.handle, _ptr(dev[0]), _ptr(dev[1]), _ptr(dev[2]), n, self.stream()), 'rz_play_set_match')
        self._play_openings = dev
        self.play_match_on = True

    def play_side(self, side):
        check(self.lib.rz_play_side(self.handle, int(side), self.stream()), 'rz_play_side')

    def active_flags(self):
        out = np.zeros(self.n_games, np.uint8)
        check(self.lib.rz_active_read(self.handle, ctypes.c_void_p(out.ctypes.data)), 'rz_active_read')
        return out

    def play_resolve(self, slot, move):
        check(self.lib.rz_play_resolve(self.handle, int(slot), int(move), self.stream()), 'rz_play_resolve')

    def play_stop(self):
        self.flush_deferred()
        check(self.lib.rz_play_stop(self.handle, self.stream()), 'rz_play_stop')
        self._play_active = None

    def play_state(self):
        gid = np.zeros(self.n_games, np.int64)
        ply = np.zeros(self.n_games, np.int32)
        state = np.zeros(self.n_games, np.int32)
        steps = ctypes.c_int64(0)
        check(self.lib.rz_play_state(self.handle, ctypes.c_void_p(gid.ctypes.data), ctypes.c_void_p(ply.ctypes.data),
                                     ctypes.c_void_p(state.ctypes.data), ctypes.byref(steps)), 'rz_play_state')
        return gid, ply, state, steps.value

# ... 82 lines not shown
```

### rlzero_amd/route.py

```python
import os
from collections import namedtuple

from ._hip import SCORE_UCT_REF

SPLIT_TRUNKS = ('split_f16', 'split_f16_tiles', 'split_f16_fp8')
EVERY_BOARD_SPLIT_TRUNKS = ('split_f16', 'split_f16_tiles')
DELTA_TRUNKS = ('split_f16', )
RESIDENT_TRUNKS = ('split_f16', 'split_f16_fp8')


def rows_kernel_board(rows, cols):
    return 11 <= rows <= 16 and 11 <= cols <= 16


def tile_resident_board(rows, cols):
    return rows <= 10 and cols <= 10


def compact_grid_board(rows, cols, environ=None):
    if cols > 7 or cols < 1:
        return False
    tile_rows = min(32 // cols, 16)
    tiles = (rows + tile_rows - 1) // tile_rows
    return tiles <= 2 and tiles * tile_rows + 2 <= 15 and _on(environ, 'RZ_NET_COMPACT')


def _on(environ, name):
    return (os.environ if environ is None else environ).get(name, '1') != '0'


def fc_in_trunk_pays(rows, cols, n_actions):
    cells = rows * cols
    return rows <= 10 and (n_actions * 4 * cells + 64 * 2 * cells) * 4 <= 40 * 1024


Route = namedtuple('Route', 'needs_planes deferred delta delta_three_launch resident resident_delta compact_resident resident_per_cu')
Route.__doc__ = """How the leaves of a search are evaluated:
needs_planes        the trunk reads float observation planes (otherwise the engine's leaf bitboards: no plane is written)
deferred            trunk -> tree step, the policy half in one batch later (otherwise trunk -> FC GEMM -> tree step)
delta               the receptive-field trunk against cached bases of the root is usable
delta_three_launch  ... and the three-launch step runs on it
resident            a whole search is ONE launch, one workgroup per game
resident_delta      the resident search could run the receptive-field trunk (k_delta_res): two games per CU
compact_resident    the net's resident search runs on the compact LDS grid: two games per CU
resident_per_cu     resident workgroups a CU holds (2: a launch takes any number of games, in rounds beyond 2 x CUs)"""


def decide(rows, cols, algo='split_f16', split_ok=True, heads_algo='auto', use_positions=True, deferred_priors=True, delta_trunk=True,
           resident_search=True, score_mode=SCORE_UCT_REF, in_flight=1, n_games=0, n_cus=0, same_board=True, environ=None):
    split = split_ok and algo in SPLIT_TRUNKS
    one_sim = in_flight == 1
    deferred = bool(split and deferred_priors and use_positions and one_sim and score_mode in (SCORE_UCT_REF, 'uct_ref'))
    rows_board = rows_kernel_board(rows, cols)
    delta = bool(split and delta_trunk and same_board and rows_board and algo in DELTA_TRUNKS and _on(environ, 'RZ_NET_DELTA'))
    resident_delta = delta and _on(environ, 'RZ_NET_DELTA_RESIDENT')
    net_resident = split and algo in RESIDENT_TRUNKS and (rows_board or tile_resident_board(rows, cols))
    compact = net_resident and not rows_board and compact_grid_board(rows, cols, environ)
    per_cu = 2 if (resident_delta or (compact and same_board)) else 1
    return Route(not (use_positions and split), deferred, delta, bool(delta and use_positions and one_sim and not deferred and heads_algo != 'f32'),
                 bool(resident_search and deferred and net_resident and (per_cu >= 2 or n_games <= n_cus)), resident_delta, compact, per_cu)
```

Baseline: 22.89 million.

## Compute policy channels on demand only for kept rows in resident delta search

```diff
diff --git a/include/rlzero_hip.h b/include/rlzero_hip.h
--- a/include/rlzero_hip.h
+++ b/include/rlzero_hip.h
@@ -7,7 +7,7 @@
 extern "C" {
 #endif
 
-#define RZ_ABI_VERSION 31
+#define RZ_ABI_VERSION 32
 #define RZ_MAX_BOARD_SIZE 16
 #define RZ_BOARD_WORDS 4
 #define RZ_MAX_IN_FLIGHT 16
@@ -168,6 +168,8 @@
 } rz_kept_rows;
 int rz_deferred_keep(rz_engine *e, rz_kept_rows *out, void *stream);
 int rz_deferred_flush_kept(rz_engine *e, const rz_deferred_logits *logits, void *stream);
+int rz_deferred_keep_all(rz_engine *e, rz_kept_rows *out, void *stream);
+int rz_deferred_flush_rows(rz_engine *e, const rz_deferred_logits *logits, void *stream);
 int rz_deferred_keep_stats(rz_engine *e, uint64_t *h_out2, int32_t reset);
 
 int rz_root_visits(rz_engine *e, int32_t *d_visits, void *stream);
@@ -272,6 +274,8 @@
 int rz_net_delta_trunk_engine(rz_net *net, rz_engine *engine, void *stream);
 int rz_net_delta_stats(rz_net *net, uint32_t *h_out8, int32_t reset);
 int rz_net_search_resident(rz_net *net, rz_engine *engine, int32_t n_sims, int32_t select_first, void *stream);
+int rz_net_search_resident_values(rz_net *net, rz_engine *engine, int32_t n_sims, int32_t select_first, void *stream);
+int rz_net_policy_rows(rz_net *net, rz_engine *engine, const rz_kept_rows *kept, void *stream);
 int rz_net_heads(rz_net *net, int32_t n_boards, float *d_logp, float *d_value, void *stream);
 int rz_net_heads_gemm(rz_net *net, int32_t n_boards, rz_raw_heads *out, void *stream);
 int rz_net_forward(rz_net *net, const float *d_obs, int32_t n_boards, float *d_logp,
diff --git a/profiles/microbench/delta_resident_phases.py b/profiles/microbench/delta_resident_phases.py
--- a/profiles/microbench/delta_resident_phases.py
+++ b/profiles/microbench/delta_resident_phases.py
@@ -12,7 +12,11 @@
          (9, 'bar + conv3 + heads'), (10, 'bar'), (11, 'features'), (12, 'bar'), (16, 'value layer'), (17, 'expand + backup'),
          (2, 'sel: root record'), (8, 'sel: root scan / answer'), (13, 'sel: level-0 cell'), (14, 'sel: deeper levels'), (15, 'sel: terminal test + leaf stores'),
          (18, 'selection (rest: hand-over)'), (19, 'wave 1: pre-scan'), (20, 'wave 1: wait behind it')]
-sizes = [int(a) for a in sys.argv[1:]] or [1, 256, 512]
+VALUES = '--values' in sys.argv[1:]
+if VALUES:
+    import rlzero_amd.route as _R
+    _R.policy_on_demand = lambda *a, **k: True
+sizes = [int(a) for a in sys.argv[1:] if a != '--values'] or [1, 256, 512]
 for games in sizes:
     torch.manual_seed(0)
     net = PolicyValueNet(15).to('cuda:0')
@@ -31,6 +35,7 @@
     a, b = torch.cuda.Event(enable_timing=True), torch.cuda.Event(enable_timing=True)
     ev.hip.delta_stats(reset=True)
     a.record(); eng.sim_chunk(ev, sims); b.record(); torch.cuda.synchronize()
+    assert (eng.search_launches[True] > 0) == VALUES and (eng.search_launches[False] > 0) != VALUES
     st = ev.hip.delta_stats()
     out = (ctypes.c_longlong * 24)()
     assert lib.rz_net_debug_profile(out) == 0
diff --git a/rlzero_amd/_hip.py b/rlzero_amd/_hip.py
--- a/rlzero_amd/_hip.py
+++ b/rlzero_amd/_hip.py
@@ -3,7 +3,7 @@
 from ctypes import (POINTER, Structure, c_char_p, c_double, c_int, c_int32, c_int64, c_uint32, c_uint64,
                     c_void_p)
 
-ABI_VERSION = 31
+ABI_VERSION = 32
 BOARD_WORDS = 4
 MAX_BOARD_SIZE = 16
 MAX_IN_FLIGHT = 16
@@ -123,6 +123,8 @@
     'rz_deferred_flush': (c_int, [P, POINTER(RzDeferredLogits), c_int32, P]),
     'rz_deferred_keep': (c_int, [P, POINTER(RzKeptRows), P]),
     'rz_deferred_flush_kept': (c_int, [P, POINTER(RzDeferredLogits), P]),
+    'rz_deferred_keep_all': (c_int, [P, POINTER(RzKeptRows), P]),
+    'rz_deferred_flush_rows': (c_int, [P, POINTER(RzDeferredLogits), P]),
     'rz_deferred_keep_stats': (c_int, [P, POINTER(c_uint64), c_int32]),
     'rz_root_visits': (c_int, [P, P, P]),
     'rz_root_wsum': (c_int, [P, P, P]),
@@ -167,6 +169,8 @@
     'rz_net_trunk_leaves_deferred': (c_int, [P, P, P, P, c_int32, P, POINTER(RzValueHead), P]),
     'rz_net_deferred_gemm': (c_int, [P, c_int32, c_int32, POINTER(RzDeferredLogits), P]),
     'rz_net_deferred_gemm_rows': (c_int, [P, POINTER(RzKeptRows), POINTER(RzDeferredLogits), P]),
+    'rz_net_search_resident_values': (c_int, [P, P, c_int32, c_int32, P]),
+    'rz_net_policy_rows': (c_int, [P, P, POINTER(RzKeptRows), P]),
     'rz_net_search_resident': (c_int, [P, P, c_int32, c_int32, P]),
     'rz_net_delta_reserve': (c_int, [P, c_int32]),
     'rz_net_delta_invalidate': (c_int, [P, P]),
diff --git a/rlzero_amd/csrc/rz_delta.h b/rlzero_amd/csrc/rz_delta.h
--- a/rlzero_amd/csrc/rz_delta.h
+++ b/rlzero_amd/csrc/rz_delta.h
@@ -179,17 +179,17 @@
     }
 }
 
-template <int T>
-__device__ __forceinline__ void reduce_scatter(const float (&vals)[6 * T], float (&out)[6 * T / 4]) {
-    float r1[3 * T];
-#pragma unroll
-    for (int i = 0; i < 3 * T; ++i) {
-        const auto sw = __builtin_amdgcn_permlane16_swap(__float_as_uint(vals[i]), __float_as_uint(vals[3 * T + i]), false, false);
+template <int T, int O = 6>
+__device__ __forceinline__ void reduce_scatter(const float (&vals)[O * T], float (&out)[O * T / 4]) {
+    float r1[O * T / 2];
+#pragma unroll
+    for (int i = 0; i < O * T / 2; ++i) {
+        const auto sw = __builtin_amdgcn_permlane16_swap(__float_as_uint(vals[i]), __float_as_uint(vals[O * T / 2 + i]), false, false);
         r1[i] = __uint_as_float(sw[0]) + __uint_as_float(sw[1]);
     }
 #pragma unroll
-    for (int i = 0; i < 3 * T / 2; ++i) {
-        const auto sw = __builtin_amdgcn_permlane32_swap(__float_as_uint(r1[i]), __float_as_uint(r1[3 * T / 2 + i]), false, false);
+    for (int i = 0; i < O * T / 4; ++i) {
+        const auto sw = __builtin_amdgcn_permlane32_swap(__float_as_uint(r1[i]), __float_as_uint(r1[O * T / 4 + i]), false, false);
         out[i] = __uint_as_float(sw[0]) + __uint_as_float(sw[1]);
     }
 }
@@ -218,12 +218,13 @@
     }
 }
 
-template <int NT>
+template <int NT, int OLO = 0, int OHI = 6>
 __device__ __forceinline__ void conv3_tiles(lds_u32 map2, const uint16_t *list3, const void *wts, int lane, int wave, bool sync,
                                             const char *headw, float k3, float *shares) {
-    constexpr int T = NT <= 4 ? 4 : 8;
+    constexpr int T = NT <= 4 ? 4 : 8, O = OHI - OLO;
+    static_assert(OLO % 2 == 0 && OHI % 2 == 0 && 0 <= OLO && OLO < OHI && OHI <= 6, "pairs of outputs");
     const int n = lane & 15, g = lane >> 4;
-    float vals[6 * T];
+    float vals[O * T];
     {
         f32x4 acc[2][NT];
         conv3_g<NT>(map2, list3, wts, lane, sync, acc);
@@ -245,22 +246,22 @@
                     for (int j = 0; j < 4; ++j) {
                         const float hv = fmaxf(fmaf(acc[m][t < NT ? t : 0][j], k3, b3r[m][j]), 0.0f);
 #pragma unroll
-                        for (int o2 = 0; o2 < 3; ++o2) {
+                        for (int o2 = OLO / 2; o2 < OHI / 2; ++o2) {
                             const int e = 6 * j + 2 * o2;
                             v2[o2] = __builtin_elementwise_fma(f32x2{hwr[m][e >> 2][e & 3], hwr[m][e >> 2][(e & 3) + 1]}, f32x2{hv, hv}, v2[o2]);
                         }
                     }
             }
 #pragma unroll
-            for (int o = 0; o < 6; ++o) vals[t * 6 + o] = v2[o >> 1][o & 1];
-        }
-    }
-    float mine[6 * T / 4];
-    reduce_scatter<T>(vals, mine);
+            for (int o = OLO; o < OHI; ++o) vals[t * O + o - OLO] = v2[o >> 1][o & 1];
+        }
+    }
+    float mine[O * T / 4];
+    reduce_scatter<T, O>(vals, mine);
     const int t0 = (T / 2) * (g & 1) + (T / 4) * (g >> 1);
 #pragma unroll
-    for (int i = 0; i < 6 * T / 4; ++i)
-        if (t0 + i / 6 < NT) shares[((t0 + i / 6) * 4 + wave) * 96 + (i % 6) * 16 + n] = mine[i];
+    for (int i = 0; i < O * T / 4; ++i)
+        if (t0 + i / O < NT) shares[((t0 + i / O) * 4 + wave) * 96 + (OLO + i % O) * 16 + n] = mine[i];
 }
 
 struct Leaf {
@@ -317,7 +318,7 @@
     return ((uint64_t)(unsigned)__builtin_amdgcn_readfirstlane((int)(v >> 32)) << 32) | (unsigned)__builtin_amdgcn_readfirstlane((int)v);
 }
 
-template <bool SETS>
+template <bool SETS, int OLO = 0, int OHI = 6>
 __device__ __forceinline__ int delta_passes(const NetDev &nd, const DeltaArgs &da, char *lds, int tid0, int wave, const Leaf &leaf, const Layers &ly,
                                             f32x4 headv, bool &use_delta, Prof &prof) {
     char *in0 = lds, *c1 = lds + kOffC1, *c2 = lds + kOffC2, *zrec = lds + kOffZero, *headw = lds + kOffHead;
@@ -375,7 +376,7 @@
         {
             const int ov = pass < 0 && is_cell && !f[2] ? (int)kBaseV + tid * 4 : kOutside;
 #pragma unroll
-            for (int o = 0; o < 6; ++o) bv[o] = __builtin_bit_cast(float, __builtin_amdgcn_raw_buffer_load_b32(b_rsrc, ov + o * kCells * 4, 0, 0));
+            for (int o = OLO; o < OHI; ++o) bv[o] = __builtin_bit_cast(float, __builtin_amdgcn_raw_buffer_load_b32(b_rsrc, ov + o * kCells * 4, 0, 0));
         }
         sp::f16x8 a1[3][2];
         f32x4 bias1[4];
@@ -534,15 +535,15 @@
             const int first = nt3 <= 6 ? nt3 : 4;
             switch (first) {
                 case 0: __syncthreads(); break;
-                case 1: conv3_tiles<1>(m2, list3, t3p, lane, wave, true, headw, k3, shares); break;
-                case 2: conv3_tiles<2>(m2, list3, t3p, lane, wave, true, headw, k3, shares); break;
-                case 3: conv3_tiles<3>(m2, list3, t3p, lane, wave, true, headw, k3, shares); break;
-                case 4: conv3_tiles<4>(m2, list3, t3p, lane, wave, true, headw, k3, shares); break;
-                case 5: conv3_tiles<5>(m2, list3, t3p, lane, wave, true, headw, k3, shares); break;
-                default: conv3_tiles<6>(m2, list3, t3p, lane, wave, true, headw, k3, shares); break;
-            }
-            if (nt3 == 7) conv3_tiles<3>(m2, list3 + 64, t3p, lane, wave, false, headw, k3, shares + 4 * 4 * 96);
-            else if (nt3 >= 8) conv3_tiles<4>(m2, list3 + 64, t3p, lane, wave, false, headw, k3, shares + 4 * 4 * 96);
+                case 1: conv3_tiles<1, OLO, OHI>(m2, list3, t3p, lane, wave, true, headw, k3, shares); break;
+                case 2: conv3_tiles<2, OLO, OHI>(m2, list3, t3p, lane, wave, true, headw, k3, shares); break;
+                case 3: conv3_tiles<3, OLO, OHI>(m2, list3, t3p, lane, wave, true, headw, k3, shares); break;
+                case 4: conv3_tiles<4, OLO, OHI>(m2, list3, t3p, lane, wave, true, headw, k3, shares); break;
+                case 5: conv3_tiles<5, OLO, OHI>(m2, list3, t3p, lane, wave, true, headw, k3, shares); break;
+                default: conv3_tiles<6, OLO, OHI>(m2, list3, t3p, lane, wave, true, headw, k3, shares); break;
+            }
+            if (nt3 == 7) conv3_tiles<3, OLO, OHI>(m2, list3 + 64, t3p, lane, wave, false, headw, k3, shares + 4 * 4 * 96);
+            else if (nt3 >= 8) conv3_tiles<4, OLO, OHI>(m2, list3 + 64, t3p, lane, wave, false, headw, k3, shares + 4 * 4 * 96);
         }
         NET_TICK(9);
         __syncthreads();
@@ -557,7 +558,7 @@
             const float *share = shares + (rank[2] >> 4) * 4 * 96 + (rank[2] & 15);
             float *basev = mode == 1 ? reinterpret_cast<float *>(const_cast<char *>(base) + kBaseV) : nullptr;
 #pragma unroll
-            for (int o = 0; o < 6; ++o) {
+            for (int o = OLO; o < OHI; ++o) {
                 float v;
                 if (f[2]) {
                     float s = share[o * 16];
@@ -845,6 +846,7 @@
 }
 
 constexpr int kResVrow = 512;
+template <bool POL>
 __global__ __launch_bounds__(256, 2) void k_delta_res(NetDev nd, _Float16 *__restrict__ store16, DeferredOut later, DeltaArgs da, ResArgs<true> res) {
     __shared__ __attribute__((aligned(16))) char lds[kLdsBytes];
     __shared__ float res_vrow[kResVrow];
@@ -946,13 +948,13 @@
         for (int i = 0; i < kMaxD; ++i) leaf.dys[i] = leaf.dxs[i] = -100;
         leaf.base = da.recs + ((size_t)game * 2 + parity) * kBaseBytes;
         leaf.cell_planes = planes_of(ls, tid_s, tm, has_last, lc, nst);
-        leaf.dst16 = slot0 + sim < later.n_slots ? store16 + (size_t)(slot0 + sim) * later.slot_halfs + (size_t)(game >> 5) * nd.groups_act * 1024 + (game & 31) * 16 : nullptr;
+        leaf.dst16 = POL && slot0 + sim < later.n_slots ? store16 + (size_t)(slot0 + sim) * later.slot_halfs + (size_t)(game >> 5) * nd.groups_act * 1024 + (game & 31) * 16 : nullptr;
         leaf.vdst = res_vrow;
         leaf.dst32 = nullptr;
         leaf.deferred = true;
         leaf.store_head = sim == 0;
         NET_TICK(0);
-        const int n_tiles = delta_passes<true>(nd, da, lds, tid_s, wave, leaf, ly, headv, use_delta, prof);
+        const int n_tiles = delta_passes<true, POL ? 0 : 4, 6>(nd, da, lds, tid_s, wave, leaf, ly, headv, use_delta, prof);
         tiles_total += n_tiles & 0xffff;
         tiles2_total += n_tiles >> 16;
         deltas += use_delta ? 1 : 0;
@@ -1024,4 +1026,78 @@
 #endif
 }
 
-}
+struct PolicyRows {
+    const int32_t *rows, *count;
+    const uint64_t *stones;
+    const int32_t *lw;
+    int n_games, n_slots;
+    long long slot_halfs;
+};
+__global__ __launch_bounds__(256, 2) void k_trunk_policy_rows(NetDev nd, _Float16 *__restrict__ store16, DeltaArgs da, PolicyRows pr) {
+    __shared__ __attribute__((aligned(16))) char lds[kLdsBytes];
+    const int tid0 = threadIdx.x, wave = __builtin_amdgcn_readfirstlane(tid0 >> 6);
+    const int BW = nd.BW;
+    Prof prof;
+#ifdef RZ_NET_PROFILE
+    for (int i = 0; i < 24; ++i) prof.acc[i] = 0;
+    prof.t = __builtin_readcyclecounter();
+#endif
+    Layers ly;
+    ly.t2p = reinterpret_cast<const char *>(nd.t2) + (size_t)wave * rt::Geo<32>::steps * 2 * 1024;
+    ly.t3p = reinterpret_cast<const char *>(nd.t3) + (size_t)(2 * wave) * rt::Geo<64>::steps * 2 * 1024;
+    f32x4 headv = tid0 < 192 ? reinterpret_cast<const f32x4 *>(nd.whp)[tid0] : reinterpret_cast<const f32x4 *>(nd.b3)[(tid0 - 192) & 31];
+    {
+        const float *bh = nd.bh + (tid0 == 225 ? 4 : 0);
+        const f32x4 hbv = {bh[0], bh[1], tid0 == 225 ? 0.0f : bh[2], tid0 == 225 ? 0.0f : bh[3]};
+        headv = (tid0 == 224 || tid0 == 225) ? hbv : headv;
+    }
+    ly.k1 = nd.s_inv[2], ly.k2 = nd.s_inv[0], ly.k3 = nd.s_inv[1];
+    ly.act1 = nd.s_inv[5], ly.act2 = nd.s_inv[6], ly.act3 = nd.s_inv[7];
+    const int n_rows = pr.count[0];
+    {
+        const f32x4 zero = {0.f, 0.f, 0.f, 0.f};
+        f32x4 *z = reinterpret_cast<f32x4 *>(lds);
+        for (int i = tid0; i < sp::kInPieceBytes / 16; i += 256) z[i] = zero;
+        if (tid0 < P2 / 16) reinterpret_cast<f32x4 *>(lds + kOffZero)[tid0] = zero;
+        init_maps(lds, tid0);
+    }
+    __syncthreads();
+    bool first = true;
+    for (int i = blockIdx.x; i < n_rows; i += gridDim.x) {
+        int tid_r = tid0;
+        asm volatile("" : "+v"(tid_r));
+        const int rec = pr.rows[i];
+        const int game = rec % pr.n_games, slot = rec / pr.n_games;
+        const uint64_t *sb = pr.stones + (size_t)rec * 8;
+        const BaseHdr *hd = da.hdr + game;
+        uint64_t ls[8], rs[8];
+        int nst = 0;
+#pragma unroll
+        for (int q = 0; q < 8; ++q) {
+            ls[q] = sb[q];
+            rs[q] = hd->stones[q];
+            nst += __popcll(ls[q]);
+        }
+        const int lw = pr.lw[rec];
+        const int h_tm = hd->to_move, h_valid = hd->valid;
+        const int tm = rzt::pend_lw_to_move(lw), lc = rzt::pend_lw_last(lw);
+        const bool has_last = nst > 0;
+        if ((unsigned)slot >= (unsigned)pr.n_slots) continue;
+        Leaf leaf;
+        int parity = 0, nD = 0;
+        bool use_delta = changed_cells(ls, rs, nst, tm, lc, has_last, h_valid != 0, h_tm, da.bw_rcp, BW, leaf.dys, leaf.dxs, parity, nD);
+        leaf.base = da.recs + ((size_t)game * 2 + parity) * kBaseBytes;
+        leaf.cell_planes = planes_of(ls, tid_r, tm, has_last, lc, nst);
+        leaf.dst16 = store16 + (size_t)slot * pr.slot_halfs + (size_t)(game >> 5) * nd.groups_act * 1024 + (game & 31) * 16;
+        leaf.vdst = nullptr;
+        leaf.dst32 = nullptr;
+        leaf.sets = nullptr;
+        leaf.deferred = false;
+        leaf.store_head = first;
+        first = false;
+        (void)delta_passes<false, 0, 4>(nd, da, lds, tid_r, wave, leaf, ly, headv, use_delta, prof);
+        __syncthreads();
+    }
+}
+
+}
diff --git a/rlzero_amd/csrc/rz_engine.hip b/rlzero_amd/csrc/rz_engine.hip
--- a/rlzero_amd/csrc/rz_engine.hip
+++ b/rlzero_amd/csrc/rz_engine.hip
@@ -147,7 +147,7 @@
     __shared__ int sh[4][2];
     const int g = blockIdx.x, tid = threadIdx.x, lane = tid & 63, wave = tid >> 6;
     const int n = E.pend[g] < E.pend_cap ? E.pend[g] : E.pend_cap;
-    const int keep = keep_of[g];
+    const int keep = keep_of != nullptr ? keep_of[g] : -2;
     uint64_t root[2][kWords], occ[kWords];
     load_board(E.root_stones, g, root);
 #pragma unroll
@@ -208,8 +208,10 @@
     }
     if (last && lane == 0) {
         Kp.count[0] = at;
-        Kp.stats[0] += (unsigned long long)at;
-        Kp.stats[1] += (unsigned long long)pending;
+        if (Kp.stats != nullptr) {
+            Kp.stats[0] += (unsigned long long)at;
+            Kp.stats[1] += (unsigned long long)pending;
+        }
     }
 }
 
@@ -1972,6 +1974,7 @@
     const long long G = e->cfg.n_games;
     if ((rc = dev_alloc(e, &e->dev.pend_pb, (long long)slots * G)) != RZ_OK) return rc;
     if ((rc = dev_alloc(e, &e->dev.pend_ctr, (long long)slots * G)) != RZ_OK) return rc;
+    if ((rc = dev_alloc(e, &e->dev.pend_lw, (long long)slots * G)) != RZ_OK) return rc;
     if ((rc = dev_alloc(e, &e->dev.pend_stones, (long long)slots * G * 2 * kWords)) != RZ_OK) return rc;
     if (e->dev.pend == nullptr) {
         if ((rc = dev_alloc(e, &e->dev.pend, G)) != RZ_OK) return rc;
@@ -2082,6 +2085,34 @@
     out->n_games = e->cfg.n_games;
     out->reserved = 0;
     return launched("k_keep_rows");
+}
+
+int rz_deferred_keep_all(rz_engine *e, rz_kept_rows *out, void *stream) {
+    int rc = check_engine(e);
+    if (rc != RZ_OK) return rc;
+    if (!out) return fail(RZ_ERR_ARG, "NULL output pointer");
+    if (e->dev.pend_cap <= 0) return fail(RZ_ERR_ARG, "call rz_deferred_reserve first");
+    Keep all = e->keep;
+    all.stats = nullptr;
+    k_keep_mark<<<per_game(e), dim3(256), 0, as_stream(stream)>>>(e->dev, nullptr, all);
+    k_keep_rows<<<per_game(e), dim3(kWave), 0, as_stream(stream)>>>(e->dev, all);
+    out->rows = e->keep.rows;
+    out->count = e->keep.count;
+    out->capacity = (int64_t)e->dev.pend_cap * e->cfg.n_games;
+    out->n_games = e->cfg.n_games;
+    out->reserved = 0;
+    return launched("k_keep_rows");
+}
+
+int rz_deferred_flush_rows(rz_engine *e, const rz_deferred_logits *logits, void *stream) {
+    int rc = check_engine(e);
+    if (rc != RZ_OK) return rc;
+    if (e->dev.pend_cap <= 0) return fail(RZ_ERR_ARG, "call rz_deferred_reserve first");
+    if (!logits || !logits->raw) return fail(RZ_ERR_ARG, "rz_deferred_logits: NULL pointer");
+    if (logits->ld < e->dev.A) return fail(RZ_ERR_ARG, "rz_deferred_logits: rows shorter than the policy");
+    k_deferred_priors_rows<<<dim3(2048), dim3(kWave), 0, as_stream(stream)>>>(e->dev, logits->raw, logits->ld, e->keep.rows, e->keep.count);
+    if (!(e->play_on && e->play_drawn)) k_deferred_reset<<<flat_grid(e), dim3(256), 0, as_stream(stream)>>>(e->dev);
+    return launched("k_deferred_priors_rows");
 }
 
 int rz_deferred_flush_kept(rz_engine *e, const rz_deferred_logits *logits, void *stream) {
diff --git a/rlzero_amd/csrc/rz_net.hip b/rlzero_amd/csrc/rz_net.hip
--- a/rlzero_amd/csrc/rz_net.hip
+++ b/rlzero_amd/csrc/rz_net.hip
@@ -3094,7 +3094,7 @@
     return RZ_OK;
 }
 
-int rz_net_search_resident(rz_net *net, rz_engine *engine, int32_t n_sims, int32_t select_first, void *stream) {
+static int search_resident(rz_net *net, rz_engine *engine, int32_t n_sims, int32_t select_first, void *stream, bool policy) {
     rzt::Dev dev;
     int rc = rz_device_view(engine, &dev, (int64_t)sizeof(dev));
     if (rc != RZ_OK) return rc;
@@ -3136,12 +3136,16 @@
     const dim3 grid((unsigned)dev.n_games);
     const hipStream_t st = (hipStream_t)stream;
     net->feat16_valid = net->feat32_valid = false;
+    if (!policy && !delta_res)
+        return net_fail(RZ_ERR_ARG, "rz_net_search_resident_values: the search without policy features is k_delta_res's (the default trunk on a board of "
+                                    "11 .. 16 rows and columns, rz_net_delta_reserve for the engine's games, rz_net_delta_resident on)");
     if (delta_res) {
         if (select_first) {
             if ((rc = rz_net_delta_bases(net, dev.root_stones, dev.root_to_move, dev.n_games, stream)) != RZ_OK) return rc;
         }
         dl::DeltaArgs da{net->d_base_hdr, net->d_base_recs, net->d_base_ones, nullptr, net->d_delta_stats, 0, (65536 + net->dev.BW - 1) / net->dev.BW, net->d_win};
-        dl::k_delta_res<<<grid, dim3(256), 0, st>>>(net->dev, net->d_store16, later, da, res);
+        if (policy) dl::k_delta_res<true><<<grid, dim3(256), 0, st>>>(net->dev, net->d_store16, later, da, res);
+        else dl::k_delta_res<false><<<grid, dim3(256), 0, st>>>(net->dev, net->d_store16, later, da, res);
         if (hipGetLastError() != hipSuccess) return net_fail(RZ_ERR_HIP, "launch of the resident search (k_delta_res) failed");
         return RZ_OK;
     }
@@ -3153,6 +3157,37 @@
         launch_trunk_split<true>(tc.ms, compact_res, grid, st, net->dev, nullptr, leaves, nullptr, net->d_store16, dev.n_games, net->d_flags,
                                  nullptr, nullptr, later, res);
     if (hipGetLastError() != hipSuccess) return net_fail(RZ_ERR_HIP, "launch of the resident search failed");
+    return RZ_OK;
+}
+
+int rz_net_search_resident(rz_net *net, rz_engine *engine, int32_t n_sims, int32_t select_first, void *stream) {
+    return search_resident(net, engine, n_sims, select_first, stream, true);
+}
+
+int rz_net_search_resident_values(rz_net *net, rz_engine *engine, int32_t n_sims, int32_t select_first, void *stream) {
+    return search_resident(net, engine, n_sims, select_first, stream, false);
+}
+
+int rz_net_policy_rows(rz_net *net, rz_engine *engine, const rz_kept_rows *kept, void *stream) {
+    if (!kept) return net_fail(RZ_ERR_ARG, "NULL argument");
+    rzt::Dev dev;
+    int rc = rz_device_view(engine, &dev, (int64_t)sizeof(dev));
+    if (rc != RZ_OK) return rc;
+    if ((rc = net_ready(net, dev.n_games)) != RZ_OK) return rc;
+    if (!kept->rows || !kept->count) return net_fail(RZ_ERR_ARG, "rz_kept_rows: NULL pointer");
+    if (!delta_covers(net) || net->base_games < dev.n_games || !split_trunk_ok(net))
+        return net_fail(RZ_ERR_ARG, "rz_net_policy_rows: the receptive-field trunk (the default trunk on a board of 11 .. 16 rows and columns) and "
+                                    "rz_net_delta_reserve for the engine's games");
+    if (dev.BH != net->dev.BH || dev.BW != net->dev.BW || dev.A != net->dev.A) return net_fail(RZ_ERR_ARG, "engine and network disagree on the board");
+    if (dev.pend_cap <= 0 || dev.pend_stones == nullptr || dev.pend_lw == nullptr) return net_fail(RZ_ERR_ARG, "rz_net_policy_rows: rz_deferred_reserve first");
+    if (kept->n_games != dev.n_games || dev.n_games > net->store_boards || kept->capacity < 1 || kept->capacity > (int64_t)dev.pend_cap * dev.n_games)
+        return net_fail(RZ_ERR_ARG, "rz_net_policy_rows: the rows are not this engine's, or more boards than rz_net_deferred_reserve()d");
+    dl::DeltaArgs da{net->d_base_hdr, net->d_base_recs, net->d_base_ones, nullptr, nullptr, 0, (65536 + net->dev.BW - 1) / net->dev.BW, nullptr};
+    const dl::PolicyRows pr{kept->rows, kept->count, dev.pend_stones, dev.pend_lw, dev.n_games, net->store_slots,
+                            (long long)net->store_tiles * net->dev.groups_act * 1024};
+    const dim3 grid((unsigned)(2 * (net->n_cus > 0 ? net->n_cus : 1)));
+    dl::k_trunk_policy_rows<<<grid, dim3(256), 0, (hipStream_t)stream>>>(net->dev, net->d_store16, da, pr);
+    if (hipGetLastError() != hipSuccess) return net_fail(RZ_ERR_HIP, "launch of k_trunk_policy_rows failed");
     return RZ_OK;
 }
 
diff --git a/rlzero_amd/csrc/rz_tree.h b/rlzero_amd/csrc/rz_tree.h
--- a/rlzero_amd/csrc/rz_tree.h
+++ b/rlzero_amd/csrc/rz_tree.h
@@ -41,6 +41,7 @@
     int pend_cap;
     int32_t *pend, *pend_pb, *pend_ctr;
     uint64_t *pend_stones;
+    int32_t *pend_lw;
     unsigned long long *trace;
     uint64_t valid[kWords];
     int bw_rcp, n_rcp;
@@ -48,6 +49,10 @@
     const uint64_t *line_tab;
     int line_masks;
 };
+
+__host__ __device__ __forceinline__ int pend_lw_pack(int to_move, int last) { return ((last + 1) & 0xffff) | (to_move << 16); }
+__host__ __device__ __forceinline__ int pend_lw_to_move(int lw) { return (lw >> 16) & 1; }
+__host__ __device__ __forceinline__ int pend_lw_last(int lw) { return (lw & 0xffff) - 1; }
 
 constexpr int kFirstCap = 4;
 __device__ __forceinline__ int rec_k(const int4 &lo) { return lo.w & 0xffff; }
@@ -768,6 +773,7 @@
     const int nblk = E.nblk[g];
     const int top_now = E.top[g];
     const int noise_ctr = E.noise_ctr[g];
+    const int leaf_tm = DEF ? E.leaf_to_move[gk] : 0, leaf_lc = DEF ? E.leaf_last[gk] : 0;
     const int32_t *path = E.path + (long long)gk * E.path_stride;
     const int path_lane = path[lane < E.path_stride ? lane : 0];
     uint64_t st[2][kWords];
@@ -874,6 +880,7 @@
                 if (lane == 0) {
                     E.pend_pb[rec] = ptop;
                     E.pend_ctr[rec] = noise_ctr;
+                    E.pend_lw[rec] = pend_lw_pack(leaf_tm, leaf_lc);
                     if (E.add_noise) E.noise_ctr[g] = noise_ctr + 1;
                 }
                 store_board<W>(E.pend_stones, (int)rec, st, lane);
diff --git a/rlzero_amd/engine.py b/rlzero_amd/engine.py
--- a/rlzero_amd/engine.py
+++ b/rlzero_amd/engine.py
@@ -207,6 +207,10 @@
         return self.route(environ={}).resident
 
     def search_resident(self, eng, n_sims, select_first=False):
+        if eng.__dict__.pop('_search_values', False):
+            check(self.lib.rz_net_search_resident_values(self.handle, eng.handle, int(n_sims), 1 if select_first else 0, self._stream()),
+                  'rz_net_search_resident_values')
+            return
         check(self.lib.rz_net_search_resident(self.handle, eng.handle, int(n_sims), 1 if select_first else 0, self._stream()), 'rz_net_search_resident')
 
     def deferred_gemm(self, n_boards, n_slots):
@@ -214,6 +218,9 @@
         check(self.lib.rz_net_deferred_gemm(self.handle, int(n_boards), int(n_slots), ctypes.byref(out), self._stream()),
               'rz_net_deferred_gemm')
         return out
+
+    def policy_rows(self, eng, kept):
+        check(self.lib.rz_net_policy_rows(self.handle, eng.handle, ctypes.byref(kept), self._stream()), 'rz_net_policy_rows')
 
     def deferred_gemm_rows(self, kept):
         out = _hip.RzDeferredLogits()
@@ -553,9 +560,12 @@
         self._graphs = {}
         self.roots_epoch = 0
         self._def_ev, self._def_pending, self._def_slots, self._def_slot_ptr, self._capturing = None, 0, 0, None, False
+        self._def_values = False
         self.deferred_max_bytes = 32 << 30
         self._playouts = None
         self.flush_kept = os.environ.get('RZ_FLUSH_KEPT', '1') != '0'
+        self.policy_on_demand = os.environ.get('RZ_POLICY_ON_DEMAND', '1') != '0'
+        self.search_launches = {True: 0, False: 0}
 
     def stream(self):
         return _current_stream(self.torch, self.device)
@@ -768,7 +778,7 @@
         if self._def_ev is not evaluator:
             self.flush_deferred()
             hip = evaluator.hip
-            per_slot = hip.deferred_bytes_per_slot(self.n_leaves) + 80 * self.n_games
+            per_slot = hip.deferred_bytes_per_slot(self.n_leaves) + 84 * self.n_games
             slots = int(max(16, min(max(self.n_playout, 16), self.deferred_max_bytes // per_slot)))
             if self._capturing:
                 raise HipError('the deferred-priors store must be reserved before a hipGraph capture (warm_graph does that)')
@@ -805,8 +815,10 @@
             if m < n and (self._playouts is not None or getattr(self, 'play_cap_on', False)):
                 raise ValueError('per-game simulation counts need the whole search in one launch: %d simulations, %d store slots' % (n, m))
             if resident:
+                self._search_mode(evaluator)
                 evaluator.search_resident(self, m, True)
             else:
+                self._search_mode(None)
                 check(lib.rz_select_step(h, None, self.stream()), 'rz_select_step')
                 for i in range(m):
                     head = evaluator.deferred_trunk(self)
@@ -819,6 +831,23 @@
                 self._def_stream = self.torch.cuda.current_stream(self.device)
             n -= m
 
+    def _search_mode(self, evaluator):
+        values = False
+        if evaluator is not None:
+            values = _route.policy_on_demand(self._ask(evaluator)[0], move_step=bool(getattr(self, '_play_on', False)),
+                                             flush_kept=bool(self.flush_kept), match=bool(getattr(self, 'play_match_on', False)),
+                                             allowed=bool(self.policy_on_demand))
+        if self._def_pending > 0 and values != self._def_values:
+            if self._capturing:
+                raise HipError('records of the other search mode are pending: flush before the capture')
+            self.flush_deferred()
+        if evaluator is not None:
+            self._search_values = values
+            self.search_launches[values] += 1
+        if not self._capturing:
+            self._def_values = values
+        return values
+
     def flush_deferred(self, move=False):
         if self._def_pending <= 0 or self._def_ev is None:
             return
@@ -826,7 +855,9 @@
         if then is not None and then != cur:
             cur.wait_stream(then)
         if move:
-            self._enqueue_move_flush(self._def_ev.hip, self._def_pending)
+            self._enqueue_move_flush(self._def_ev.hip, self._def_pending, self._def_values)
+        elif self._def_values:
+            self._enqueue_rows_flush(self._def_ev.hip, 'all')
         else:
             logits = self._def_ev.hip.deferred_gemm(self.n_leaves, self._def_pending)
             check(self.lib.rz_deferred_flush(self.handle, ctypes.byref(logits), self._def_pending, self.stream()), 'rz_deferred_flush')
@@ -834,9 +865,25 @@
             then.wait_stream(cur)
         self._def_pending = 0
 
-    def _enqueue_move_flush(self, hip, n_slots):
+    def _enqueue_rows_flush(self, hip, what):
         lib, h, st = self.lib, self.handle, self.stream()
-        if self.flush_kept:
+        kept = _hip.RzKeptRows()
+        if what == 'kept':
+            check(lib.rz_deferred_keep(h, ctypes.byref(kept), st), 'rz_deferred_keep')
+        else:
+            check(lib.rz_deferred_keep_all(h, ctypes.byref(kept), st), 'rz_deferred_keep_all')
+        hip.policy_rows(self, kept)
+        logits = hip.deferred_gemm_rows(kept)
+        if what == 'all':
+            check(lib.rz_deferred_flush_rows(h, ctypes.byref(logits), st), 'rz_deferred_flush_rows')
+        else:
+            check(lib.rz_deferred_flush_kept(h, ctypes.byref(logits), st), 'rz_deferred_flush_kept')
+
+    def _enqueue_move_flush(self, hip, n_slots, values=False):
+        lib, h, st = self.lib, self.handle, self.stream()
+        if values:
+            self._enqueue_rows_flush(hip, 'kept' if self.flush_kept else 'all_move')
+        elif self.flush_kept:
             kept = _hip.RzKeptRows()
             check(lib.rz_deferred_keep(h, ctypes.byref(kept), st), 'rz_deferred_keep')
             logits = hip.deferred_gemm_rows(kept)
@@ -1094,9 +1141,10 @@
         try:
             with t.cuda.graph(graph):
                 st = self.stream()
+                values = self._search_mode(evaluator)
                 evaluator.search_resident(self, n, True)
                 check(lib.rz_play_draw(h, st), 'rz_play_draw')
-                self._enqueue_move_flush(hip, n)
+                self._enqueue_move_flush(hip, n, values)
                 check(lib.rz_play_apply(h, st), 'rz_play_apply')
         finally:
             self._capturing = False
diff --git a/rlzero_amd/route.py b/rlzero_amd/route.py
--- a/rlzero_amd/route.py
+++ b/rlzero_amd/route.py
@@ -34,6 +34,18 @@
     return rows <= 10 and (n_actions * 4 * cells + 64 * 2 * cells) * 4 <= 40 * 1024
 
 
+def policy_on_demand(route, move_step=False, flush_kept=True, match=False, allowed=True):
+    return bool(route.resident and route.resident_delta and move_step and flush_kept and not match and allowed)
+
+
+def pend_lw_pack(to_move, last):
+    return ((int(last) + 1) & 0xffff) | (int(to_move) << 16)
+
+
+def pend_lw_unpack(word):
+    return (int(word) >> 16) & 1, (int(word) & 0xffff) - 1
+
+
 Route = namedtuple('Route', 'needs_planes deferred delta delta_three_launch resident resident_delta compact_resident resident_per_cu')
 Route.__doc__ = """How the leaves of a search are evaluated:
 needs_planes        the trunk reads float observation planes (otherwise the engine's leaf bitboards: no plane is written)
```

After: 24.41 million (median of 6 runs). 1.07x the previous value.
